# JakobHavtorn/benchmarking-lvms

Hardware: AMD Instinct MI355X
Metric: audio frames/sec training (VRNN, 16 kHz mu-law) (higher is better)
Workload: dtype f32

## Files before the change

### benchmarking-lvms_amd/blvm/ops.py

```python
import ctypes
from typing import List, NamedTuple, Optional, Sequence

import torch

from . import _hip
from ._hip import VrnnWeights, check, load, ptr, stream_ptr

ACT_NONE, ACT_RELU, ACT_LEAKY = 0, 1, 2
LEAKY_SLOPE = 0.01

LAYOUT_BATCH_MAJOR, LAYOUT_TIME_MAJOR = 0, 1

seq_timer_hook = None


def _tick(tag):
    if seq_timer_hook is not None:
        seq_timer_hook(tag)


def _c_ints(v):
    return (ctypes.c_int * len(v))(*[int(i) for i in v])


# ... 626 lines not shown


def _rollout(scratch_floats, T, max_scratch_floats, who, x, call, carry):
    n = _steps_per_launch(scratch_floats, T, max_scratch_floats, who) if T > 0 else 0
    scratch = torch.empty(scratch_floats(n), device=x.device, dtype=torch.float32)
    if n == T:
        call(0, T, None, x, scratch)
        return
    state = None
    for t0 in range(0, T, n):
        t1 = min(T, t0 + n)
        xc = torch.empty(x.shape[0], t1 - t0, x.shape[2], device=x.device, dtype=torch.float32)
        call(t0, t1, state, xc, scratch)
        x[:, t0:t1] = xc
        state = carry(xc, t1)


def _decode_weight_ptrs(w, first, first_lin, dec_lin, lik_lin):
    keep = [_f32c(t) for lin in (*first_lin, *dec_lin, lik_lin) for t in (lin.weight, lin.bias)]
    names = [f"{part}_{k}{i}" for part in (first, "dec") for i in range(3) for k in "wb"] + ["lik_w", "lik_b"]
    _hip.fill(w, names, [ptr(t) for t in keep])
    return keep


def _head_scalars(head):
    if isinstance(head, DmolHead):
        return 0, int(head.num_mix), float(head.log_eps), 0.0, 0.0
    if isinstance(head, GmmHead):
        return 1, int(head.num_mix), 0.0, float(head.sd_beta), float(head.sd_eps)
    if isinstance(head, GaussHead):
        return 2, 0, 0.0, float(head.sd_beta), float(head.sd_eps)
    raise TypeError(f"head: one of ops.DmolHead, ops.GmmHead, ops.GaussHead (got {type(head).__name__})")


@torch.no_grad()
def vrnn_decode(enc_lin, cell_params, dec_lin, lik_lin, x0, h0, eps, u, v, S, H, Z, R, num_mix, sd_eps, slope, log_eps, whole_chip=None,
                max_scratch_floats=None, head=None):
    from ._hip import VrnnDecodeWeights

    lib = load()
    T, B = eps.shape[0], x0.shape[0]
    dev = x0.device
    cp = [_f32c(p) for p in cell_params]
    cw = _pack_weights(cp)
    w = VrnnDecodeWeights()
    keep = _decode_weight_ptrs(w, "enc", enc_lin, dec_lin, lik_lin)
    w.cell = ctypes.pointer(cw)
    x0, eps = _f32c(x0), _f32c(eps)
    h0 = _f32c(h0) if h0 is not None else None
    u = _f32c(u) if u is not None else None
    v = _f32c(v) if v is not None else None
    if whole_chip is None:
        whole_chip = B <= lib.blvm_pchain_max_batch()
    hs5 = None if head is None else _head_scalars(head)
    x = torch.empty(B, T, S, device=dev, dtype=torch.float32)
    hn = torch.empty(B, R, device=dev, dtype=torch.float32)
    if whole_chip:

        def call(t0, t1, state, xc, scratch):
            xs, hs = (x0, h0) if state is None else state
            uc, vc = (None if u is None else u[t0:t1]), (None if v is None else v[t0:t1])
            if hs5 is None:
                check(lib.blvm_vrnn_generate(ctypes.byref(w), ptr(xs), ptr(hs), ptr(eps[t0:t1]), ptr(uc), ptr(vc), t1 - t0, B, S, H, Z, R, num_mix,
                                             sd_eps, slope, log_eps, ptr(xc), ptr(hn), ptr(scratch), stream_ptr()), "blvm_vrnn_generate")
            else:
                check(lib.blvm_vrnn_generate_head(ctypes.byref(w), ptr(xs), ptr(hs), ptr(eps[t0:t1]), ptr(uc), ptr(vc), t1 - t0, B, S, H, Z, R, *hs5,
                                                  sd_eps, slope, ptr(xc), ptr(hn), ptr(scratch), stream_ptr()), "blvm_vrnn_generate_head")

        floats = ((lambda n: lib.blvm_vrnn_generate_scratch_floats(n, B, S, H, Z, R)) if hs5 is None
                  else (lambda n: lib.blvm_vrnn_generate_scratch_floats_head(n, B, S, H, Z, R, hs5[0])))
        _rollout(floats, T, max_scratch_floats, "vrnn_decode", x, call, lambda xc, t1: (xc[:, -1].contiguous(), hn.clone()))
        return x, hn
    scratch = torch.empty(lib.blvm_vrnn_decode_scratch_floats(S, H, Z, R), device=dev, dtype=torch.float32)
    if hs5 is None:
        check(lib.blvm_vrnn_decode(ctypes.byref(w), ptr(x0), ptr(h0), ptr(eps), ptr(u), ptr(v), T, B, S, H, Z, R, num_mix, sd_eps, slope,
                                   log_eps, ptr(x), ptr(hn), ptr(scratch), stream_ptr()), "blvm_vrnn_decode")
    else:
        check(lib.blvm_vrnn_decode_head(ctypes.byref(w), ptr(x0), ptr(h0), ptr(eps), ptr(u), ptr(v), T, B, S, H, Z, R, *hs5, sd_eps, slope,
                                        ptr(x), ptr(hn), ptr(scratch), stream_ptr()), "blvm_vrnn_decode_head")
    return x, hn


class _VRNNSeqFunction(torch.autograd.Function):

    @staticmethod
    def forward(ctx, enc, h0, eps, x_sl_dev, cfg, dec, *params):
        Tp, B, X, H, Z, R, residual, sd_eps, stride, fn_floor = cfg
        enc, eps = _f32c(enc), _f32c(eps)
        params, dparams = tuple(_f32c(p) for p in params[:28]), tuple(_f32c(p) for p in params[28:])
        dev = enc.device
        lib = load()
        f32 = dict(device=dev, dtype=torch.float32)
        decin = torch.empty(Tp + 1, B, H + R, **f32)
        mu_q, sd_q, mu_p, sd_p, z = (torch.empty(Tp, B, Z, **f32) for _ in range(5))
        w = _pack_weights(params)
        if dec is None:
            reserve = torch.empty(lib.blvm_vrnn_reserve_floats(Tp, B, X, H, Z, R), **f32)
            _tick("fwd_begin")
            check(
                lib.blvm_vrnn_seq_fwd(w, ptr(enc), ptr(_f32c(h0)) if h0 is not None else None, ptr(eps), Tp, B, X, H, Z, R,
                                      int(residual), sd_eps, ptr(decin), ptr(mu_q), ptr(sd_q), ptr(mu_p), ptr(sd_p), ptr(z),
                                      ptr(reserve), stream_ptr()),
                "blvm_vrnn_seq_fwd",
            )
        else:
            keep = [_f32c(t.detach()) for lin in dec.layers for t in (lin.weight, lin.bias)]
            DH, SF = keep[0].shape[0], keep[4].shape[0]
            ys = [torch.empty(Tp * B, n, **f32) for n in (DH, DH, SF)]
            three = ctypes.c_void_p * 3
            dw, db, dy = three(*(ptr(t) for t in keep[0::2])), three(*(ptr(t) for t in keep[1::2])), three(*(ptr(t) for t in ys))
            reserve = torch.empty(lib.blvm_vrnn_fwd_reserve_floats(Tp, B, X, H, Z, R, DH, SF), **f32)
            folded = ctypes.c_int(0)
            _tick("fwd_begin")
            check(
                lib.blvm_vrnn_seq_fwd_dec(w, ptr(enc), ptr(_f32c(h0)) if h0 is not None else None, ptr(eps), Tp, B, X, H, Z, R,
                                          int(residual), sd_eps, ptr(decin), ptr(mu_q), ptr(sd_q), ptr(mu_p), ptr(sd_p), ptr(z),
                                          ptr(reserve), dw, db, dy, DH, SF, dec.slope, ctypes.byref(folded), stream_ptr()),
                "blvm_vrnn_seq_fwd_dec",
            )
            dec.given = tuple(ys[: folded.value]) if folded.value else None
        joint = dec is not None and len(dparams) == 6 and dec.given is not None and len(dec.given) == 3
        _tick("fwd_end")
        kld = torch.zeros(B, device=dev, dtype=torch.float64)
        kld_fn = torch.zeros(B, device=dev, dtype=torch.float64)
        check(
            lib.blvm_kl_fwd(ptr(mu_q), ptr(sd_q), ptr(mu_p), ptr(sd_p), LAYOUT_TIME_MAJOR, ptr(x_sl_dev), B, Tp, Z, stride,
                            fn_floor, ptr(kld), ptr(kld_fn), stream_ptr()),
            "blvm_kl_fwd",
        )
        ctx.cfg = cfg
        ctx.has_h0 = h0 is not None
        ctx.joint, ctx.n_dpar, ctx.dec_slope = joint, len(dparams), dec.slope if joint else 0.0
        ctx.save_for_backward(enc, eps, x_sl_dev, decin, mu_q, sd_q, mu_p, sd_p, z, reserve, *params, *((*dparams, ys[0], ys[1]) if joint else ()))
        ctx.mark_non_differentiable(mu_q, sd_q, mu_p, sd_p, z)
        ctx.set_materialize_grads(False)
        return decin, kld, kld_fn, mu_q, sd_q, mu_p, sd_p, z, (ys[2] if joint else None)

    @staticmethod
    def backward(ctx, d_decin, g_kld, g_kld_fn, *rest):
        Tp, B, X, H, Z, R, residual, sd_eps, stride, fn_floor = ctx.cfg
        enc, eps, x_sl_dev, decin, mu_q, sd_q, mu_p, sd_p, z, reserve, *params = ctx.saved_tensors
        dev = enc.device
        lib = load()
        f32 = dict(device=dev, dtype=torch.float32)
        c_raw = _grad_f32(g_kld) if g_kld is not None else None
        c_fn = _grad_f32(g_kld_fn) if g_kld_fn is not None else None
        d_dec = rest[5] if ctx.joint else None
        dgrads = (None,) * ctx.n_dpar
        if d_dec is not None:
            params, (W1, b1, W2, b2, W3, b3, y1, y2) = params[:28], params[28:]
            dz3, M, DH, SF, slope = _f32c(d_dec), Tp * B, W2.shape[0], W3.shape[0], ctx.dec_slope
            dy2, dy1 = torch.empty(M, DH, **f32), torch.empty(M, DH, **f32)
            grads = _zeros_like_many(params)
            d_enc = torch.empty_like(enc)
            d_h0 = torch.empty(B, R, **f32) if ctx.has_h0 else None
            w, g = _pack_weights(params), _pack_weights(grads, _hip.VrnnGrads)
            folded = ctypes.c_int(0)
            if d_decin is None:
                ws = torch.empty(lib.blvm_vrnn_bwd_dec_workspace_floats(Tp, B, X, H, Z, R, DH, SF), **f32)
                dw = (ctypes.c_void_p * 3)(ptr(W1), ptr(W2), ptr(W3))
                _tick("bwd_begin")
                check(
                    lib.blvm_vrnn_seq_bwd_dec(w, ptr(enc), ptr(eps), ptr(decin), ptr(mu_q), ptr(sd_q), ptr(mu_p), ptr(sd_p), ptr(z),
                                              ptr(reserve), ptr(x_sl_dev), ptr(c_raw), ptr(c_fn), stride, fn_floor, Tp, B, X, H, Z, R,
                                              int(residual), sd_eps, ptr(d_enc), ptr(d_h0), g, ptr(ws), ptr(dz3), ptr(y1), ptr(y2), dw,
                                              ptr(dy2), ptr(dy1), DH, SF, slope, ctypes.byref(folded), stream_ptr()),
                    "blvm_vrnn_seq_bwd_dec",
                )
            if not folded.value:
                gemm(0, 1, M, DH, SF, dz3, SF, W3, DH, dy2, DH, slope=slope, gate=y2, ldg=DH)
                gemm(0, 1, M, DH, DH, dy2, DH, W2, DH, dy1, DH, slope=slope, gate=y1, ldg=DH)
                dx = torch.empty(M, H + R, **f32)
                gemm(0, 1, M, H + R, DH, dy1, DH, W1, H + R, dx, H + R, slope=slope)
                dd = torch.zeros_like(decin)
                dd[:Tp] = dx.view(Tp, B, H + R)
                if d_decin is not None:
                    dd = dd + _f32c(d_decin)
                ws = torch.empty(lib.blvm_vrnn_bwd_workspace_floats(Tp, B, X, H, Z, R), **f32)
                _tick("bwd_begin")
                check(
                    lib.blvm_vrnn_seq_bwd(w, ptr(enc), ptr(eps), ptr(decin), ptr(mu_q), ptr(sd_q), ptr(mu_p), ptr(sd_p), ptr(z),
                                          ptr(reserve), ptr(dd), ptr(x_sl_dev), ptr(c_raw), ptr(c_fn), stride, fn_floor, Tp, B,
                                          X, H, Z, R, int(residual), sd_eps, ptr(d_enc), ptr(d_h0), g, ptr(ws), stream_ptr()),
                    "blvm_vrnn_seq_bwd",
                )
            _tick("bwd_end")
            dpar = (W1, b1, W2, b2, W3, b3)
            want = [ctx.needs_input_grad[6 + 28 + i] for i in range(6)]
            sizes = [(dpar[i].numel() + 3) // 4 * 4 if want[i] else 0 for i in range(6)]
            flat = torch.zeros(sum(sizes), **f32)
            views, off = [], 0
            for i in range(6):
                views.append(flat[off : off + dpar[i].numel()].view(dpar[i].shape) if want[i] else None)
                off += sizes[i]
            x2d = decin[:Tp].view(M, H + R)
            wgrad_group([(dz3, y2, views[4], views[5]), (dy2, y1, views[2], views[3]), (dy1, x2d, views[0], views[1])], M)
            return (d_enc, d_h0, None, None, None, None, *grads, *views)
        params = params[:28]
        d_decin = _f32c(d_decin) if d_decin is not None else torch.zeros_like(decin)
        grads = _zeros_like_many(params)
        d_enc = torch.empty_like(enc)
        d_h0 = torch.empty(B, R, **f32) if ctx.has_h0 else None
        ws = torch.empty(lib.blvm_vrnn_bwd_workspace_floats(Tp, B, X, H, Z, R), **f32)
        w, g = _pack_weights(params), _pack_weights(grads, _hip.VrnnGrads)
        _tick("bwd_begin")
        check(
            lib.blvm_vrnn_seq_bwd(w, ptr(enc), ptr(eps), ptr(decin), ptr(mu_q), ptr(sd_q), ptr(mu_p), ptr(sd_p), ptr(z),
                                  ptr(reserve), ptr(d_decin), ptr(x_sl_dev), ptr(c_raw), ptr(c_fn), stride, fn_floor, Tp, B,
                                  X, H, Z, R, int(residual), sd_eps, ptr(d_enc), ptr(d_h0), g, ptr(ws), stream_ptr()),
            "blvm_vrnn_seq_bwd",
        )
        _tick("bwd_end")
        return (d_enc, d_h0, None, None, None, None, *grads, *dgrads)


def vrnn_sequence(enc, h0, eps, x_sl_dev, params: Sequence[torch.Tensor], X, H, Z, R, residual_posterior, stride,
                  free_nats=0.0, sd_eps=1e-6, decoder=None):
    Tp, B, _ = enc.shape
    fn_floor = float(free_nats) / Z if free_nats else 0.0
    cfg = (Tp, B, X, H, Z, R, int(residual_posterior), float(sd_eps), int(stride), fn_floor)
    if decoder is None:
        return _VRNNSeqFunction.apply(enc, h0, eps, x_sl_dev, cfg, None, *params)[:8]
    decoder.given = decoder.dec = None
    dparams = ()
    if decoder.head_gates and load().blvm_vrnn_dec_bwd_fold(-1):
        dparams = tuple(t for lin in decoder.layers for t in (lin.weight, lin.bias))
    *out, decoder.dec = _VRNNSeqFunction.apply(enc, h0, eps, x_sl_dev, cfg, decoder, *params, *dparams)
    return tuple(out)


class DecoderFold:

    def __init__(self, layers, slope: float = LEAKY_SLOPE, head_gates: bool = False):
        self.layers, self.slope, self.given, self.head_gates, self.dec = list(layers), float(slope), None, bool(head_gates), None




class _LSTMSeqFunction(torch.autograd.Function):
    @staticmethod
    def forward(ctx, inp, h0, c0, lens_dev, Wih, Whh, bih, bhh):
        inp, Wih, Whh, bih, bhh = (_f32c(t) for t in (inp, Wih, Whh, bih, bhh))
        T, B, I = inp.shape
        H = Whh.shape[1]
        lib = load()
        f32 = dict(device=inp.device, dtype=torch.float32)
        out = torch.empty(T, B, H, **f32)
        hn, cn = torch.empty(B, H, **f32), torch.empty(B, H, **f32)
        reserve = torch.empty(lib.blvm_lstm_reserve_floats(T, B, H), **f32)
        check(
            lib.blvm_lstm_seq_fwd(ptr(Wih), ptr(Whh), ptr(bih), ptr(bhh), ptr(inp), ptr(_f32c(h0)) if h0 is not None else None,
                                  ptr(_f32c(c0)) if c0 is not None else None, ptr(lens_dev), T, B, I, H, ptr(out), ptr(hn), ptr(cn),
                                  ptr(reserve), stream_ptr()),
            "blvm_lstm_seq_fwd",
        )
        ctx.dims = (T, B, I, H)
        ctx.has_state = (h0 is not None, c0 is not None)
        ctx.save_for_backward(inp, Wih, Whh, reserve)
        ctx.mark_non_differentiable(hn, cn)
        return out, hn, cn

    @staticmethod
    def backward(ctx, d_out, _dhn, _dcn):
        T, B, I, H = ctx.dims
        inp, Wih, Whh, reserve = ctx.saved_tensors
        lib = load()
        f32 = dict(device=inp.device, dtype=torch.float32)
        d_out = _f32c(d_out)
        d_in = torch.empty_like(inp) if ctx.needs_input_grad[0] else None
        d_h0 = torch.empty(B, H, **f32) if ctx.has_state[0] and ctx.needs_input_grad[1] else None
        d_c0 = torch.empty(B, H, **f32) if ctx.has_state[1] and ctx.needs_input_grad[2] else None
        dWih, dWhh = torch.zeros_like(Wih), torch.zeros_like(Whh)
        dbih, dbhh = torch.zeros(4 * H, **f32), torch.zeros(4 * H, **f32)
        ws = torch.empty(lib.blvm_lstm_bwd_workspace_floats(T, B, H), **f32)
        check(
            lib.blvm_lstm_seq_bwd(ptr(Wih), ptr(Whh), ptr(inp), ptr(reserve), ptr(d_out), T, B, I, H, ptr(d_in), ptr(d_h0),
                                  ptr(d_c0), ptr(dWih), ptr(dWhh), ptr(dbih), ptr(dbhh), ptr(ws), stream_ptr()),
            "blvm_lstm_seq_bwd",
        )
        return d_in, d_h0, d_c0, None, dWih, dWhh, dbih, dbhh


def lstm_sequence(inp, h0, c0, lens_dev, Wih, Whh, bih, bhh):
    return _LSTMSeqFunction.apply(inp, h0, c0, lens_dev, Wih, Whh, bih, bhh)


class _LSTMBidirSeqFunction(torch.autograd.Function):

    @staticmethod
    def forward(ctx, inp, lens_dev, Wih_f, Whh_f, bih_f, bhh_f, Wih_r, Whh_r, bih_r, bhh_r):
        inp, *params = (_f32c(t) for t in (inp, Wih_f, Whh_f, bih_f, bhh_f, Wih_r, Whh_r, bih_r, bhh_r))
        T, B, I = inp.shape
        H = params[1].shape[1]
        lib = load()
        if not lib.blvm_lstm_bidir_applies(T, B, H):
            return None
        f32 = dict(device=inp.device, dtype=torch.float32)
        out = torch.empty(T, B, 2 * H, **f32)
        reserve = torch.empty(lib.blvm_lstm_bidir_reserve_floats(T, B, H), **f32)
        rc = lib.blvm_lstm_bidir_fwd(*(ptr(p) for p in params), ptr(inp), ptr(lens_dev), T, B, I, H, ptr(out), ptr(reserve), stream_ptr())
        if rc == BLVM_NOT_APPLICABLE:
            return None
        check(rc, "blvm_lstm_bidir_fwd")
        ctx.dims = (T, B, I, H)
        ctx.save_for_backward(inp, lens_dev, reserve, *params)
        return out

    @staticmethod
    def backward(ctx, d_out):
        T, B, I, H = ctx.dims
        inp, lens_dev, reserve, Wih_f, Whh_f, bih_f, bhh_f, Wih_r, Whh_r, bih_r, bhh_r = ctx.saved_tensors
        lib = load()
        d_out = _f32c(d_out)
        d_in = torch.empty_like(inp) if ctx.needs_input_grad[0] else None
        grads = [torch.zeros_like(p) for p in (Wih_f, Whh_f, bih_f, bhh_f, Wih_r, Whh_r, bih_r, bhh_r)]
        ws = torch.empty(lib.blvm_lstm_bidir_bwd_workspace_floats(T, B, H), device=inp.device, dtype=torch.float32)
        check(
            lib.blvm_lstm_bidir_bwd(ptr(Wih_f), ptr(Whh_f), ptr(Wih_r), ptr(Whh_r), ptr(inp), ptr(lens_dev), ptr(reserve), ptr(d_out),
                                    T, B, I, H, ptr(d_in), *(ptr(g) for g in grads), ptr(ws), stream_ptr()),
            "blvm_lstm_bidir_bwd",
        )
        return (d_in, None, *grads)


def lstm_bidir_sequence(inp, lens_dev, fwd_params, rev_params):
    return _LSTMBidirSeqFunction.apply(inp, lens_dev, *fwd_params, *rev_params)


def lstm_bidir_path_counts():
    out = (ctypes.c_ulonglong * 2)()
    check(load().blvm_lstm_bidir_path_counts(out), "blvm_lstm_bidir_path_counts")
    return int(out[0]), int(out[1])


def lstm_decode_weights(emb_lin, lstm, dec_lin, lik_lin):
    L = lstm.num_layers
    lk = [[_f32c(getattr(lstm, f"{n}_l{l}")) for l in range(L)] for n in ("weight_ih", "weight_hh", "bias_ih", "bias_hh")]
    arrays = [(ctypes.c_void_p * L)(*[t.data_ptr() for t in ts]) for ts in lk]
    w = _hip.LstmDecodeWeights()
    keep = _decode_weight_ptrs(w, "emb", emb_lin, dec_lin, lik_lin)
    w.wih, w.whh, w.bih, w.bhh = (ctypes.cast(a, ctypes.POINTER(ctypes.c_void_p)) for a in arrays)
    return w, (keep, lk, arrays)


def lstm_generate(emb_lin, lstm, dec_lin, lik_lin, x0, h0, c0, u, v, S, H, num_mix, log_eps, T=None, max_scratch_floats=None):
    lib = load()
    L, B, dev = lstm.num_layers, x0.shape[0], x0.device
    if (u is None) != (v is None) or (u is None and T is None):
        raise ValueError("lstm_generate: u and v are given together; the mode (neither) needs T")
    T = int(T) if u is None else u.shape[0]
    w, _keep = lstm_decode_weights(emb_lin, lstm, dec_lin, lik_lin)
    x0 = _f32c(x0)
    h0 = _f32c(h0) if h0 is not None else None
    c0 = _f32c(c0) if c0 is not None else None
# ... 1217 lines not shown
```

### benchmarking-lvms_amd/csrc/vrnn.hip

```cpp
#include <vector>
#include <stdlib.h>

#include <algorithm>
#include <atomic>

#include "common.h"
#include "pchain.h"
#include "vrnn_static.h"

namespace blvm {
namespace {

#include "stages.h"


template <int NW>
__global__ __launch_bounds__(NW * 64) void gru_stage_kernel(const float* decin_t, const float* Wih, const float* xg,
                                                            const float* gh, int B, int H, int R, float* decin_next,
                                                            float* rg, float* ug, float* ng) {
  __shared__ float red[3 * NW * 256];
  const int r0 = blockIdx.y * 16, c0 = blockIdx.x * 16, wave = threadIdx.x >> 6;
  const int ldd = H + R;
  const int t = threadIdx.x & 255;
  const int row = r0 + (t >> 4), col = c0 + (t & 15);
// ... 5 lines not shown
  const float hp = decin_t[(size_t)rowc * ldd + H + col];
  f32x4 acc[3];
#pragma unroll
  for (int g = 0; g < 3; ++g) acc[g] = (f32x4){0.f, 0.f, 0.f, 0.f};
  {
    const float* const As[3] = {decin_t, decin_t, decin_t};
    const float* const Ws[3] = {Wih, Wih, Wih};
    const int la[3] = {ldd, ldd, ldd}, lw[3] = {H, H, H}, cs[3] = {c0, R + c0, 2 * R + c0};
    wave_gemm16_multi<NW, 3, true>(As, la, r0, B, Ws, lw, cs, H, wave, acc);
  }
  float v[3];
  reduce_tiles<3, NW>(acc, red, v);
  if (!own) return;
  const float r = sigmoidf_(v[0] + x0 + hr);
  const float u = sigmoidf_(v[1] + x1 + hz);
  const float n = tanhf(v[2] + x2 + r * hn);
  decin_next[(size_t)row * ldd + H + col] = (1.f - u) * n + u * hp;
  const size_t o = (size_t)row * R + col;
  rg[o] = r; ug[o] = u; ng[o] = n;
}

struct DhArgs {
  const float *DP0, *DQ0;
  const float *WpT, *WqT;
  float* G;
  const float *rg, *ug, *ng, *gh;
  const float* decin_s;
  const float* ddecin_s;
  float *dgi, *dgh;
  int B, H, R, has_gemm, has_gates;
};

template <int NW>
__global__ __launch_bounds__(NW * 64) void dh_stage_kernel(const float* DP0, const float* DQ0, const float* WpT, const float* WqT,
                                                           float* G, unsigned b_h, int R, unsigned has, DhArgs a) {
  const int B = b_h & 0xffff, H = b_h >> 16;
  const int has_gemm = has & 1, has_gates = (has >> 1) & 1;
  __shared__ float red[2 * NW * 256];
  const int r0 = blockIdx.y * 16, c0 = blockIdx.x * 16, wave = threadIdx.x >> 6;
  const int ldd = H + R;
  const int t = threadIdx.x & 255;
  const int row = r0 + (t >> 4), col = c0 + (t & 15);
  const bool own = threadIdx.x < 256 && row < B;
  const int rowc = row < B ? row : r0;
  const size_t o = (size_t)rowc * R + col, o3 = (size_t)rowc * 3 * R + col;
  const float g0 = G[o];
  float r = 0.f, u = 0.f, n = 0.f, hn = 0.f, hp = 0.f, dd = 0.f;
  auto prefetch = [&]() {
    if (has_gates) {
      r = a.rg[o]; u = a.ug[o]; n = a.ng[o]; hn = a.gh[o3 + 2 * R];
      hp = a.decin_s[(size_t)rowc * ldd + H + col];
      dd = a.ddecin_s[(size_t)rowc * ldd + H + col];
    }
  };
  float v[2] = {0.f, 0.f};
  if (has_gemm) {
    f32x4 acc[2];
    acc[0] = (f32x4){0.f, 0.f, 0.f, 0.f};
    acc[1] = (f32x4){0.f, 0.f, 0.f, 0.f};
    {
      const float* const As[2] = {DP0, DQ0};
      const float* const Ws[2] = {WpT, WqT};
      const int ld[2] = {H, H}, cs[2] = {c0, c0};
      wave_gemm16_multi<NW, 2, false>(As, ld, r0, B, Ws, ld, cs, H, wave, acc, prefetch);
    }
    reduce_tiles<2, NW>(acc, red, v);
  } else {
    prefetch();
  }
  if (!own) return;
  const float g = g0 + v[0] + v[1];
  if (!has_gates) { G[o] = g; return; }
  const float dn_pre = g * (1.f - u) * (1.f - n * n);
  const float du_pre = g * (hp - n) * u * (1.f - u);
  const float dr_pre = dn_pre * hn * r * (1.f - r);
  a.dgi[o3] = dr_pre; a.dgi[o3 + R] = du_pre; a.dgi[o3 + 2 * R] = dn_pre;
  a.dgh[o3] = dr_pre; a.dgh[o3 + R] = du_pre; a.dgh[o3 + 2 * R] = dn_pre * r;
  G[o] = g * u + dd;
}

inline int vrnn_rt_max_b() {
  static int v = [] {
    const char* e = getenv("BLVM_PCHAIN_RT_MAX_B");
    return e ? atoi(e) : 256;
  }();
  return v;
}
inline int vrnn_rt(int B) {
  static const int min_b = [] { const char* e = getenv("BLVM_PCHAIN_RT_MIN_B"); return e ? atoi(e) : 65; }();
  if (B < min_b || B > vrnn_rt_max_b() || pchain_max_batch() <= 0 || operand_16bit()) return 0;
  if (B <= kPchainCarveMaxB && B > pchain_max_batch()) return 0;
  return 2;
}
inline bool vrnn_row_groups(int B) { return vrnn_rt(B) > 0; }
inline bool vrnn_shared_deal(bool groups, int tl) {
  static const int forced = [] { const char* e = getenv("BLVM_PCHAIN_SHARED"); return e ? atoi(e) : -1; }();
  static const int rt_tl = [] { const char* e = getenv("BLVM_PCHAIN_RT_SHARED_TL"); return e ? atoi(e) : 7; }();
  if (forced >= 0) return forced != 0;
  return groups && rt_tl > 0 && tl >= rt_tl;
}
inline bool vrnn_persistent(int B) { return pchain_applies(B) || vrnn_row_groups(B); }

struct Reserve {
  float *P[3], *Q[3], *FZ[3], *GHb, *RG, *UG, *NG, *XQ, *XG, *RAWQ, *RAWP;
  float *Wp[3], *Wq[3], *Wph, *Wqh, *Wf[4], *Wih, *Whh;
  float *H16, *P16[3], *Q16[3], *Z16, *FZ16[3], *PHI16;
  float *Y116, *Y216, *Y1P, *Wd[3];
  size_t x16_bytes;
};

size_t carve_reserve(float* base, int Tp, int B, int H, int Z, int R, Reserve* r, int SF = 0) {
  const size_t n = (size_t)Tp * B;
  Arena ar{base};
  Reserve tmp;
  for (int i = 0; i < 3; ++i) tmp.P[i] = ar.take(n * H);
  for (int i = 0; i < 3; ++i) tmp.Q[i] = ar.take(n * H);
  for (int i = 0; i < 3; ++i) tmp.FZ[i] = ar.take(n * H);
  tmp.GHb = ar.take(n * 3 * R);
  tmp.RG = ar.take(n * R); tmp.UG = ar.take(n * R); tmp.NG = ar.take(n * R);
  tmp.XQ = ar.take(n * H);
  tmp.XG = ar.take(n * 3 * R);
  tmp.RAWQ = ar.take(n * Z); tmp.RAWP = ar.take(n * Z);
  tmp.Wp[0] = ar.take((size_t)H * R); tmp.Wq[0] = ar.take((size_t)H * R);
  for (int i = 1; i < 3; ++i) { tmp.Wp[i] = ar.take((size_t)H * H); tmp.Wq[i] = ar.take((size_t)H * H); }
  tmp.Wph = ar.take((size_t)2 * Z * H); tmp.Wqh = ar.take((size_t)2 * Z * H);
  tmp.Wf[0] = ar.take((size_t)H * Z);
  for (int i = 1; i < 4; ++i) tmp.Wf[i] = ar.take((size_t)H * H);
  tmp.Wih = ar.take((size_t)3 * R * H); tmp.Whh = ar.take((size_t)3 * R * R);
  tmp.H16 = nullptr;
  if (B <= kPchainCarveMaxB || B <= vrnn_rt_max_b()) {
    const size_t rows = (size_t)((B + 15) / 16) * 16, m = (size_t)Tp * rows;
    tmp.H16 = ar.take((m + rows) * R);
    for (int i = 0; i < 3; ++i) tmp.P16[i] = ar.take(m * H);
    for (int i = 0; i < 3; ++i) tmp.Q16[i] = ar.take(m * H);
    tmp.Z16 = ar.take(m * Z);
    for (int i = 0; i < 3; ++i) tmp.FZ16[i] = ar.take(m * H);
    tmp.PHI16 = ar.take(m * H);
    tmp.Y116 = tmp.Y216 = tmp.Y1P = nullptr;
    if (SF > 0) { tmp.Y116 = ar.take(m * H); tmp.Y216 = ar.take(m * H); tmp.Y1P = ar.take(n * H); }
    tmp.x16_bytes = ar.bytes_from(tmp.H16);
    if (SF > 0) { tmp.Wd[0] = ar.take((size_t)H * (H + R)); tmp.Wd[1] = ar.take((size_t)H * H); tmp.Wd[2] = ar.take((size_t)SF * H); }
  }
  if (r) *r = tmp;
  return ar.floats();
}

struct BwdWs {
  float *pT[3], *phT, *qT[3], *qhT, *fT[4], *wihT, *whhT;
  float *DGI, *DGH, *DPHI[4], *DQH, *DPH, *DP[3], *DQ[3], *G;
  float *GA, *GB, *DP16[3], *DQ16[3], *DGI16, *DGH16, *DPHI16[4], *DPH16, *DQH16, *DPHI16b, *DPHI16c;
  size_t x16_bytes;
  float *DPHI3b, *DPHI3c;
  float *DY216, *DY116, *DD, *dT[3];
};

size_t carve_ws(float* base, int Tp, int B, int X, int H, int Z, int R, BwdWs* w, int SF = 0) {
  (void)X;
  const size_t n = (size_t)Tp * B;
  Arena ar{base};
  BwdWs t;
  t.pT[0] = ar.take((size_t)R * H); t.pT[1] = ar.take((size_t)H * H); t.pT[2] = ar.take((size_t)H * H);
  t.phT = ar.take((size_t)H * 2 * Z);
  t.qT[0] = ar.take((size_t)R * H); t.qT[1] = ar.take((size_t)H * H); t.qT[2] = ar.take((size_t)H * H);
  t.qhT = ar.take((size_t)H * 2 * Z);
  t.fT[0] = ar.take((size_t)Z * H);
  for (int i = 1; i < 4; ++i) t.fT[i] = ar.take((size_t)H * H);
  t.wihT = ar.take((size_t)H * 3 * R);
  t.whhT = ar.take((size_t)R * 3 * R);
  t.DGI = ar.take(n * 3 * R); t.DGH = ar.take(n * 3 * R);
  for (int i = 0; i < 4; ++i) t.DPHI[i] = ar.take(n * H);
  t.DQH = ar.take(n * 2 * Z); t.DPH = ar.take(n * 2 * Z);
  for (int i = 0; i < 3; ++i) t.DP[i] = ar.take(n * H);
  for (int i = 0; i < 3; ++i) t.DQ[i] = ar.take(n * H);
  t.G = ar.take((size_t)B * R);
  t.GA = nullptr;
  if (B <= kPchainCarveMaxB || B <= vrnn_rt_max_b()) {
    const size_t m = (size_t)Tp * ((B + 15) / 16) * 16;
    t.GA = ar.take(n * R); t.GB = ar.take(n * R);
    for (int i = 0; i < 3; ++i) { t.DP16[i] = ar.take(m * H); t.DQ16[i] = ar.take(m * H); }
    t.DGI16 = ar.take(m * 3 * R); t.DGH16 = ar.take(m * 3 * R);
    for (int i = 0; i < 4; ++i) t.DPHI16[i] = ar.take(m * H);
    t.DPH16 = ar.take(m * 2 * Z); t.DQH16 = ar.take(m * 2 * Z);
    t.DPHI16b = ar.take(m * H); t.DPHI16c = ar.take(m * H);
    t.DY216 = t.DY116 = t.DD = nullptr;
    if (SF > 0) { t.DY216 = ar.take(m * H); t.DY116 = ar.take(m * H); t.DD = ar.take(n * (H + R)); }
    t.x16_bytes = ar.bytes_from(t.GA);
    t.DPHI3b = ar.take(n * H); t.DPHI3c = ar.take(n * H);
    if (SF > 0) { t.dT[0] = ar.take((size_t)(H + R) * H); t.dT[1] = ar.take((size_t)H * H); t.dT[2] = ar.take((size_t)H * SF); }
  }
  if (w) *w = t;
  return ar.floats();
}

__global__ __launch_bounds__(256) void add3_kernel(float4* __restrict__ a, const float4* __restrict__ b, const float4* __restrict__ c, size_t n4) {
  for (size_t i = (size_t)blockIdx.x * 256 + threadIdx.x; i < n4; i += (size_t)gridDim.x * 256) {
    float4 x = a[i];
    const float4 y = b[i], z = c[i];
    x.x += y.x + z.x; x.y += y.y + z.y; x.z += y.z + z.z; x.w += y.w + z.w;
    a[i] = x;
  }
}

inline bool pchain_split3() {
  static int v = [] {
    const char* e = getenv("BLVM_PCHAIN_SPLIT3");
    return e ? atoi(e) : 1;
  }();
  return v != 0;
}

struct VrnnDecoder {
  const float *w[3], *b[3];
  float* y[3];
};
int g_dec_fold = [] { const char* e = getenv("BLVM_VRNN_DEC_FOLD"); const int v = e ? atoi(e) : 1; return v >= 0 && v <= 2 ? v : 1; }();
long g_dec_folded = 0;
int dec_ct(int layers, int SF) { return layers == 3 ? SF / 16 : layers == 2 ? 1 : 0; }
int vrnn_dec_folds(int B, int H, int Z, int R, int DH, int SF) {
  if (!g_dec_fold || !vrnn_persistent(B) || device_cus() < 32 || operand_16bit() || pchain_optype(B) != OP_F32) return 0;
  if (B > 64 || vrnn_row_groups(B) || Z != H || DH != H || SF <= 0 || SF % 16 != 0) return 0;
  const int tl = (B + 15) / 16, layers = g_dec_fold == 2 ? 2 : 3;
  const bool fits = pchain::vrnn_fwd_deal(H / 16, Z / 16, R / 16, tl, device_cus() & ~7, vrnn_shared_deal(false, tl), dec_ct(layers, SF)).dec[0].nwg > 0;
  return fits ? layers : 0;
}

struct VrnnDecBwd {
  const float *dz3, *y1, *y2, *w[3];
  float *dy2, *dy1;
  int DH, SF;
  float slope;
};
int g_dec_bwd_fold = [] { const char* e = getenv("BLVM_VRNN_DEC_BWD_FOLD"); return e ? (atoi(e) != 0 ? 1 : 0) : 1; }();
long g_dec_bwd_folded = 0;
bool vrnn_dec_bwd_folds(int Tp, int B, int H, int Z, int R, int DH, int SF) {
  if (!g_dec_bwd_fold || !vrnn_persistent(B) || device_cus() < 32 || operand_16bit() || pchain_optype(B) != OP_F32) return false;
  if (B > 64 || vrnn_row_groups(B) || Z != H || DH != H || H != 256 || R != 512 || SF <= 0 || SF % 16 != 0) return false;
  if (Tp + 1 <= pchain::kArmAhead || Tp <= pchain::kBdecAhead) return false;
  const int tl = (B + 15) / 16;
  if (vrnn_shared_deal(false, tl)) return false;
  const pchain::VrnnBwdDeal dl = pchain::vrnn_bwd_deal(H / 16, Z / 16, R / 16, tl, device_cus() & ~7, false, pchain_split3(), (H + R) / 16);
  return dl.split3 && dl.bdec[0].nwg > 0;
}

enum { VRNN_FWD_PROGRAM = 0, VRNN_FWD_PER_LINK = 1, VRNN_BWD_PROGRAM = 2, VRNN_BWD_PER_LINK = 3, VRNN_ROW_GROUPS = 4, VRNN_LIN16 = 5, VRNN_LIN32 = 6 };
std::atomic<unsigned long long> g_vrnn_counts[7];
inline void count_vrnn(int k) { g_vrnn_counts[k].fetch_add(1, std::memory_order_relaxed); }
inline void count_lin(int tile_width) { count_vrnn(tile_width == 32 ? VRNN_LIN32 : VRNN_LIN16); }

int check_dims(int Tp, int B, int X, int H, int Z, int R) {
  BLVM_REQUIRE(Tp > 0 && B > 0, "vrnn: bad Tp=%d B=%d", Tp, B);
  BLVM_REQUIRE(X > 0 && H > 0 && Z > 0 && R > 0 && X % 16 == 0 && H % 16 == 0 && Z % 16 == 0 && R % 16 == 0,
               "vrnn: X,H,Z,R must be positive multiples of 16 (got %d,%d,%d,%d)", X, H, Z, R);
  BLVM_REQUIRE(B < 65536 && H < 65536 && R < 65536, "vrnn: B, H and R must be below 65536 (packed kernel arguments)");
  return BLVM_OK;
}

}
}

using namespace blvm;

extern "C" int blvm_vrnn_path_counts(unsigned long long out[7]) {
  BLVM_REQUIRE(out, "vrnn_path_counts: null pointer");
  for (int k = 0; k < 7; ++k) out[k] = g_vrnn_counts[k].load(std::memory_order_relaxed);
  return BLVM_OK;
}

extern "C" size_t blvm_vrnn_reserve_floats(int Tp, int B, int X, int H, int Z, int R) {
  (void)X;
  return carve_reserve(nullptr, Tp, B, H, Z, R, nullptr);
}
extern "C" size_t blvm_vrnn_fwd_reserve_floats(int Tp, int B, int X, int H, int Z, int R, int DH, int SF) {
  (void)X;
  return carve_reserve(nullptr, Tp, B, H, Z, R, nullptr, vrnn_dec_folds(B, H, Z, R, DH, SF) ? SF : 0);
}
extern "C" int blvm_vrnn_dec_fold(int mode) {
  if (mode == -2) return (int)std::min<long>(g_dec_folded, 0x7fffffffL);
  const int was = g_dec_fold;
  if (mode >= 0) g_dec_fold = mode <= 2 ? mode : 1;
  return was;
}

extern "C" size_t blvm_vrnn_bwd_workspace_floats(int Tp, int B, int X, int H, int Z, int R) {
  return carve_ws(nullptr, Tp, B, X, H, Z, R, nullptr);
}
extern "C" size_t blvm_vrnn_bwd_dec_workspace_floats(int Tp, int B, int X, int H, int Z, int R, int DH, int SF) {
  return carve_ws(nullptr, Tp, B, X, H, Z, R, nullptr, vrnn_dec_bwd_folds(Tp, B, H, Z, R, DH, SF) ? SF : 0);
}
extern "C" int blvm_vrnn_dec_bwd_fold(int mode) {
  if (mode == -2) return (int)std::min<long>(g_dec_bwd_folded, 0x7fffffffL);
  const int was = g_dec_bwd_fold;
  if (mode >= 0) g_dec_bwd_fold = mode != 0;
  return was;
}

static int vrnn_seq_fwd_impl(const BlvmVrnnWeights* w, const float* enc, const float* h0, const float* eps,
                             int Tp, int B, int X, int H, int Z, int R, int residual_posterior, float sd_eps,
                             float* decin, float* mu_q, float* sd_q, float* mu_p, float* sd_p, float* z,
                             float* reserve, hipStream_t s, const VrnnDecoder* dec = nullptr, int DH = 0, int SF = 0,
                             float dec_slope = 0.f, int* folded = nullptr) {
  BLVM_TRY(check_dims(Tp, B, X, H, Z, R));
  BLVM_REQUIRE(w && enc && eps && decin && mu_q && sd_q && mu_p && sd_p && z && reserve, "vrnn_fwd: null pointer");
  BLVM_REQUIRE(aligned16(enc) && aligned16(decin) && aligned16(reserve) && aligned16(z),
               "vrnn_fwd: buffers must be 16-byte aligned");
  if (folded) *folded = 0;
  const int fold = dec != nullptr ? vrnn_dec_folds(B, H, Z, R, DH, SF) : 0;
  Reserve rs;
  carve_reserve(reserve, Tp, B, H, Z, R, &rs, fold ? SF : 0);
  const size_t n = (size_t)Tp * B;
  const int ldd = H + R;
  const float beta = softplus_beta_of(sd_eps);

  BLVM_TRY(gemm_f32(0, 0, (int)n, H, X, enc, X, w->post_w[0] + R, R + X, rs.XQ, H, w->post_b[0], 0, 0.f, nullptr, 0, 0, 1, s));
  BLVM_TRY(gemm_f32(0, 0, (int)n, 3 * R, X, enc, X, w->gru_wih, X + H, rs.XG, 3 * R, w->gru_bih, 0, 0.f, nullptr, 0, 0, 1, s));

  T16PackScope pack_scope(pchain_optype(B), s);
  BLVM_TRY(t16_pack_rows(w->prior_w[0], R, H, R, rs.Wp[0], s));
  BLVM_TRY(t16_pack_rows(w->post_w[0], R + X, H, R, rs.Wq[0], s));
  for (int l = 1; l < 3; ++l) {
    BLVM_TRY(t16_pack_rows(w->prior_w[l], H, H, H, rs.Wp[l], s));
    BLVM_TRY(t16_pack_rows(w->post_w[l], H, H, H, rs.Wq[l], s));
  }
  BLVM_TRY(t16_pack_rows(w->prior_hw, H, 2 * Z, H, rs.Wph, s));
  BLVM_TRY(t16_pack_rows(w->post_hw, H, 2 * Z, H, rs.Wqh, s));
  BLVM_TRY(t16_pack_rows(w->phi_w[0], Z, H, Z, rs.Wf[0], s));
  for (int l = 1; l < 4; ++l) BLVM_TRY(t16_pack_rows(w->phi_w[l], H, H, H, rs.Wf[l], s));
  BLVM_TRY(t16_pack_rows(w->gru_wih + X, X + H, 3 * R, H, rs.Wih, s));
  BLVM_TRY(t16_pack_rows(w->gru_whh, R, 3 * R, R, rs.Whh, s));
  if (fold) {
    BLVM_TRY(t16_pack_rows(dec->w[0], H + R, H, H + R, rs.Wd[0], s));
    BLVM_TRY(t16_pack_rows(dec->w[1], H, H, H, rs.Wd[1], s));
    if (fold == 3) BLVM_TRY(t16_pack_rows(dec->w[2], H, SF, H, rs.Wd[2], s));
  }
  BLVM_TRY(pack_scope.flush());

  if (!(vrnn_persistent(B) && device_cus() >= 32)) BLVM_HIP(copy_or_zero_2d(decin + H, sizeof(float) * ldd, h0, sizeof(float) * R, B, s));
  BLVM_HIP(hipMemset2DAsync(decin + n * ldd, sizeof(float) * ldd, 0, sizeof(float) * H, B, s));

  const int rt = (B + 15) / 16;
  if (vrnn_persistent(B) && device_cus() >= 32) {
    using namespace pchain;
    const int ctH = H / 16, ctZ = Z / 16, ctR = R / 16, cus = device_cus() & ~7;
    const long sH = (long)B * H, sZ = (long)B * Z, sR = (long)B * R, s3R = 3 * sR, sD = (long)B * ldd;
    const long xH = (long)rt * 16 * H, xZ = (long)rt * 16 * Z, xR = (long)rt * 16 * R;
    const bool groups = vrnn_row_groups(B);
    count_vrnn(VRNN_FWD_PROGRAM);
    if (groups) count_vrnn(VRNN_ROW_GROUPS);
    const int RTG = groups ? vrnn_rt(B) : 1;
    const int tl = (rt + RTG - 1) / RTG;
    const bool shared = vrnn_shared_deal(groups, tl);
    const VrnnFwdDeal dl = vrnn_fwd_deal(ctH, ctZ, ctR, tl, cus, shared, dec_ct(fold, SF));
    Builder bld;
    bld.begin(pchain_optype(B), Tp, B, groups ? 8 : 4, false, dl.g);
    bld.p.rt_group = RTG;
    Operands hp;
    hp.p[LIN_A] = {rs.H16, xR}; hp.p[LIN_W] = rs.Whh; hp.p[LIN_BIAS] = w->gru_bhh; hp.p[LIN_ORM] = {rs.GHb, s3R}; hp.ld[LD_OUT] = 3 * R;
    auto hproj = [&]() { add_desc(bld, K_LIN, dl.hproj.ct, dl.hproj.wg0, dl.hproj.nwg, R, DF_RM_SC1 | DF_GENTLE | ((pchain_tune() & 16) ? DF_CANARY : 0), 0, Tp, hp); };
    if (!shared) hproj();
    {
      const SeqLink lp[3] = {{rs.Wp[0], w->prior_b[0], rs.P[0], sH, H, rs.P16[0]}, {rs.Wp[1], w->prior_b[1], rs.P[1], sH, H, rs.P16[1]}, {rs.Wp[2], w->prior_b[2], rs.P[2], sH, H, rs.P16[2]}};
      const SeqLink lq[3] = {{rs.Wq[0], nullptr, rs.Q[0], sH, H, rs.Q16[0]}, {rs.Wq[1], w->post_b[1], rs.Q[1], sH, H, rs.Q16[1]}, {rs.Wq[2], w->post_b[2], rs.Q[2], sH, H, rs.Q16[2]}};
      add_linseq(bld, ctH, dl.prior.wg0, dl.prior.nwg, H, true, false, 0, Tp, {rs.H16, xR}, 3, lp, 0, xH, ctH, 0.f, 0, R);
      add_linseq(bld, ctH, dl.post.wg0, dl.post.nwg, H, true, false, 0, Tp, {rs.H16, xR}, 3, lq, 0, xH, ctH, 0.f, 0, R, {rs.XQ, sH}, H);
    }
    if (shared) hproj();
    {
      Operands o;
      o.p[HEAD_P16] = {rs.P16[2], xH}; o.p[HEAD_Q16] = {rs.Q16[2], xH}; o.p[HEAD_WP] = rs.Wph; o.p[HEAD_BP] = w->prior_hb; o.p[HEAD_WQ] = rs.Wqh;
      o.p[HEAD_BQ] = w->post_hb; o.p[HEAD_EPS] = {eps, sZ}; o.p[HEAD_MU_P] = {mu_p, sZ}; o.p[HEAD_SD_P] = {sd_p, sZ}; o.p[HEAD_MU_Q] = {mu_q, sZ};
      o.p[HEAD_SD_Q] = {sd_q, sZ}; o.p[HEAD_RAW_P] = {rs.RAWP, sZ}; o.p[HEAD_RAW_Q] = {rs.RAWQ, sZ}; o.p[HEAD_Z] = {z, sZ}; o.p[HEAD_Z16] = {rs.Z16, xZ};
      o.ld[LD_OUT] = Z; o.n16[N16_OUT] = ctZ; o.i[HEAD_I_Z] = Z; o.i[HEAD_I_RESIDUAL] = residual_posterior; o.f[HEAD_F_BETA] = beta; o.f[HEAD_F_INV_BETA] = 1.f / beta;
      o.f[HEAD_F_SD_EPS] = sd_eps;
      add_desc(bld, K_HEAD, ctZ, dl.head.wg0, dl.head.nwg, H, 0, 0, Tp, o);
    }
    const int first_seq = Z == H ? 0 : 1;
    if (first_seq) {
      Operands o;
      o.p[LIN_A] = {rs.Z16, xZ}; o.p[LIN_W] = rs.Wf[0]; o.p[LIN_BIAS] = w->phi_b[0]; o.p[LIN_ORM] = {rs.FZ[0], sH}; o.ld[LD_OUT] = H; o.p[LIN_O16] = {rs.FZ16[0], xH};
      o.n16[N16_OUT] = ctH;
      add_desc(bld, K_LIN, ctH, dl.phi.wg0, dl.phi.nwg, Z, DF_RELU, 0, Tp, o);
    }
    {
      SeqLink lf[4];
      for (int l = first_seq; l < 4; ++l)
        lf[l - first_seq] = SeqLink{rs.Wf[l], w->phi_b[l], l == 3 ? decin : rs.FZ[l], l == 3 ? sD : sH, l == 3 ? ldd : H, l == 3 ? rs.PHI16 : rs.FZ16[l]};
      add_linseq(bld, ctH, dl.phi.wg0, dl.phi.nwg, H, true, false, 0, Tp, first_seq == 0 ? Ptr(rs.Z16, xZ) : Ptr(rs.FZ16[0], xH), 4 - first_seq,
                 lf, 0, xH, ctH, 0.f, 0);
    }
    {
      Operands o;
      o.p[GRU_X16] = {rs.PHI16, xH}; o.p[GRU_WIH] = rs.Wih; o.p[GRU_XG] = {rs.XG, s3R}; o.p[GRU_GH] = {rs.GHb, s3R}; o.p[GRU_HPREV] = {decin + H, sD};
      o.p[GRU_HRM] = {decin + sD + H, sD}; o.p[GRU_H16] = {rs.H16 + xR, xR}; o.p[GRU_RG] = {rs.RG, sR}; o.p[GRU_UG] = {rs.UG, sR}; o.p[GRU_NG] = {rs.NG, sR};
      o.ld[GRU_LD_HPREV] = ldd; o.ld[LD_OUT] = ldd; o.n16[N16_OUT] = ctR; o.i[GRU_I_R] = R;
      add_desc(bld, K_GRU, ctR, dl.gru.wg0, dl.gru.nwg, H, 0, 0, Tp, o);
    }
    if (fold) {
      const long sF = (long)B * SF;
      const int canary = (pchain_tune() & 16) ? DF_CANARY : 0, ldw = H + R;
      Operands o;
      o.p[LIN_A] = {rs.H16, xR}; o.p[LIN_W] = rs.Wd[0] + (size_t)ctH * 256; o.i[LIN_I_W_WIDTH] = ldw; o.p[LIN_BIAS] = dec->b[0];
      o.p[LIN_ORM] = {rs.Y1P, sH}; o.ld[LD_OUT] = H;
      add_desc(bld, K_LIN, dl.dec[0].ct, dl.dec[0].wg0, dl.dec[0].nwg, R, DF_RM_SC1 | DF_GENTLE | canary, 0, Tp, o);
      o = Operands();
      o.p[LIN_A] = {rs.PHI16, xH}; o.p[LIN_W] = rs.Wd[0]; o.i[LIN_I_W_WIDTH] = ldw; o.p[LIN_ADD] = {rs.Y1P, sH}; o.ld[LIN_LD_ADD] = H;
      o.p[LIN_ORM] = {dec->y[0], sH}; o.ld[LD_OUT] = H; o.p[LIN_O16] = {rs.Y116, xH}; o.n16[N16_OUT] = ctH; o.f[LIN_F_SLOPE] = dec_slope;
      add_desc(bld, K_LIN, dl.dec[1].ct, dl.dec[1].wg0, dl.dec[1].nwg, H, DF_ADD_POLLED | DF_RELU | DF_GENTLE | canary, 0, Tp, o);
      o = Operands();
      o.p[LIN_A] = {rs.Y116, xH}; o.p[LIN_W] = rs.Wd[1]; o.p[LIN_BIAS] = dec->b[1]; o.p[LIN_ORM] = {dec->y[1], sH}; o.ld[LD_OUT] = H;
      o.p[LIN_O16] = {rs.Y216, xH}; o.n16[N16_OUT] = ctH; o.f[LIN_F_SLOPE] = dec_slope;
      add_desc(bld, K_LIN, dl.dec[2].ct, dl.dec[2].wg0, dl.dec[2].nwg, H, DF_RELU | DF_GENTLE | canary, 0, Tp, o);
      if (fold == 3) {
        o = Operands();
        o.p[LIN_A] = {rs.Y216, xH}; o.p[LIN_W] = rs.Wd[2]; o.p[LIN_BIAS] = dec->b[2]; o.p[LIN_ORM] = {dec->y[2], sF}; o.ld[LD_OUT] = SF;
        o.f[LIN_F_SLOPE] = dec_slope;
        add_desc(bld, K_LIN, dl.dec[3].ct, dl.dec[3].wg0, dl.dec[3].nwg, H, DF_RELU | DF_GENTLE | canary, 0, Tp, o);
      }
    }
    ArmPlan plan;
    plan.fill(rs.H16, rs.x16_bytes);
    plan.fill(rs.GHb, sizeof(float) * n * 3 * R);
    plan.fill(decin, sizeof(float) * n * ldd);
    if (!groups) {
      plan.add(arm_t16(rs.H16, R, rt, Tp + 1));
      for (int i = 0; i < 3; ++i) { plan.add(arm_t16(rs.P16[i], H, rt, Tp)); plan.add(arm_t16(rs.Q16[i], H, rt, Tp)); plan.add(arm_t16(rs.FZ16[i], H, rt, Tp)); }
      plan.add(arm_t16(rs.Z16, Z, rt, Tp));
      plan.add(arm_t16(rs.PHI16, H, rt, Tp));
      plan.add(arm_t16(rs.Y116, H, rt, Tp)); plan.add(arm_t16(rs.Y216, H, rt, Tp));
      plan.add(arm_rm(rs.Y1P, H, B, Tp));
      plan.add(arm_rm(rs.GHb, 3 * R, B, Tp));
      plan.add(arm_rm(decin, ldd, B, Tp));
    }
    auto pre = [&]() -> int {
      BLVM_HIP(copy_or_zero_2d(decin + H, sizeof(float) * ldd, h0, sizeof(float) * R, B, s));
      return pchain_rows_to_t16(h0, R, B, R, rs.H16, s);
    };
    BLVM_TRY(vrnn_launch(bld, true, "vrnn_fwd", s, plan, pre));
    if (fold) { ++g_dec_folded; if (folded) *folded = fold; }
    return BLVM_OK;
  }
  count_vrnn(VRNN_FWD_PER_LINK);
  for (int t = 0; t < Tp; ++t) {
    const size_t oH = (size_t)t * B * H, oZ = (size_t)t * B * Z, oR = (size_t)t * B * R, o3R = (size_t)t * B * 3 * R;
    const float* dec_t = decin + (size_t)t * B * ldd;
    float* dec_n = decin + (size_t)(t + 1) * B * ldd;
    const float* hprev = dec_t + H;
    LinLaunch a;
    a.B = B;
    a.nseg = 3;
    a.seg[0] = seg(hprev, ldd, rs.Wp[0], R, w->prior_b[0], nullptr, 0, nullptr, 0, rs.P[0] + oH, H, H, R, 1);
    a.seg[1] = seg(hprev, ldd, rs.Wq[0], R, nullptr, rs.XQ + oH, H, nullptr, 0, rs.Q[0] + oH, H, H, R, 1);
    a.seg[2] = seg(hprev, ldd, rs.Whh, R, w->gru_bhh, nullptr, 0, nullptr, 0, rs.GHb + o3R, 3 * R, 3 * R, R, 0);
    count_lin(launch_lin(a, s));
    a.nseg = 2;
    for (int l = 1; l < 3; ++l) {
      a.seg[0] = seg(rs.P[l - 1] + oH, H, rs.Wp[l], H, w->prior_b[l], nullptr, 0, nullptr, 0, rs.P[l] + oH, H, H, H, 1);
      a.seg[1] = seg(rs.Q[l - 1] + oH, H, rs.Wq[l], H, w->post_b[l], nullptr, 0, nullptr, 0, rs.Q[l] + oH, H, H, H, 1);
      count_lin(launch_lin(a, s));
    }
    HeadArgs h;
    h.P = rs.P[2] + oH; h.Q = rs.Q[2] + oH;
    h.Wp = rs.Wph; h.bp = w->prior_hb; h.Wq = rs.Wqh; h.bq = w->post_hb;
    h.eps = eps + oZ;
    h.mu_p = mu_p + oZ; h.sd_p = sd_p + oZ; h.mu_q = mu_q + oZ; h.sd_q = sd_q + oZ; h.z = z + oZ;
    h.raw_p = rs.RAWP + oZ; h.raw_q = rs.RAWQ + oZ;
    h.B = B; h.H = H; h.Z = Z; h.residual = residual_posterior;
    h.beta = beta; h.inv_beta = 1.f / beta; h.sd_eps = sd_eps; h.muq_raw = nullptr;
    launch_head(h, pick_nw(H, 4), dim3(Z / 16, rt), s);
    a.nseg = 1;
    a.seg[0] = seg(z + oZ, Z, rs.Wf[0], Z, w->phi_b[0], nullptr, 0, nullptr, 0, rs.FZ[0] + oH, H, H, Z, 1);
    count_lin(launch_lin(a, s));
    a.seg[0] = seg(rs.FZ[0] + oH, H, rs.Wf[1], H, w->phi_b[1], nullptr, 0, nullptr, 0, rs.FZ[1] + oH, H, H, H, 1);
    count_lin(launch_lin(a, s));
    a.seg[0] = seg(rs.FZ[1] + oH, H, rs.Wf[2], H, w->phi_b[2], nullptr, 0, nullptr, 0, rs.FZ[2] + oH, H, H, H, 1);
    count_lin(launch_lin(a, s));
    a.seg[0] = seg(rs.FZ[2] + oH, H, rs.Wf[3], H, w->phi_b[3], nullptr, 0, nullptr, 0, decin + (size_t)t * B * ldd, ldd, H, H, 1);
    count_lin(launch_lin(a, s));
    {
      const int nw = pick_nw(H, 3);
      const dim3 grid(R / 16, rt);
      const float *xg_t = rs.XG + o3R, *gh_t = rs.GHb + o3R;
      float *rg_t = rs.RG + oR, *ug_t = rs.UG + oR, *ng_t = rs.NG + oR;
      LAUNCH_NW(gru_stage_kernel<NW_>, nw, grid, s, dec_t, (const float*)rs.Wih, xg_t, gh_t, B, H, R, dec_n, rg_t, ug_t, ng_t);
    }
  }
  BLVM_CHECK_LAUNCH("vrnn_seq_fwd");
  return BLVM_OK;
}

extern "C" int blvm_vrnn_seq_fwd(const BlvmVrnnWeights* w, const float* enc, const float* h0, const float* eps,
                                 int Tp, int B, int X, int H, int Z, int R, int residual_posterior, float sd_eps,
                                 float* decin, float* mu_q, float* sd_q, float* mu_p, float* sd_p, float* z,
                                 float* reserve, void* stream_) {
  return vrnn_seq_fwd_impl(w, enc, h0, eps, Tp, B, X, H, Z, R, residual_posterior, sd_eps, decin, mu_q, sd_q, mu_p, sd_p, z, reserve,
                           static_cast<hipStream_t>(stream_));
}

extern "C" int blvm_vrnn_seq_fwd_dec(const BlvmVrnnWeights* w, const float* enc, const float* h0, const float* eps,
                                     int Tp, int B, int X, int H, int Z, int R, int residual_posterior, float sd_eps,
                                     float* decin, float* mu_q, float* sd_q, float* mu_p, float* sd_p, float* z,
                                     float* reserve, const float* const* dec_w, const float* const* dec_b, float* const* dec_y,
                                     int DH, int SF, float slope, int* folded, void* stream_) {
  BLVM_REQUIRE(dec_w && dec_b && dec_y && folded, "vrnn_seq_fwd_dec: null pointer");
  VrnnDecoder d;
  for (int l = 0; l < 3; ++l) {
    d.w[l] = dec_w[l]; d.b[l] = dec_b[l]; d.y[l] = dec_y[l];
    BLVM_REQUIRE(d.w[l] && d.b[l] && d.y[l] && aligned16(d.y[l]), "vrnn_seq_fwd_dec: decoder layer %d: null or unaligned pointer", l);
  }
  BLVM_REQUIRE(DH > 0 && SF > 0, "vrnn_seq_fwd_dec: bad decoder widths %d, %d", DH, SF);
  return vrnn_seq_fwd_impl(w, enc, h0, eps, Tp, B, X, H, Z, R, residual_posterior, sd_eps, decin, mu_q, sd_q, mu_p, sd_p, z, reserve,
                           static_cast<hipStream_t>(stream_), &d, DH, SF, slope, folded);
}

static int vrnn_seq_bwd_impl(const BlvmVrnnWeights* w, const float* enc, const float* eps, const float* decin,
                             const float* mu_q, const float* sd_q, const float* mu_p, const float* sd_p,
                             const float* z, const float* reserve, const float* d_decin, const int32_t* x_sl,
                             const float* c_raw, const float* c_fn, int stride, float fn_floor, int Tp, int B, int X, int H, int Z,
                             int R, int residual_posterior, float sd_eps, float* d_enc, float* d_h0,
                             const BlvmVrnnGrads* gr, float* workspace, hipStream_t s, const VrnnDecBwd* dec = nullptr) {
  BLVM_TRY(check_dims(Tp, B, X, H, Z, R));
  BLVM_REQUIRE(w && enc && eps && decin && mu_q && sd_q && mu_p && sd_p && z && reserve && (d_decin || dec) && workspace && gr,
               "vrnn_bwd: null pointer");
  BLVM_REQUIRE((c_fn == nullptr && c_raw == nullptr) || x_sl != nullptr, "vrnn_bwd: KL coefficients need x_sl");
  BLVM_REQUIRE(aligned16(workspace) && aligned16(reserve) && aligned16(d_decin), "vrnn_bwd: buffers must be 16-byte aligned");
  Reserve rs;
  carve_reserve(const_cast<float*>(reserve), Tp, B, H, Z, R, &rs);
  BwdWs ws;
  carve_ws(workspace, Tp, B, X, H, Z, R, &ws, dec ? dec->SF : 0);
  const size_t n = (size_t)Tp * B;
  const int ldd = H + R;
  const float beta = softplus_beta_of(sd_eps);

  T16PackScope pack_scope(pchain_optype(B), s);
  BLVM_TRY(t16_pack_transposed(w->prior_w[0], R, H, R, ws.pT[0], s));
  BLVM_TRY(t16_pack_transposed(w->prior_w[1], H, H, H, ws.pT[1], s));
  BLVM_TRY(t16_pack_transposed(w->prior_w[2], H, H, H, ws.pT[2], s));
  BLVM_TRY(t16_pack_transposed(w->prior_hw, H, 2 * Z, H, ws.phT, s));
  BLVM_TRY(t16_pack_transposed(w->post_w[0], R + X, H, R, ws.qT[0], s));
  BLVM_TRY(t16_pack_transposed(w->post_w[1], H, H, H, ws.qT[1], s));
  BLVM_TRY(t16_pack_transposed(w->post_w[2], H, H, H, ws.qT[2], s));
  BLVM_TRY(t16_pack_transposed(w->post_hw, H, 2 * Z, H, ws.qhT, s));
  BLVM_TRY(t16_pack_transposed(w->phi_w[0], Z, H, Z, ws.fT[0], s));
  for (int i = 1; i < 4; ++i) BLVM_TRY(t16_pack_transposed(w->phi_w[i], H, H, H, ws.fT[i], s));
  BLVM_TRY(t16_pack_transposed(w->gru_wih + X, X + H, 3 * R, H, ws.wihT, s));
  BLVM_TRY(t16_pack_transposed(w->gru_whh, R, 3 * R, R, ws.whhT, s));
  if (dec) {
    BLVM_TRY(t16_pack_transposed(dec->w[0], H + R, H, H + R, ws.dT[0], s));
    BLVM_TRY(t16_pack_transposed(dec->w[1], H, H, H, ws.dT[1], s));
    BLVM_TRY(t16_pack_transposed(dec->w[2], H, dec->SF, H, ws.dT[2], s));
  }
  BLVM_TRY(pack_scope.flush());

  BLVM_HIP(hipMemsetAsync(ws.G, 0, sizeof(float) * (size_t)B * R, s));
  const int rt = (B + 15) / 16;

  auto launch_dh = [&](int t_gemm, int s_gates) {
    DhArgs d;
    d.has_gemm = t_gemm >= 0; d.has_gates = s_gates >= 0;
    d.DP0 = d.has_gemm ? ws.DP[0] + (size_t)t_gemm * B * H : nullptr;
    d.DQ0 = d.has_gemm ? ws.DQ[0] + (size_t)t_gemm * B * H : nullptr;
    d.WpT = ws.pT[0]; d.WqT = ws.qT[0]; d.G = ws.G;
    const size_t sg = d.has_gates ? (size_t)s_gates : 0;
    d.rg = rs.RG + sg * B * R; d.ug = rs.UG + sg * B * R; d.ng = rs.NG + sg * B * R;
    d.gh = rs.GHb + sg * B * 3 * R;
    d.decin_s = decin + sg * B * ldd; d.ddecin_s = d_decin + sg * B * ldd;
    d.dgi = ws.DGI + sg * B * 3 * R; d.dgh = ws.DGH + sg * B * 3 * R;
    d.B = B; d.H = H; d.R = R;
    {
      const int nw = pick_nw(H, 2);
      const dim3 grid(R / 16, rt);
      const unsigned b_h = (unsigned)B | ((unsigned)H << 16), has = (d.has_gemm ? 1u : 0u) | (d.has_gates ? 2u : 0u);
      LAUNCH_NW(dh_stage_kernel<NW_>, nw, grid, s, d.DP0, d.DQ0, d.WpT, d.WqT, d.G, b_h, R, has, d);
    }
  };

  const float* hprev_all = decin + H;
  auto batched = [&]() -> int {
    if (d_enc) {
      BLVM_TRY(gemm_f32(0, 1, (int)n, X, H, ws.DQ[0], H, w->post_w[0] + R, R + X, d_enc, X, nullptr, 0, 0.f, nullptr, 0, 0, 1, s));
      BLVM_TRY(gemm_f32(0, 1, (int)n, X, 3 * R, ws.DGI, 3 * R, w->gru_wih, X + H, d_enc, X, nullptr, 0, 0.f, nullptr, 0, 1, 1, s));
    }
    {
      WgradGroup grp;
      auto job = [&](const float* D, int ldd_, int n_out, const float* Act, int lda, int k_in, float* dW, int ldw, float* db = nullptr) {
        grp.add(D, ldd_, n_out, Act, lda, k_in, dW, ldw, db);
      };
      job(ws.DGI, 3 * R, 3 * R, enc, X, X, gr->gru_wih, X + H, gr->gru_bih);
      job(ws.DGI, 3 * R, 3 * R, decin, ldd, H, gr->gru_wih ? gr->gru_wih + X : nullptr, X + H);
      job(ws.DGH, 3 * R, 3 * R, hprev_all, ldd, R, gr->gru_whh, R, gr->gru_bhh);
      job(ws.DPHI[0], H, H, z, Z, Z, gr->phi_w[0], Z, gr->phi_b[0]);
      for (int l = 1; l < 4; ++l) job(ws.DPHI[l], H, H, rs.FZ[l - 1], H, H, gr->phi_w[l], H, gr->phi_b[l]);
      job(ws.DPH, 2 * Z, 2 * Z, rs.P[2], H, H, gr->prior_hw, H, gr->prior_hb);
      job(ws.DQH, 2 * Z, 2 * Z, rs.Q[2], H, H, gr->post_hw, H, gr->post_hb);
      for (int l = 2; l >= 1; --l) {
        job(ws.DP[l], H, H, rs.P[l - 1], H, H, gr->prior_w[l], H, gr->prior_b[l]);
        job(ws.DQ[l], H, H, rs.Q[l - 1], H, H, gr->post_w[l], H, gr->post_b[l]);
      }
      job(ws.DP[0], H, H, hprev_all, ldd, R, gr->prior_w[0], R, gr->prior_b[0]);
      job(ws.DQ[0], H, H, hprev_all, ldd, R, gr->post_w[0], R + X);
      job(ws.DQ[0], H, H, enc, X, X, gr->post_w[0] ? gr->post_w[0] + R : nullptr, R + X, gr->post_b[0]);
      BLVM_TRY(grp.run(n, s));
    }
    return BLVM_OK;
  };
  if (vrnn_persistent(B) && device_cus() >= 32) {
    using namespace pchain;
    const int ctH = H / 16, ctZ = Z / 16, ctR = R / 16, cus = device_cus() & ~7, T = Tp;
    const long sH = (long)B * H, sZ = (long)B * Z, sR = (long)B * R, s3R = 3 * sR, s2Z = 2 * sZ, sD = (long)B * ldd;
    const long xH = (long)rt * 16 * H, x2Z = (long)rt * 16 * 2 * Z, x3R = (long)rt * 16 * 3 * R;
    const bool groups = vrnn_row_groups(B);
    count_vrnn(VRNN_BWD_PROGRAM);
    if (groups) count_vrnn(VRNN_ROW_GROUPS);
    const int RTG = groups ? vrnn_rt(B) : 1;
    const int tl = (rt + RTG - 1) / RTG;
    const bool shared = vrnn_shared_deal(groups, tl);
    const VrnnBwdDeal dl = vrnn_bwd_deal(ctH, ctZ, ctR, tl, cus, shared, pchain_split3(), dec ? (H + R) / 16 : 0);
    BLVM_REQUIRE(!dec || (dl.split3 && dl.bdec[0].nwg > 0 && !groups), "vrnn_bwd: the deal has no decoder leader range");
    Builder bld;
    bld.begin(pchain_optype(B), T + 1, B, groups ? 8 : 2, true, dl.g);
    bld.p.rt_group = RTG;
    auto last = [&](const float* base, long step) { return rev(base, step, T - 1); };
    {
      Operands o;
      o.p[GRUB_D0_16] = rev(ws.DP16[0], xH, T); o.p[GRUB_D1_16] = rev(ws.DQ16[0], xH, T); o.p[GRUB_W0] = ws.pT[0]; o.p[GRUB_W1] = ws.qT[0];
      o.p[GRUB_G_IN] = rev(ws.GB, sR, T); o.p[GRUB_RG] = last(rs.RG, sR); o.p[GRUB_UG] = last(rs.UG, sR); o.p[GRUB_NG] = last(rs.NG, sR);
      o.p[GRUB_GH] = last(rs.GHb, s3R); o.p[GRUB_HPREV] = last(decin + H, sD); o.p[GRUB_DD] = dec ? Ptr() : last(d_decin + H, sD); o.p[GRUB_DGI] = last(ws.DGI, s3R);
      o.p[GRUB_DGI16] = last(ws.DGI16, x3R); o.p[GRUB_DGH] = last(ws.DGH, s3R); o.p[GRUB_DGH16] = last(ws.DGH16, x3R); o.p[GRUB_GA] = last(ws.GA, sR);
      o.p[GRUB_G_OUT] = d_h0 ? d_h0 : ws.G; o.ld[GRUB_LD_H] = ldd; o.ld[LD_OUT] = 3 * R; o.n16[N16_OUT] = 3 * ctR; o.i[GRUB_I_R] = R; o.i[GRUB_I_GEMM_FROM] = 1;
      o.i[GRUB_I_GATES_TO] = T; o.i[GRUB_I_GIN_FROM] = 1;
      add_desc(bld, K_GRUB, ctR, dl.grub.wg0, dl.grub.nwg, H, 0, 0, T + 1, o);
    }
    const bool split3 = dl.split3;
    Operands o;
    o.p[LIN_GATE] = last(decin, sD); o.ld[LIN_LD_ADD] = ldd; o.ld[LIN_LD_GATE] = ldd; o.ld[LD_OUT] = H; o.n16[N16_OUT] = ctH;
    if (split3) {
      const size_t wthird = (size_t)ctR * 256 / (bld.p.ot != OP_F32 ? 2 : 1);
      float* const orm[3] = {ws.DPHI[3], ws.DPHI3b, ws.DPHI3c};
      float* const o16[3] = {ws.DPHI16[3], ws.DPHI16b, ws.DPHI16c};
      o.ld[LIN_LD_A] = 3 * R; o.i[LIN_I_W_WIDTH] = 3 * R;
      for (int part = 0; part < 3; ++part) {
        o.p[LIN_A] = last(ws.DGI16 + (size_t)part * ctR * 256, x3R); o.p[LIN_W] = ws.wihT + part * wthird;
        o.p[LIN_ADD] = dec ? (part == 2 ? last(ws.DD, sD) : Ptr()) : (part == 0 ? last(d_decin, sD) : Ptr());
        o.p[LIN_ORM] = last(orm[part], sH); o.p[LIN_O16] = last(o16[part], xH);
        add_desc(bld, K_LIN, ctH, dl.part[part].wg0, dl.part[part].nwg, R, dec && part == 2 ? DF_ADD_POLLED | DF_ADD_EARLY : 0, 0, T, o);
      }
    } else {
      o.p[LIN_A] = last(ws.DGI16, x3R); o.p[LIN_W] = ws.wihT; o.p[LIN_ADD] = last(d_decin, sD); o.p[LIN_ORM] = last(ws.DPHI[3], sH);
      o.p[LIN_O16] = last(ws.DPHI16[3], xH);
      add_desc(bld, K_LIN, ctH, dl.dphi.wg0, dl.dphi.nwg, 3 * R, 0, 0, T, o);
    }
    Operands gb;
    gb.p[LIN_A] = last(ws.DGH16, x3R); gb.p[LIN_W] = ws.whhT; gb.p[LIN_ADD] = last(ws.GA, sR); gb.ld[LIN_LD_ADD] = R; gb.p[LIN_ORM] = last(ws.GB, sR); gb.ld[LD_OUT] = R;
    if (dec) { gb.p[LIN_ADD2] = last(ws.DD + H, sD); gb.i[LIN_I_LD_ADD2] = ldd; }
    add_desc(bld, K_LIN, ctR, dl.gb.wg0, dl.gb.nwg, 3 * R,
             DF_ADD_POLLED | DF_RM_SC1 | DF_GENTLE | ((pchain_tune() & 16) ? DF_CANARY : 0) | (dec ? DF_ADD2_POLLED : 0), 0, T, gb);
    auto blink = [&](const float* W, const float* gate, float* orm, float* o16) { return rev_link(W, gate, orm, o16, T - 1, sH, H, xH); };
    const SeqLink lf[3] = {blink(ws.fT[3], rs.FZ[2], ws.DPHI[2], ws.DPHI16[2]), blink(ws.fT[2], rs.FZ[1], ws.DPHI[1], ws.DPHI16[1]),
                           blink(ws.fT[1], rs.FZ[0], ws.DPHI[0], ws.DPHI16[0])};
    if (split3) {
      Operands o3;
      o3.p[LIN_A] = last(ws.DPHI16[3], xH); o3.p[LIN_W] = ws.fT[3]; o3.p[LIN_GATE] = last(rs.FZ[2], sH); o3.ld[LIN_LD_GATE] = H; o3.p[LIN_ORM] = last(ws.DPHI[2], sH);
      o3.ld[LD_OUT] = H; o3.p[LIN_O16] = last(ws.DPHI16[2], xH); o3.n16[N16_OUT] = ctH; o3.p[LIN_A2] = last(ws.DPHI16b, xH); o3.p[LIN_A3] = last(ws.DPHI16c, xH);
      add_desc(bld, K_LIN, ctH, dl.wide_h.wg0, dl.wide_h.nwg, H, DF_A_SUM3, 0, T, o3);
    }
    add_linseq(bld, ctH, dl.wide_h.wg0, dl.wide_h.nwg, H, false, true, 0, T, last(ws.DPHI16[split3 ? 2 : 3], xH), split3 ? 2 : 3, lf + (split3 ? 1 : 0), -sH,
               -xH, ctH, 0.f, H);
    {
      Operands z;
      z.p[DZ_D16] = last(ws.DPHI16[0], xH); z.p[DZ_WT] = ws.fT[0]; z.p[DZ_MU_Q] = last(mu_q, sZ); z.p[DZ_SD_Q] = last(sd_q, sZ); z.p[DZ_MU_P] = last(mu_p, sZ);
      z.p[DZ_SD_P] = last(sd_p, sZ); z.p[DZ_EPS] = last(eps, sZ); z.p[DZ_RAW_Q] = last(rs.RAWQ, sZ); z.p[DZ_RAW_P] = last(rs.RAWP, sZ); z.p[DZ_X_SL] = x_sl;
      z.p[DZ_C_RAW] = c_raw; z.p[DZ_C_FN] = c_fn; z.p[DZ_DQH] = last(ws.DQH, s2Z); z.p[DZ_DQH16] = last(ws.DQH16, x2Z); z.p[DZ_DPH] = last(ws.DPH, s2Z);
      z.p[DZ_DPH16] = last(ws.DPH16, x2Z); z.ld[LD_OUT] = 2 * Z; z.n16[N16_OUT] = 2 * ctZ; z.i[DZ_I_Z] = Z; z.i[DZ_I_RESIDUAL] = residual_posterior;
      z.i[DZ_I_STRIDE] = stride; z.i[DZ_I_T0] = T - 1; z.f[DZ_F_FN_FLOOR] = fn_floor; z.f[DZ_F_BETA] = beta; z.f[DZ_F_SD_EPS] = sd_eps;
      add_desc(bld, K_DZ, ctZ, dl.dz.wg0, dl.dz.nwg, H, 0, 0, T, z);
    }
    {
      const SeqLink lp[3] = {blink(ws.phT, rs.P[2], ws.DP[2], ws.DP16[2]), blink(ws.pT[2], rs.P[1], ws.DP[1], ws.DP16[1]), blink(ws.pT[1], rs.P[0], ws.DP[0], ws.DP16[0])};
      const SeqLink lq[3] = {blink(ws.qhT, rs.Q[2], ws.DQ[2], ws.DQ16[2]), blink(ws.qT[2], rs.Q[1], ws.DQ[1], ws.DQ16[1]), blink(ws.qT[1], rs.Q[0], ws.DQ[0], ws.DQ16[0])};
      add_linseq(bld, ctH, dl.prior.wg0, dl.prior.nwg, H, false, true, 0, T, last(ws.DPH16, x2Z), 3, lp, -sH, -xH, ctH, 0.f, H, 2 * Z);
      add_linseq(bld, ctH, dl.post.wg0, dl.post.nwg, H, false, true, 0, T, last(ws.DQH16, x2Z), 3, lq, -sH, -xH, ctH, 0.f, H, 2 * Z);
    }
    if (dec) {
      const int L = kBdecAhead, SF = dec->SF;
      const long sF = (long)B * SF;
      auto lead = [&](const float* base, long step) { return rev(base, step, T - 1 - L); };
      Operands b0, b1, b2;
      b0.p[LIN_A] = lead(dec->dz3, sF); b0.ld[LIN_LD_A] = SF; b0.p[LIN_W] = ws.dT[2]; b0.p[LIN_GATE] = lead(dec->y2, sH); b0.ld[LIN_LD_GATE] = H;
      b0.p[LIN_ORM] = lead(dec->dy2, sH); b0.ld[LD_OUT] = H; b0.p[LIN_O16] = lead(ws.DY216, xH); b0.n16[N16_OUT] = ctH; b0.f[LIN_F_SLOPE] = dec->slope;
      add_desc(bld, K_LIN, ctH, dl.bdec[0].wg0, dl.bdec[0].nwg, SF, DF_A_PLAIN | DF_GENTLE, 0, T - L, b0);
      b1.p[LIN_A] = lead(ws.DY216, xH); b1.p[LIN_W] = ws.dT[1]; b1.p[LIN_GATE] = lead(dec->y1, sH); b1.ld[LIN_LD_GATE] = H;
      b1.p[LIN_ORM] = lead(dec->dy1, sH); b1.ld[LD_OUT] = H; b1.p[LIN_O16] = lead(ws.DY116, xH); b1.n16[N16_OUT] = ctH; b1.f[LIN_F_SLOPE] = dec->slope;
      add_desc(bld, K_LIN, ctH, dl.bdec[1].wg0, dl.bdec[1].nwg, H, DF_GENTLE | DF_CANARY, 0, T - L, b1);
      b2.p[LIN_A] = lead(ws.DY116, xH); b2.p[LIN_W] = ws.dT[0]; b2.p[LIN_ORM] = lead(ws.DD, sD); b2.ld[LD_OUT] = ldd;
      add_desc(bld, K_LIN, (H + R) / 16, dl.bdec[2].wg0, dl.bdec[2].nwg, H, DF_RM_SC1 | DF_GENTLE | DF_CANARY, 0, T - L, b2);
    }
    ArmPlan plan;
    plan.fill(ws.GA, ws.x16_bytes);
    if (!groups) {
      plan.add(arm_rm(ws.GA, R, B, T, true)); plan.add(arm_rm(ws.GB, R, B, T, true));
      for (int i = 0; i < 3; ++i) { plan.add(arm_t16(ws.DP16[i], H, rt, T, true)); plan.add(arm_t16(ws.DQ16[i], H, rt, T, true)); }
      plan.add(arm_t16(ws.DGI16, 3 * R, rt, T, true)); plan.add(arm_t16(ws.DGH16, 3 * R, rt, T, true));
      for (int i = 0; i < 4; ++i) plan.add(arm_t16(ws.DPHI16[i], H, rt, T, true));
      plan.add(arm_t16(ws.DPH16, 2 * Z, rt, T, true)); plan.add(arm_t16(ws.DQH16, 2 * Z, rt, T, true));
      plan.add(arm_t16(ws.DPHI16b, H, rt, T, true)); plan.add(arm_t16(ws.DPHI16c, H, rt, T, true));
      if (dec) { plan.add(arm_t16(ws.DY216, H, rt, T, true)); plan.add(arm_t16(ws.DY116, H, rt, T, true)); plan.add(arm_rm(ws.DD, ldd, B, T, true)); }
    }
    auto lead_rows = [&]() -> int {
      if (!dec) return BLVM_OK;
      const int L = kBdecAhead, M = L * B, SF = dec->SF;
      const size_t r0 = (size_t)(T - L) * B;
      BLVM_TRY(gemm_f32(0, 1, M, H, SF, dec->dz3 + r0 * SF, SF, dec->w[2], H, dec->dy2 + r0 * H, H, nullptr, 0, dec->slope, dec->y2 + r0 * H, H, 0, 1, s));
      BLVM_TRY(gemm_f32(0, 1, M, H, H, dec->dy2 + r0 * H, H, dec->w[1], H, dec->dy1 + r0 * H, H, nullptr, 0, dec->slope, dec->y1 + r0 * H, H, 0, 1, s));
      return gemm_f32(0, 1, M, H + R, H, dec->dy1 + r0 * H, H, dec->w[0], H + R, ws.DD + r0 * ldd, ldd, nullptr, 0, 0.f, nullptr, 0, 0, 1, s);
    };
    BLVM_TRY(vrnn_launch(bld, false, "vrnn_bwd", s, plan, lead_rows));
    if (dec) ++g_dec_bwd_folded;
    if (split3) {
      const size_t n4 = n * H / 4;
      hipLaunchKernelGGL(add3_kernel, dim3((unsigned)std::min<size_t>((n4 + 255) / 256, 2048)), dim3(256), 0, s, reinterpret_cast<float4*>(ws.DPHI[3]),
                         reinterpret_cast<const float4*>(ws.DPHI3b), reinterpret_cast<const float4*>(ws.DPHI3c), n4);
    }
    return batched();
  }

  BLVM_REQUIRE(!dec, "vrnn_bwd: the decoder leader needs the persistent path");
  count_vrnn(VRNN_BWD_PER_LINK);
  launch_dh(-1, Tp - 1);
  for (int t = Tp - 1; t >= 0; --t) {
    const size_t oH = (size_t)t * B * H, oZ = (size_t)t * B * Z, o3R = (size_t)t * B * 3 * R, o2Z = (size_t)t * B * 2 * Z;
    const float* dec_t = decin + (size_t)t * B * ldd;
    const float* ddec_t = d_decin + (size_t)t * B * ldd;
    LinLaunch a;
    a.B = B;
    a.nseg = 2;
    a.seg[0] = seg(ws.DGI + o3R, 3 * R, ws.wihT, 3 * R, nullptr, ddec_t, ldd, dec_t, ldd, ws.DPHI[3] + oH, H, H, 3 * R, 0);
    a.seg[1] = seg(ws.DGH + o3R, 3 * R, ws.whhT, 3 * R, nullptr, ws.G, R, nullptr, 0, ws.G, R, R, 3 * R, 0);
    count_lin(launch_lin(a, s));
    a.nseg = 1;
    for (int l = 3; l >= 1; --l) {
      a.seg[0] = seg(ws.DPHI[l] + oH, H, ws.fT[l], H, nullptr, nullptr, 0, rs.FZ[l - 1] + oH, H, ws.DPHI[l - 1] + oH, H, H, H, 0);
      count_lin(launch_lin(a, s));
    }
    DzArgs d;
    d.D = ws.DPHI[0] + oH; d.WT = ws.fT[0]; d.D2 = nullptr; d.WT2 = nullptr; d.dz_add = nullptr; d.ld_add = 0; d.has_gemm = 1;
    d.mu_q = mu_q + oZ; d.sd_q = sd_q + oZ; d.mu_p = mu_p + oZ; d.sd_p = sd_p + oZ; d.eps = eps + oZ;
    d.raw_q = rs.RAWQ + oZ; d.raw_p = rs.RAWP + oZ;
    d.x_sl = x_sl; d.c_raw = c_raw; d.c_fn = c_fn;
    d.dqh = ws.DQH + o2Z; d.dph = ws.DPH + o2Z;
    d.B = B; d.H = H; d.Z = Z; d.residual = residual_posterior; d.t = t; d.stride = stride;
    d.fn_floor = fn_floor; d.beta = beta; d.sd_eps = sd_eps; d.muq_raw = nullptr;
    launch_dz(d, pick_nw(H, 1), dim3(Z / 16, rt), s);
    a.nseg = 2;
    a.seg[0] = seg(ws.DPH + o2Z, 2 * Z, ws.phT, 2 * Z, nullptr, nullptr, 0, rs.P[2] + oH, H, ws.DP[2] + oH, H, H, 2 * Z, 0);
    a.seg[1] = seg(ws.DQH + o2Z, 2 * Z, ws.qhT, 2 * Z, nullptr, nullptr, 0, rs.Q[2] + oH, H, ws.DQ[2] + oH, H, H, 2 * Z, 0);
    count_lin(launch_lin(a, s));
    for (int l = 2; l >= 1; --l) {
      a.seg[0] = seg(ws.DP[l] + oH, H, ws.pT[l], H, nullptr, nullptr, 0, rs.P[l - 1] + oH, H, ws.DP[l - 1] + oH, H, H, H, 0);
      a.seg[1] = seg(ws.DQ[l] + oH, H, ws.qT[l], H, nullptr, nullptr, 0, rs.Q[l - 1] + oH, H, ws.DQ[l - 1] + oH, H, H, H, 0);
      count_lin(launch_lin(a, s));
    }
    launch_dh(t, t - 1);
  }
  BLVM_CHECK_LAUNCH("vrnn_seq_bwd");
  if (d_h0) BLVM_HIP(hipMemcpyAsync(d_h0, ws.G, sizeof(float) * (size_t)B * R, hipMemcpyDeviceToDevice, s));

  return batched();
}

extern "C" int blvm_vrnn_seq_bwd(const BlvmVrnnWeights* w, const float* enc, const float* eps, const float* decin,
                                 const float* mu_q, const float* sd_q, const float* mu_p, const float* sd_p,
                                 const float* z, const float* reserve, const float* d_decin, const int32_t* x_sl,
                                 const float* c_raw, const float* c_fn, int stride, float fn_floor, int Tp, int B, int X, int H, int Z,
                                 int R, int residual_posterior, float sd_eps, float* d_enc, float* d_h0,
                                 const BlvmVrnnGrads* gr, float* workspace, void* stream_) {
  return vrnn_seq_bwd_impl(w, enc, eps, decin, mu_q, sd_q, mu_p, sd_p, z, reserve, d_decin, x_sl, c_raw, c_fn, stride, fn_floor, Tp, B, X,
                           H, Z, R, residual_posterior, sd_eps, d_enc, d_h0, gr, workspace, static_cast<hipStream_t>(stream_));
}

extern "C" int blvm_vrnn_seq_bwd_dec(const BlvmVrnnWeights* w, const float* enc, const float* eps, const float* decin,
                                     const float* mu_q, const float* sd_q, const float* mu_p, const float* sd_p, const float* z,
                                     const float* reserve, const int32_t* x_sl, const float* c_raw, const float* c_fn, int stride,
                                     float fn_floor, int Tp, int B, int X, int H, int Z, int R, int residual_posterior, float sd_eps,
                                     float* d_enc, float* d_h0, const BlvmVrnnGrads* gr, float* workspace, const float* dz3,
                                     const float* dec_y1, const float* dec_y2, const float* const* dec_w, float* dy2, float* dy1, int DH,
                                     int SF, float slope, int* folded, void* stream_) {
  BLVM_REQUIRE(folded != nullptr, "vrnn_bwd_dec: null pointer");
  *folded = 0;
  BLVM_TRY(check_dims(Tp, B, X, H, Z, R));
  if (!vrnn_dec_bwd_folds(Tp, B, H, Z, R, DH, SF)) return BLVM_OK;
  BLVM_REQUIRE(dz3 && dec_y1 && dec_y2 && dec_w && dec_w[0] && dec_w[1] && dec_w[2] && dy2 && dy1, "vrnn_bwd_dec: null pointer");
  BLVM_REQUIRE(aligned16(dz3) && aligned16(dy2) && aligned16(dy1), "vrnn_bwd_dec: buffers must be 16-byte aligned");
  const VrnnDecBwd dec{dz3, dec_y1, dec_y2, {dec_w[0], dec_w[1], dec_w[2]}, dy2, dy1, DH, SF, slope};
  BLVM_TRY(vrnn_seq_bwd_impl(w, enc, eps, decin, mu_q, sd_q, mu_p, sd_p, z, reserve, nullptr, x_sl, c_raw, c_fn, stride, fn_floor, Tp, B, X,
                             H, Z, R, residual_posterior, sd_eps, d_enc, d_h0, gr, workspace, static_cast<hipStream_t>(stream_), &dec));
  *folded = 1;
  return BLVM_OK;
}
```

### benchmarking-lvms_amd/csrc/vrnn_static.h

```cpp
#pragma once
#include <algorithm>
#include <initializer_list>

#include "pchain.h"

namespace blvm {
namespace pchain {

struct LinkRange {
  int ct, wg0, nwg;
};
constexpr int kMaxTiles = 8;
struct VrnnFwdDeal {
  int def_n, half, g, spare;
  LinkRange hproj, prior, post, head, phi, gru, dec[4];
};
inline VrnnFwdDeal vrnn_fwd_deal(int ctH, int ctZ, int ctR, int tl, int cus, bool shared, int ctD = 0) {
  VrnnFwdDeal d;
  d.def_n = shared ? 0 : range_for(3 * ctR * tl, std::min(cus / 4, 64));
  d.half = range_for(ctH * tl, (cus - d.def_n) / 2);
  d.g = 2 * d.half;
  const int wide = shared ? d.half : d.g;
  d.hproj = shared ? LinkRange{3 * ctR, d.half, d.half} : LinkRange{3 * ctR, d.g, d.def_n};
  d.prior = LinkRange{ctH, 0, d.half};
  d.post = LinkRange{ctH, d.half, d.half};
  d.head = LinkRange{ctZ, 0, range_for(ctZ * tl, wide)};
  d.phi = LinkRange{ctH, 0, range_for(ctH * tl, wide)};
  d.gru = LinkRange{ctR, 0, range_for(ctR * tl, d.g)};
  d.spare = shared ? 0 : cus - d.g - d.def_n;
  for (LinkRange& r : d.dec) r = LinkRange{0, 0, 0};
  if (ctD > 0 && d.spare >= 8) {
    const int w0 = d.g + d.def_n, n12 = range_for(ctH * tl, d.spare), n3 = range_for(ctD * tl, d.spare);
    bool fits = true;
    for (bool xcd : {false, true})
      fits = fits && tiles_per_workgroup(tl, ctH, n12, xcd) <= 1 && tiles_per_workgroup(tl, ctD, n3, xcd) <= kMaxTiles;
    if (fits) {
      d.dec[0] = d.dec[1] = d.dec[2] = LinkRange{ctH, w0, n12};
      d.dec[3] = LinkRange{ctD, w0, n3};
    }
  }
  return d;
}
constexpr int kBdecAhead = 2;
struct VrnnBwdDeal {
  int def_n, half, g, spare;
  bool split3;
  LinkRange grub, part[3], dphi, gb, wide_h, dz, prior, post, bdec[3];
};
inline VrnnBwdDeal vrnn_bwd_deal(int ctH, int ctZ, int ctR, int tl, int cus, bool shared, bool allow_split3, int ctD = 0) {
  VrnnBwdDeal d;
  d.def_n = shared ? 0 : range_for(ctR * tl, std::min(cus / 4, 64));
  d.half = range_for(ctH * tl, (cus - d.def_n) / 2);
  d.g = 2 * d.half;
  const int wide = shared ? d.half : d.g;
  d.spare = cus - d.g - d.def_n;
  d.split3 = !shared && d.spare >= 8 && d.half >= 8 && allow_split3;
  d.grub = LinkRange{ctR, 0, range_for(ctR * tl, d.g)};
  d.part[0] = LinkRange{ctH, 0, range_for(ctH * tl, d.half)};
  d.part[1] = LinkRange{ctH, d.half, range_for(ctH * tl, d.half)};
  d.part[2] = LinkRange{ctH, d.g + d.def_n, d.split3 ? range_for(ctH * tl, d.spare) : 0};
  d.dphi = LinkRange{ctH, 0, range_for(ctH * tl, wide)};
  d.gb = shared ? LinkRange{ctR, d.half, d.half} : LinkRange{ctR, d.g, d.def_n};
  d.wide_h = LinkRange{ctH, 0, range_for(ctH * tl, wide)};
  d.dz = LinkRange{ctZ, 0, range_for(ctZ * tl, wide)};
  d.prior = LinkRange{ctH, 0, d.half};
  d.post = LinkRange{ctH, d.half, d.half};
  for (LinkRange& r : d.bdec) r = LinkRange{0, 0, 0};
  if (ctD > 0 && d.split3) {
    const int w0 = d.part[2].wg0, n = d.part[2].nwg;
    bool fits = n == ctH * tl;
    for (bool xcd : {false, true})
      fits = fits && tiles_per_workgroup(tl, ctH, n, xcd) <= 1 && tiles_per_workgroup(tl, ctD, n, xcd) <= kMaxTiles;
    if (fits) {
      d.bdec[0] = d.bdec[1] = LinkRange{ctH, w0, n};
      d.bdec[2] = LinkRange{ctD, w0, n};
    }
  }
  return d;
}

constexpr std::initializer_list<int> kFwdResident = {1, 2, 3, 4, 5};
constexpr std::initializer_list<int> kBwdResident = {0, 1, 2, 3, 5, 6, 7, 8, 9};
constexpr int kFwdDesc = 6, kFwdDecDesc = 10;
constexpr std::initializer_list<int> kFwdDecResident = {6, 7, 8};
constexpr int kBwdDesc = 10, kBwdDecDesc = 13;
constexpr std::initializer_list<int> kBwdDecResident = {11};
inline bool one_tile_each(const Program& p, std::initializer_list<int> links, bool xcd) {
  for (int i : links)
    if (tiles_per_workgroup((p.B + 15) / 16, p.d[i].ct, p.d[i].nwg, xcd) > 1) return false;
  return true;
}
inline bool one_tile_each(const Program& p, std::initializer_list<int> links) { return one_tile_each(p, links, p.xcd != 0); }

enum Place {
  kPlaceProgram = 0,
  kPlacePlain = 1,
  kPlaceLocal = 2,
};
constexpr int kPlaceSpan = 128;
__host__ __device__ __forceinline__ int place_wg(int p) { return p < kPlaceSpan ? 64 * ((p & 7) >> 2) + 4 * (p >> 3) + (p & 3) : p; }
inline bool place_local_applies(const Program& p, int prior, int post, int grid) {
  if ((p.B + 15) / 16 != 4 || grid < kPlaceSpan) return false;
  if (p.d[prior].wg0 != 0 || p.d[prior].nwg != 64 || p.d[post].wg0 != 64 || p.d[post].nwg != 64) return false;
  for (int i = 0; i < p.ndesc; ++i) {
    const int lo = p.d[i].wg0, hi = lo + p.d[i].nwg;
    const bool kept = (lo == 0 && (hi == 64 || hi == kPlaceSpan)) || (lo == 64 && hi == kPlaceSpan) || lo >= kPlaceSpan;
    if (!kept) return false;
  }
  return true;
}
inline int place_for(int want, int fallback, const Program& p, int prior, int post, int grid) {
  if (want == kPlaceLocal) return place_local_applies(p, prior, post, grid) ? kPlaceLocal : (fallback == kPlacePlain ? kPlacePlain : kPlaceProgram);
  return want == kPlacePlain ? kPlacePlain : kPlaceProgram;
}
inline bool place_xcd(int place, const Program& p) { return place == kPlaceProgram && p.xcd != 0; }
inline int grid_of(const Program& p) {
  int g = 0;
  for (int i = 0; i < p.ndesc; ++i) g = std::max(g, p.d[i].wg0 + p.d[i].nwg);
  return g;
}

constexpr int kArmAhead = 4;
constexpr int kArmMax = 24;
constexpr int kArmCandidates = 64;
struct ArmEntry {
  float* base;
  int step, tile, n4, n4_last, nslabs;
};
struct ArmTable {
  ArmEntry e[kArmMax];
  int n;
};
inline ArmEntry arm_t16(float* buf, int width, int rt, int nslabs, bool reversed = false) {
  const int step = rt * 16 * width;
  return ArmEntry{reversed ? buf + (long)(nslabs - 1) * step : buf, reversed ? -step : step, 16 * width, 4 * width, 4 * width, nslabs};
}
inline ArmEntry arm_rm(float* buf, int ld, int B, int nslabs, bool reversed = false) {
  const int step = B * ld, rt = (B + 15) / 16;
  return ArmEntry{reversed ? buf + (long)(nslabs - 1) * step : buf, reversed ? -step : step, 16 * ld, 4 * ld, (B - 16 * (rt - 1)) * ld / 4, nslabs};
}
struct ArmPlan {
  ArmTable tab{};
  struct Region { void* p; size_t bytes; } full[3] = {};
  int nfull = 0;
  void add(const ArmEntry& e) { if (e.base != nullptr && tab.n < kArmMax) tab.e[tab.n++] = e; else if (e.base != nullptr) tab.n = kArmMax + 1; }
  void fill(void* p, size_t bytes) { full[nfull++] = Region{p, bytes}; }
};
__host__ __device__ __forceinline__ void arm_share(const ArmEntry& e, int r, int rt, int k, int log2n, int* first, int* count) {
  const int total = r == rt - 1 ? e.n4_last : e.n4, per = (total + (1 << log2n) - 1) >> log2n;
  *first = k * per < total ? k * per : total;
  *count = per < total - *first ? per : total - *first;
}
inline bool arm_rank(const Program& p, int link, int cand0, int ncand, bool xcd, int w, int* r, int* k, int* n) {
  const int rt = (p.B + 15) / 16;
  const Desc& d = p.d[link];
  TileIter mine(w, d.wg0, d.nwg, rt, d.ct, xcd);
  if (w < cand0 || w >= cand0 + ncand || !mine.valid()) return false;
  *r = mine.r0() / 16; *k = 0; *n = 0;
  for (int c = cand0; c < cand0 + ncand; ++c) {
    TileIter it(c, d.wg0, d.nwg, rt, d.ct, xcd);
    if (!it.valid() || it.r0() != mine.r0()) continue;
    ++*n;
    if (c < w) ++*k;
  }
  return true;
}
inline int arm_operand_slot(int kind) {
  switch (kind) {
    case K_LIN: return LIN_A;
    case K_LINSEQ: return LINSEQ_A0;
    case K_HEAD: return HEAD_P16;
    case K_GRU: return GRU_X16;
    case K_GRUB: return GRUB_D0_16;
    case K_DZ: return DZ_D16;
    default: return -1;
  }
}
inline bool arm_applies(const Program& p, const ArmTable& t, int link, std::initializer_list<int> idle, int cand0, int ncand, bool xcd) {
  const int rt = (p.B + 15) / 16;
  if (t.n <= 0 || t.n > kArmMax || ncand <= 0 || ncand > kArmCandidates || p.S <= kArmAhead || p.rt_group != 1) return false;
  for (int i = 0; i < t.n; ++i) {
    const ArmEntry& e = t.e[i];
    const long span = e.step < 0 ? -(long)e.step : e.step;
    if (e.base == nullptr || (reinterpret_cast<unsigned long long>(e.base) & 15) != 0 || e.step % 4 != 0 || e.tile % 4 != 0) return false;
    if (e.n4 <= 0 || e.n4_last <= 0 || e.n4_last > e.n4 || 4L * e.n4 > e.tile || (long)(rt - 1) * e.tile + 4L * e.n4_last > span) return false;
    if (e.nslabs < p.S - 1 || e.nslabs > p.S + 1) return false;
  }
  for (int i = 0; i < p.ndesc; ++i) {
    const Desc& d = p.d[i];
    const int slot = arm_operand_slot(d.kind);
    if (slot < 0 || d.p[slot] == nullptr || p.stride[d.sidx[slot]] == 0) return false;
    if (d.kind == K_LIN && (d.flags & DF_A_PLAIN) != 0) {
      const Desc& role = p.d[link];
      for (int w = d.wg0; w < d.wg0 + d.nwg; ++w)
        if (TileIter(w, d.wg0, d.nwg, rt, d.ct, xcd).valid() && !TileIter(w, role.wg0, role.nwg, rt, role.ct, xcd).valid()) return false;
      continue;
    }
    bool inside = false;
    for (int k = 0; k < t.n && !inside; ++k) {
      const ArmEntry& e = t.e[k];
      const long span = e.step < 0 ? -(long)e.step : e.step;
      const float* lo = e.step < 0 ? e.base - (long)(e.nslabs - 1) * span : e.base;
      inside = d.p[slot] >= lo && d.p[slot] <= lo + (long)e.nslabs * span;
    }
    if (!inside) return false;
  }
  const Desc& d = p.d[link];
  int armers[4] = {0, 0, 0, 0};
  if (rt > 4) return false;
  for (int w = cand0; w < cand0 + ncand; ++w) {
    int tiles = 0, r = 0;
    for (TileIter it(w, d.wg0, d.nwg, rt, d.ct, xcd); it.valid(); it.next()) { ++tiles; r = it.r0() / 16; }
    if (tiles > 1) return false;
    if (tiles == 1) ++armers[r];
    for (int i : idle)
      if (TileIter(w, p.d[i].wg0, p.d[i].nwg, rt, p.d[i].ct, xcd).valid()) return false;
  }
  for (int r = 0; r < rt; ++r)
    if (armers[r] == 0 || (armers[r] & (armers[r] - 1)) != 0) return false;
  return true;
}

}
}
```

### benchmarking-lvms_amd/csrc/vrnn_static.hip

```cpp
#include <algorithm>
#include <mutex>

#include "common.h"
#include "pchain.h"
#include "vrnn_static.h"

namespace blvm {
namespace {
using namespace pchain;

struct SPtr {
  float* base;
  int stride;
  __device__ __forceinline__ float* at(int s) const { return base + (long)s * stride; }
};

__device__ __forceinline__ int placed_wg(int place) { return place == kPlaceLocal ? place_wg((int)blockIdx.x) : (int)blockIdx.x; }
__device__ __forceinline__ int tile_lanes(int w, int wg0, int nwg, int rt, int ct, bool xcd) {
  TileIter it(w, wg0, nwg, rt, ct, xcd);
  const int lane = threadIdx.x & 63;
  it.j += lane * it.step;
  return (lane < kMaxTiles && it.valid()) ? (it.r0() | (it.c() << 16)) : -1;
}
__device__ __forceinline__ int tile_count(int lanes) { return __popcll(__ballot(lanes >= 0)); }

constexpr int kAnatBase = 128, kAnatRole = 512, kAnatSlots = 56;
#ifdef PCHAIN_TPROF
__device__ __forceinline__ void anat_begin(unsigned* tab) {
  for (int i = threadIdx.x; i < kAnatSlots * 8; i += blockDim.x) tab[i] = 0u;
  __syncthreads();
}
__device__ __forceinline__ void anat_arm(Poll& pl) { pl.rpolls = 0; pl.t_st = 0; }
__device__ __forceinline__ void anat_note(unsigned* tab, int slot, const Poll& pl) {
  const unsigned long long now = wall_clock64();
  if ((threadIdx.x & 63) == 0 && pl.rpolls != 0) {
    unsigned* q = tab + (slot * 2 + (threadIdx.x < 256 ? 0 : 1)) * 4;
    atomicAdd(q, 1u); atomicAdd(q + 1, pl.rpolls); atomicAdd(q + 2, (unsigned)(pl.t_ok - pl.t_issue));
    atomicAdd(q + 3, (unsigned)((pl.t_st != 0 ? pl.t_st : now) - pl.t_ok));
  }
}
__device__ __forceinline__ void anat_end(const unsigned* tab, unsigned long long* prof, int role, bool chosen) {
  __syncthreads();
  if (prof != nullptr && chosen)
    for (int i = threadIdx.x; i < kAnatSlots * 8; i += blockDim.x) prof[kAnatBase + role * kAnatRole + i] = tab[i];
}
#define ANAT(x) x
#else
#define ANAT(x)
#endif

struct LinChainArgs {
  SPtr a16, orm, o16;
  const float *W, *bias;
  int ldo, n16, B, s0, S, wg0, nwg, ct, xcd, place;
  Ctl ctl;
  int pace_early, pace_epi;
  ANAT(unsigned long long* prof;)
};
template <class PC>
__device__ __forceinline__ PC chain_pace(const LinChainArgs& a) {
  if constexpr (PC::paced) return PC{a.pace_early, a.pace_epi};
  else return PC();
}

template <int NW, int K, bool RES, class PC = PaceOff>
__global__ __launch_bounds__(NW * 64, 1) void static_lin_chain_kernel(LinChainArgs a) {
  __shared__ __attribute__((aligned(16))) float red[2][NW * 256];
  ANAT(__shared__ unsigned anat[kAnatSlots * 8]; anat_begin(anat);)
  const int w = placed_wg(a.place), B = a.B;
  const int tiles = tile_lanes(w, a.wg0, a.nwg, (B + 15) / 16, a.ct, a.place == kPlaceProgram && a.xcd != 0);
  const int nt = tile_count(tiles);
  if (nt == 0) return;
  Poll pl{a.ctl, 0u, false, 1};
  int par = 0;
  if constexpr (RES) {
    const int trc = __builtin_amdgcn_readlane(tiles, 0), r0 = trc & 0xffff, c0 = (trc >> 16) * 16;
    WRegs<OP_F32, 1, K / (16 * NW)> ws;
    const float* const Ws[1] = {a.W};
    const int cs[1] = {c0};
    load_w<NW, OP_F32, 1, K / (16 * NW)>(ws.w, Ws, cs, K);
    const PC pace = chain_pace<PC>(a);
    for (int s = a.s0; s < a.S; ++s) {
      pl.code = (unsigned)s << 4;
      auto late = [&]() { return LinLate{a.bias, nullptr, nullptr, 0, 0, false, true, 0.f, Out{a.orm.at(s), a.ldo, false, a.o16.at(s), a.n16}}; };
      ANAT(anat_arm(pl);)
      tile_lin_late<NW, OP_F32>(a.a16.at(s), 0, true, a.W, K, late, r0, c0, B, red[par], pl, nullptr, nullptr, 0, ws, pace);
      ANAT(anat_note(anat, 0, pl);)
      par ^= 1;
    }
    ANAT(anat_end(anat, a.prof, 0, w == a.wg0);)
    return;
  }
  for (int s = a.s0; s < a.S; ++s) {
    pl.code = (unsigned)s << 4;
    const float* A = a.a16.at(s);
    auto late = [&]() { return LinLate{a.bias, nullptr, nullptr, 0, 0, false, true, 0.f, Out{a.orm.at(s), a.ldo, false, a.o16.at(s), a.n16}}; };
    for (int tk = 0; tk < nt; ++tk) {
      const int trc = __builtin_amdgcn_readlane(tiles, tk);
      tile_lin_late<NW, false>(A, 0, true, a.W, K, late, trc & 0xffff, (trc >> 16) * 16, B, red[par], pl);
      par ^= 1;
    }
  }
}

constexpr int kH = 256, kR = 512;

struct LinArgs {
  SPtr a, a2, a3, add, gate, orm, o16, o16b;
  const float *W, *bias;
  int ld0, ld1, ld2, ld3, n16, n16b, w_width;
  float slope;
};
struct SeqArgs {
  SPtr a0, add0, aux[4], orm[4], o16[4];
  const float* W[4];
  int ld[4], ldadd0, ldgate, n16;
  float slope;
};
struct HeadArgs {
  SPtr P, Q, eps, mu_p, sd_p, mu_q, sd_q, raw_p, raw_q, muq_raw, z, z16, z16b;
  const float *Wp, *bp, *Wq, *bq;
  int ld3, n16, n16b, Z, residual;
  float beta, inv_beta, sd_eps;
};
struct GruArgs {
  SPtr X, xg, gh, hprev, hrm, h16, h16b, rg, ug, ng;
  const float *Wih, *bih;
  int ld0, ld3, n16, n16b, R;
};
struct DzArgs {
  SPtr D, add, mu_q, sd_q, mu_p, sd_p, eps, raw_q, raw_p, muq_raw, dqh, dqh16, dph, dph16;
  const float *WT, *c_raw, *c_fn;
  const int32_t* x_sl;
  int ld1, ld3, n16, Z, residual, stride, t0, first_gemm;
  float fn_floor, beta, sd_eps;
};
struct GrubArgs {
  SPtr D0, D1, g_in, rg, ug, ng, gh, hprev, dd, dgi, dgi16, dgh, dgh16, ga, g_add;
  const float *W0, *W1, *g_out;
  int ld0, ld1, ld3, n16, R, first_gemm, end_gates, first_gin;
};
struct Deal {
  int wg0, nwg, ct, s_begin, s_end, idx;
};

struct Walk {
  float* red0;
  float* red1;
  int par, B;
  Poll pl;
  ANAT(unsigned* anat;)
  __device__ __forceinline__ float* red() { par ^= 1; return par ? red0 : red1; }
  __device__ __forceinline__ void at(const Deal& d, int s, bool gentle, unsigned li = 0) {
    pl.nap = gentle ? 16 : 1;
    pl.code = ((unsigned)s << 4) | (unsigned)d.idx | (li << 28);
  }
};

template <int K, int G = 1>
using Res = WRegs<OP_F32, G, K / 256>;
template <int N, int K0, int K>
struct RunRes {
  Res<K0> first;
  Res<K> rest[N - 1];
};
__device__ __forceinline__ int tile_c0(int tiles) { return (__builtin_amdgcn_readlane(tiles, 0) >> 16) * 16; }

template <int NW, int K>
__device__ __forceinline__ void load_lin(Res<K>& r, const float* W, int ldw, int tiles, int nt) {
  if (nt == 0) return;
  const float* const Ws[1] = {W};
  const int cs[1] = {tile_c0(tiles)};
  load_w<NW, OP_F32, 1, K / 256>(r.w, Ws, cs, ldw > 0 ? ldw : K);
}
template <int NW, int N, int K0, int K>
__device__ __forceinline__ void load_run(RunRes<N, K0, K>& r, const SeqArgs& q, int tiles, int nt) {
  load_lin<NW, K0>(r.first, q.W[0], K0, tiles, nt);
#pragma unroll
  for (int li = 1; li < N; ++li) load_lin<NW, K>(r.rest[li - 1], q.W[li], K, tiles, nt);
// ... 127 lines not shown

template <int NW, class PC = PaceOff>
__device__ __forceinline__ void visit_grub(const GrubArgs& q, const Deal& d, int s, int tiles, int nt, Walk& wk, const Res<kH, 2>& ws) {
  if (nt == 0 || s < d.s_begin || s >= d.s_end) return;
  wk.at(d, s, false);
  GrubIn g;
  g.D0 = q.D0.at(s); g.D1 = q.D1.at(s); g.W0 = q.W0; g.W1 = q.W1; g.g_in = q.g_in.at(s); g.g_add = q.g_add.at(s); g.ld_gadd = q.ld1;
  g.rg = q.rg.at(s); g.ug = q.ug.at(s); g.ng = q.ng.at(s); g.gh = q.gh.at(s); g.hprev = q.hprev.at(s); g.dd = q.dd.at(s); g.ldh = q.ld0;
  g.dgi = Out{q.dgi.at(s), q.ld3, false, q.dgi16.at(s), q.n16};
  g.dgh = Out{q.dgh.at(s), q.ld3, false, q.dgh16.at(s), q.n16};
  g.ga = q.ga.at(s); g.g_out = const_cast<float*>(q.g_out);
  g.has_gemm = s >= q.first_gemm; g.has_gates = s < q.end_gates; g.has_gin = s >= q.first_gin;
  const int trc = __builtin_amdgcn_readlane(tiles, 0);
  ANAT(anat_arm(wk.pl);)
  tile_grub<NW, OP_F32>(g, kH, q.R, trc & 0xffff, (trc >> 16) * 16, wk.B, wk.red(), wk.pl, ws, PC());
  ANAT(anat_note(wk.anat, 4 * d.idx, wk.pl);)
}

struct Armer {
  int r, k, log2n;
};
__device__ __forceinline__ Armer arm_rank_dev(int w, const Deal& link, int cand0, int ncand, int rt, bool xcd, int tiles, int nt, int entries) {
  if (entries == 0 || nt != 1 || w < cand0 || w >= cand0 + ncand) return Armer{0, 0, -1};
  const int lane = threadIdx.x & 63, my_r0 = __builtin_amdgcn_readlane(tiles, 0) & 0xffff;
  const TileIter it(cand0 + lane, link.wg0, link.nwg, rt, link.ct, xcd);
  const unsigned long long same = __ballot(lane < ncand && it.valid() && it.r0() == my_r0);
  const int n = (int)__popcll(same);
  return Armer{my_r0 >> 4, (int)__popcll(same & ((1ull << (w - cand0)) - 1ull)), __builtin_ctz((unsigned)n)};
}
template <int NW>
__device__ __forceinline__ void arm_ahead(const ArmTable& t, int j, int rt, const Armer& a) {
  if (a.log2n < 0) return;
  const int lane = threadIdx.x & 63, wave = __builtin_amdgcn_readfirstlane((int)(threadIdx.x >> 6));
  const u32x4 ff = {SENTINEL, SENTINEL, SENTINEL, SENTINEL};
  for (int e = wave; e < t.n; e += NW) {
    const ArmEntry& en = t.e[e];
    if (j >= en.nslabs) continue;
    int first, count;
    arm_share(en, a.r, rt, a.k, a.log2n, &first, &count);
    const rsrc_t dst = make_rsrc(en.base + (long)j * en.step + (long)a.r * en.tile + 4L * first);
    for (int i = lane; i < count; i += 64) __builtin_amdgcn_raw_buffer_store_b128(ff, dst, 16 * i, 0, PCHAIN_STORE_AUX);
  }
  asm volatile("s_waitcnt vmcnt(0)" ::: "memory");
}

template <class A>
__device__ __forceinline__ const A& kargs() {
  typedef const __attribute__((address_space(4))) char kchar;
  kchar* p = (kchar*)__builtin_amdgcn_kernarg_segment_ptr();
  asm volatile("" : "+s"(p));
  return *(const A*)p;
}

struct FwdArgs {
  LinArgs hproj;
  SeqArgs run[2];
  HeadArgs head;
  SeqArgs phi;
  GruArgs gru;
  LinArgs dec[4];
  Deal deal[kFwdDecDesc];
  int ndec;
  int B, s0, S, xcd, place;
  Ctl ctl;
  ArmTable arm;
  ANAT(unsigned long long* prof;)
};
constexpr int kFwdProducts = 4, kBwdProducts = 2;

template <int NW, int HALF>
__device__ __forceinline__ void fwd_half(const FwdArgs& a, int w, int rt, bool xcd, Walk& wk) {
  const int t1 = tile_lanes(w, a.deal[1 + HALF].wg0, a.deal[1 + HALF].nwg, rt, a.deal[1 + HALF].ct, xcd), n1 = tile_count(t1);
  const int t3 = tile_lanes(w, a.deal[3].wg0, a.deal[3].nwg, rt, a.deal[3].ct, xcd), n3 = tile_count(t3);
  const int t4 = tile_lanes(w, a.deal[4].wg0, a.deal[4].nwg, rt, a.deal[4].ct, xcd), n4 = tile_count(t4);
  const int t5 = tile_lanes(w, a.deal[5].wg0, a.deal[5].nwg, rt, a.deal[5].ct, xcd), n5 = tile_count(t5);
  RunRes<3, kR, kH> run;
  Res<kH, 4> head;
  RunRes<4, kH, kH> phi;
  Res<kH, 3> gru;
  load_run<NW>(run, kargs<FwdArgs>().run[HALF], t1, n1);
  load_head<NW>(head, kargs<FwdArgs>().head, t3, n3);
  load_run<NW>(phi, kargs<FwdArgs>().phi, t4, n4);
  load_gru<NW>(gru, kargs<FwdArgs>().gru, t5, n5);
  for (int s = a.s0; s < a.S; ++s) {
    visit_run<NW, 3, kR, kH, false, Paced>(kargs<FwdArgs>().run[HALF], kargs<FwdArgs>().deal[1 + HALF], s, t1, n1, wk, run);
    visit_head<NW, Paced>(kargs<FwdArgs>().head, kargs<FwdArgs>().deal[3], s, t3, n3, wk, head);
    visit_run<NW, 4, kH, kH, false, Paced>(kargs<FwdArgs>().phi, kargs<FwdArgs>().deal[4], s, t4, n4, wk, phi);
    if constexpr (HALF == 0) visit_gru<NW, Paced>(kargs<FwdArgs>().gru, kargs<FwdArgs>().deal[5], s, t5, n5, wk, gru);
    else visit_gru<NW>(kargs<FwdArgs>().gru, kargs<FwdArgs>().deal[5], s, t5, n5, wk, gru);
  }
  ANAT(anat_end(wk.anat, kargs<FwdArgs>().prof, HALF, w == kargs<FwdArgs>().deal[1 + HALF].wg0);)
}

template <int NW>
__device__ __forceinline__ void fwd_post_arming(const FwdArgs& a, int w, int rt, bool xcd, Walk& wk) {
  const int t1 = tile_lanes(w, a.deal[2].wg0, a.deal[2].nwg, rt, a.deal[2].ct, xcd), n1 = tile_count(t1);
  const int t5 = tile_lanes(w, a.deal[5].wg0, a.deal[5].nwg, rt, a.deal[5].ct, xcd), n5 = tile_count(t5);
  const Armer armer = arm_rank_dev(w, a.deal[5], a.deal[2].wg0, a.deal[0].wg0 - a.deal[2].wg0, rt, xcd, t5, n5, a.arm.n);
  RunRes<3, kR, kH> run;
  Res<kH, 3> gru;
  load_run<NW>(run, kargs<FwdArgs>().run[1], t1, n1);
  load_gru<NW>(gru, kargs<FwdArgs>().gru, t5, n5);
  for (int s = a.s0; s < a.S; ++s) {
    visit_run<NW, 3, kR, kH, false, Paced>(kargs<FwdArgs>().run[1], kargs<FwdArgs>().deal[2], s, t1, n1, wk, run);
    arm_ahead<NW>(kargs<FwdArgs>().arm, s + kArmAhead, rt, armer);
    visit_gru<NW>(kargs<FwdArgs>().gru, kargs<FwdArgs>().deal[5], s, t5, n5, wk, gru);
  }
  ANAT(anat_end(wk.anat, kargs<FwdArgs>().prof, 1, w == kargs<FwdArgs>().deal[2].wg0);)
}

constexpr int kDecFlags = DF_RELU | DF_GENTLE | DF_CANARY;
template <int NW>
__device__ __forceinline__ void fwd_dec(const FwdArgs& a, int w, int rt, bool xcd, Walk& wk) {
  const int t6 = tile_lanes(w, a.deal[6].wg0, a.deal[6].nwg, rt, a.deal[6].ct, xcd), n6 = tile_count(t6);
  const int t7 = tile_lanes(w, a.deal[7].wg0, a.deal[7].nwg, rt, a.deal[7].ct, xcd), n7 = tile_count(t7);
  const int t8 = tile_lanes(w, a.deal[8].wg0, a.deal[8].nwg, rt, a.deal[8].ct, xcd), n8 = tile_count(t8);
  const int t9 = tile_lanes(w, a.deal[9].wg0, a.deal[9].nwg, rt, a.deal[9].ct, xcd), n9 = tile_count(t9);
  if ((n6 | n7 | n8 | n9) == 0) return;
  Res<kR> w1h;
  Res<kH> w1p, w2;
  load_lin<NW, kR>(w1h, kargs<FwdArgs>().dec[0].W, kargs<FwdArgs>().dec[0].w_width, t6, n6);
  load_lin<NW, kH>(w1p, kargs<FwdArgs>().dec[1].W, kargs<FwdArgs>().dec[1].w_width, t7, n7);
  load_lin<NW, kH>(w2, kargs<FwdArgs>().dec[2].W, kH, t8, n8);
  for (int s = a.s0; s < a.S; ++s) {
    visit_lin<NW, kR, DF_RM_SC1 | DF_GENTLE | DF_CANARY>(kargs<FwdArgs>().dec[0], kargs<FwdArgs>().deal[6], s, t6, n6, wk, w1h);
    visit_lin<NW, kH, DF_ADD_POLLED | kDecFlags>(kargs<FwdArgs>().dec[1], kargs<FwdArgs>().deal[7], s, t7, n7, wk, w1p);
    visit_lin<NW, kH, kDecFlags>(kargs<FwdArgs>().dec[2], kargs<FwdArgs>().deal[8], s, t8, n8, wk, w2);
    visit_lin<NW, kH, kDecFlags, PaceOff, true>(kargs<FwdArgs>().dec[3], kargs<FwdArgs>().deal[9], s, t9, n9, wk, WMem());
  }
}

template <int NW>
__global__ __launch_bounds__(NW * 64, 1) void vrnn_static_fwd_kernel(FwdArgs a) {
  extern __shared__ __attribute__((aligned(16))) float lds_red[];
  const int w = placed_wg(a.place), rt = (a.B + 15) / 16;
  const bool xcd = a.place == kPlaceProgram && a.xcd != 0;
  Walk wk{lds_red, lds_red + kFwdProducts * NW * 256, 0, a.B, Poll{a.ctl, 0u, false, 1}};
  ANAT(__shared__ unsigned anat[kAnatSlots * 8]; anat_begin(anat); wk.anat = anat;)
  if (a.ndec != 0 && w >= a.deal[6].wg0) {
    fwd_dec<NW>(a, w, rt, xcd, wk);
    return;
  }
  if (w >= a.deal[0].wg0) {
    const int t0 = tile_lanes(w, a.deal[0].wg0, a.deal[0].nwg, rt, a.deal[0].ct, xcd), n0 = tile_count(t0);
    if (n0 == 0) return;
    for (int s = a.s0; s < a.S; ++s) visit_lin<NW, kR, DF_RM_SC1 | DF_GENTLE | DF_CANARY>(kargs<FwdArgs>().hproj, kargs<FwdArgs>().deal[0], s, t0, n0, wk, WMem());
    return;
  }
  if (w < a.deal[2].wg0) fwd_half<NW, 0>(a, w, rt, xcd, wk);
  else if (a.arm.n != 0) fwd_post_arming<NW>(a, w, rt, xcd, wk);
  else fwd_half<NW, 1>(a, w, rt, xcd, wk);
}

struct BwdArgs {
  GrubArgs grub;
  LinArgs part[3], gb, sum;
  SeqArgs phi;
  DzArgs dz;
  SeqArgs run[2];
  LinArgs bdec[3];
  Deal deal[kBwdDecDesc];
  int nbdec;
  int bdec_k, gb_ldadd2;
  SPtr gb_add2;
  int B, s0, S, xcd, place;
  Ctl ctl;
  ArmTable arm;
  ANAT(unsigned long long* prof;)
};

static_assert(sizeof(BwdArgs) <= 4096 && sizeof(FwdArgs) <= 4096, "kernel argument size");

template <int NW, int HALF>
__device__ __forceinline__ void bwd_half(const BwdArgs& a, int w, int rt, bool xcd, Walk& wk) {
  const int t0 = tile_lanes(w, a.deal[0].wg0, a.deal[0].nwg, rt, a.deal[0].ct, xcd), n0 = tile_count(t0);
  const int t1 = tile_lanes(w, a.deal[1 + HALF].wg0, a.deal[1 + HALF].nwg, rt, a.deal[1 + HALF].ct, xcd), n1 = tile_count(t1);
  const int t5 = tile_lanes(w, a.deal[5].wg0, a.deal[5].nwg, rt, a.deal[5].ct, xcd), n5 = tile_count(t5);
  const int t6 = tile_lanes(w, a.deal[6].wg0, a.deal[6].nwg, rt, a.deal[6].ct, xcd), n6 = tile_count(t6);
  const int t7 = tile_lanes(w, a.deal[7].wg0, a.deal[7].nwg, rt, a.deal[7].ct, xcd), n7 = tile_count(t7);
  const int t8 = tile_lanes(w, a.deal[8 + HALF].wg0, a.deal[8 + HALF].nwg, rt, a.deal[8 + HALF].ct, xcd), n8 = tile_count(t8);
  Res<kH, 2> grub;
  Res<kR> part;
  Res<kH> sum, dz;
  RunRes<2, kH, kH> phi;
  RunRes<3, 2 * kH, kH> run;
  load_grub<NW>(grub, kargs<BwdArgs>().grub, t0, n0);
  load_lin<NW, kR>(part, kargs<BwdArgs>().part[HALF].W, kargs<BwdArgs>().part[HALF].w_width, t1, n1);
  load_lin<NW, kH>(sum, kargs<BwdArgs>().sum.W, kH, t5, n5);
  load_run<NW>(phi, kargs<BwdArgs>().phi, t6, n6);
  load_lin<NW, kH>(dz, kargs<BwdArgs>().dz.WT, kH, t7, n7);
  load_run<NW>(run, kargs<BwdArgs>().run[HALF], t8, n8);
  for (int s = a.s0; s < a.S; ++s) {
    visit_grub<NW, Paced>(kargs<BwdArgs>().grub, kargs<BwdArgs>().deal[0], s, t0, n0, wk, grub);
    visit_lin<NW, kR, 0, Paced>(kargs<BwdArgs>().part[HALF], kargs<BwdArgs>().deal[1 + HALF], s, t1, n1, wk, part);
    visit_lin<NW, kH, DF_A_SUM3, Paced>(kargs<BwdArgs>().sum, kargs<BwdArgs>().deal[5], s, t5, n5, wk, sum);
    visit_run<NW, 2, kH, kH, true, Paced>(kargs<BwdArgs>().phi, kargs<BwdArgs>().deal[6], s, t6, n6, wk, phi);
    visit_dz<NW, Paced>(kargs<BwdArgs>().dz, kargs<BwdArgs>().deal[7], s, t7, n7, wk, dz);
    if constexpr (HALF == 0) visit_run<NW, 3, 2 * kH, kH, true, Paced>(kargs<BwdArgs>().run[HALF], kargs<BwdArgs>().deal[8 + HALF], s, t8, n8, wk, run);
    else visit_run<NW, 3, 2 * kH, kH, true>(kargs<BwdArgs>().run[HALF], kargs<BwdArgs>().deal[8 + HALF], s, t8, n8, wk, run);
  }
  ANAT(anat_end(wk.anat, kargs<BwdArgs>().prof, 2 + HALF, w == kargs<BwdArgs>().deal[1 + HALF].wg0);)
}

constexpr int kGbFlags = DF_ADD_POLLED | DF_RM_SC1 | DF_GENTLE | DF_CANARY;
constexpr int kPartLeadFlags = DF_ADD_POLLED | DF_ADD_EARLY;
constexpr int kBdec0Flags = DF_A_PLAIN | DF_GENTLE, kBdec1Flags = DF_GENTLE | DF_CANARY, kBdec2Flags = DF_RM_SC1 | DF_GENTLE | DF_CANARY;
template <int NW>
__device__ __forceinline__ void bwd_spare_leader(const BwdArgs& a, int w, int rt, bool xcd, Walk& wk) {
  const int t = tile_lanes(w, a.deal[3].wg0, a.deal[3].nwg, rt, a.deal[3].ct, xcd), n = tile_count(t);
  const int t10 = tile_lanes(w, a.deal[10].wg0, a.deal[10].nwg, rt, a.deal[10].ct, xcd), n10 = tile_count(t10);
  const int t11 = tile_lanes(w, a.deal[11].wg0, a.deal[11].nwg, rt, a.deal[11].ct, xcd), n11 = tile_count(t11);
  const int t12 = tile_lanes(w, a.deal[12].wg0, a.deal[12].nwg, rt, a.deal[12].ct, xcd), n12 = tile_count(t12);
  if ((n | n10 | n11 | n12) == 0) return;
  Res<kR> part;
  Res<kH> w2;
  load_lin<NW, kR>(part, kargs<BwdArgs>().part[2].W, kargs<BwdArgs>().part[2].w_width, t, n);
  load_lin<NW, kH>(w2, kargs<BwdArgs>().bdec[1].W, kH, t11, n11);
  const Armer armer = arm_rank_dev(w, a.deal[3], a.deal[3].wg0, a.deal[3].nwg, rt, xcd, t, n, a.arm.n);
#ifdef PCHAIN_TPROF
  unsigned long long lead = 0, arming = 0;
  const unsigned long long tb = wall_clock64();
#endif
  for (int s = a.s0; s < a.S; ++s) {
    visit_lin<NW, kR, kPartLeadFlags>(kargs<BwdArgs>().part[2], kargs<BwdArgs>().deal[3], s, t, n, wk, part);
    ANAT(const unsigned long long t0 = wall_clock64();)
    visit_lin<NW, 0, kBdec0Flags>(kargs<BwdArgs>().bdec[0], kargs<BwdArgs>().deal[10], s, t10, n10, wk, WMem(), kargs<BwdArgs>().bdec_k);
    visit_lin<NW, kH, kBdec1Flags>(kargs<BwdArgs>().bdec[1], kargs<BwdArgs>().deal[11], s, t11, n11, wk, w2);
    visit_lin<NW, kH, kBdec2Flags, PaceOff, true>(kargs<BwdArgs>().bdec[2], kargs<BwdArgs>().deal[12], s, t12, n12, wk, WMem());
    ANAT(const unsigned long long t1 = wall_clock64();)
    arm_ahead<NW>(kargs<BwdArgs>().arm, s + kArmAhead, rt, armer);
    ANAT(const unsigned long long t2 = wall_clock64(); lead += t1 - t0; arming += t2 - t1;)
  }
#ifdef PCHAIN_TPROF
  const unsigned long long whole = wall_clock64() - tb;
  if (threadIdx.x == 0) {
    unsigned* q = wk.anat + 13 * 2 * 4;
    q[0] = (unsigned)(a.S - a.s0); q[2] = (unsigned)lead; q[3] = (unsigned)arming;
    q[8] = 1u; q[10] = (unsigned)whole;
  }
  anat_end(wk.anat, kargs<BwdArgs>().prof, 4, w == kargs<BwdArgs>().deal[3].wg0);
#endif
}

template <int NW>
__global__ __launch_bounds__(NW * 64, 1) void vrnn_static_bwd_kernel(BwdArgs a) {
  extern __shared__ __attribute__((aligned(16))) float lds_red[];
  const int w = placed_wg(a.place), rt = (a.B + 15) / 16;
  const bool xcd = a.place == kPlaceProgram && a.xcd != 0;
  Walk wk{lds_red, lds_red + kBwdProducts * NW * 256, 0, a.B, Poll{a.ctl, 0u, false, 1}};
  ANAT(__shared__ unsigned anat[kAnatSlots * 8]; anat_begin(anat); wk.anat = anat;)
  if (a.nbdec != 0 && w >= a.deal[3].wg0) {
    bwd_spare_leader<NW>(a, w, rt, xcd, wk);
    return;
  }
  if (w >= a.deal[3].wg0) {
    const int t = tile_lanes(w, a.deal[3].wg0, a.deal[3].nwg, rt, a.deal[3].ct, xcd), n = tile_count(t);
    if (n == 0) return;
    Res<kR> part;
    load_lin<NW, kR>(part, kargs<BwdArgs>().part[2].W, kargs<BwdArgs>().part[2].w_width, t, n);
    const Armer armer = arm_rank_dev(w, a.deal[3], a.deal[3].wg0, a.deal[3].nwg, rt, xcd, t, n, a.arm.n);
    for (int s = a.s0; s < a.S; ++s) {
      visit_lin<NW, kR, 0>(kargs<BwdArgs>().part[2], kargs<BwdArgs>().deal[3], s, t, n, wk, part);
      arm_ahead<NW>(kargs<BwdArgs>().arm, s + kArmAhead, rt, armer);
    }
    ANAT(anat_end(wk.anat, kargs<BwdArgs>().prof, 4, w == kargs<BwdArgs>().deal[3].wg0);)
    return;
  }
  if (w >= a.deal[4].wg0) {
    const int t = tile_lanes(w, a.deal[4].wg0, a.deal[4].nwg, rt, a.deal[4].ct, xcd), n = tile_count(t);
    if (n == 0) return;
    if (a.nbdec != 0) {
      for (int s = a.s0; s < a.S; ++s)
        visit_lin<NW, 3 * kR, kGbFlags | DF_ADD2_POLLED>(kargs<BwdArgs>().gb, kargs<BwdArgs>().deal[4], s, t, n, wk, WMem(), 0, kargs<BwdArgs>().gb_add2,
                                                         kargs<BwdArgs>().gb_ldadd2);
      return;
    }
    for (int s = a.s0; s < a.S; ++s)
      visit_lin<NW, 3 * kR, kGbFlags>(kargs<BwdArgs>().gb, kargs<BwdArgs>().deal[4], s, t, n, wk, WMem());
    return;
  }
  if (w < a.deal[2].wg0) bwd_half<NW, 0>(a, w, rt, xcd, wk);
  else bwd_half<NW, 1>(a, w, rt, xcd, wk);
}

int static_place_fallback() { return (pchain_tune() & 32) ? kPlacePlain : kPlaceProgram; }
int static_place_wanted() { return (pchain_tune() & 64) ? kPlaceLocal : static_place_fallback(); }

bool int_strides(const Program& p) {
  for (long v : p.stride)
    if (v < -2147483647L || v > 2147483647L) return false;
  return true;
}
SPtr sptr(const Program& p, const Desc& d, int k) { return SPtr{const_cast<float*>(d.p[k]), (int)p.stride[d.sidx[k]]}; }

template <class Kern>
int static_go(Kern kernel, int slot, int grid, size_t lds, const char* what) {
  static std::mutex mu;
  static int attr_dev[3] = {-1, -1, -1}, occ[3] = {0, 0, 0};
  int dev = 0, cus = 0;
  BLVM_HIP(hipGetDevice(&dev));
  BLVM_HIP(hipDeviceGetAttribute(&cus, hipDeviceAttributeMultiprocessorCount, dev));
  {
    std::lock_guard<std::mutex> lock(mu);
    if (attr_dev[slot] != dev) {
      BLVM_HIP(hipFuncSetAttribute(reinterpret_cast<const void*>(kernel), hipFuncAttributeMaxDynamicSharedMemorySize, (int)lds));
      BLVM_HIP(hipOccupancyMaxActiveBlocksPerMultiprocessor(&occ[slot], kernel, 1024, lds));
      attr_dev[slot] = dev;
    }
    BLVM_REQUIRE((long)occ[slot] * cus >= grid, "%s: %d workgroups are not co-resident (%d per CU x %d CUs)", what, grid, occ[slot], cus);
  }
  return BLVM_OK;
}

int static_lin_chain_launch(const Program& p, hipStream_t stream, bool resident, bool pace = false, int early = 0, int epi = 0) {
  if (p.ndesc != 1 || p.ot != OP_F32 || p.rt_group != 1 || !int_strides(p)) return 1;
  const Desc& d = p.d[0];
  if (d.kind != K_LIN || d.flags != DF_RELU || d.f[LIN_F_SLOPE] != 0.f || (d.K != 256 && d.K != 512) || d.s_begin != 0 || d.s_end != p.S) return 1;
  if (d.ld[LIN_LD_A] != 0 || d.i[LIN_I_W_WIDTH] != 0 || d.p[LIN_ADD] || d.p[LIN_GATE] || d.p[LIN_O16B] || d.p[LIN_A2] || d.p[LIN_A3] || d.n16[N16_OUTB] != 0)
    return 1;
  const int rt = (p.B + 15) / 16;
  int place = resident ? static_place_wanted() : kPlaceProgram;
  if (place == kPlaceLocal && !(rt == 4 && d.wg0 == 0 && (d.nwg == 64 || d.nwg == kPlaceSpan) && device_cus() >= kPlaceSpan)) place = static_place_fallback();
  const bool xcd = place == kPlaceProgram && p.xcd != 0;
  if (d.nwg <= 0 || (p.xcd && d.nwg % 8 != 0) || tiles_per_workgroup(rt, d.ct, d.nwg, xcd) > (resident ? 1 : kMaxTiles)) return 1;
  LinChainArgs a{sptr(p, d, LIN_A), sptr(p, d, LIN_ORM), sptr(p, d, LIN_O16), d.p[LIN_W], d.p[LIN_BIAS], d.ld[LD_OUT], d.n16[N16_OUT], p.B, p.s_first, p.S,
                 d.wg0, d.nwg, d.ct, p.xcd, place, p.ctl, early, epi};
  ANAT(a.prof = pchain_profile_buffer();)
  const int grid = place == kPlaceLocal ? kPlaceSpan : d.wg0 + d.nwg;
  auto go = [&](auto kernel) -> int {
    BLVM_TRY(static_go(kernel, 2, grid, 0, "static_lin_chain"));
    hipLaunchKernelGGL(kernel, dim3(grid), dim3(1024), 0, stream, a);
    BLVM_CHECK_LAUNCH("static_lin_chain");
    return BLVM_OK;
  };
  if (resident && pace) return d.K == 256 ? go(&static_lin_chain_kernel<16, 256, true, PaceRt>) : go(&static_lin_chain_kernel<16, 512, true, PaceRt>);
  if (resident) return d.K == 256 ? go(&static_lin_chain_kernel<16, 256, true>) : go(&static_lin_chain_kernel<16, 512, true>);
  return d.K == 256 ? go(&static_lin_chain_kernel<16, 256, false>) : go(&static_lin_chain_kernel<16, 512, false>);
}

int g_static = 1;
long g_static_launches = 0;
long g_armed_launches = 0;
bool pchain_static_on() { return g_static != 0; }

SPtr sp(const Program& p, const Desc& d, int k) { return SPtr{const_cast<float*>(d.p[k]), d.p[k] ? (int)p.stride[d.sidx[k]] : 0}; }
Deal deal_of(const Desc& d, int idx) { return Deal{d.wg0, d.nwg, d.ct, d.s_begin, d.s_end, idx}; }
bool within(const Desc& d, int lo, int hi) { return d.wg0 >= lo && d.wg0 + d.nwg <= hi; }
bool few_tiles(const Program& p, const Desc& d, bool xcd) {
  if (d.nwg <= 0 || (p.xcd && d.nwg % 8 != 0)) return false;
  return tiles_per_workgroup((p.B + 15) / 16, d.ct, d.nwg, xcd) <= kMaxTiles;
}
bool shaped(const Desc& d, int kind, int flags, int K) { return d.kind == kind && d.flags == flags && d.K == K; }
bool run(const Desc& d, int n, int K0) { return d.i[LINSEQ_I_N] == n && d.i[LINSEQ_I_K0] == K0; }

LinArgs lin_args(const Program& p, const Desc& d) {
  return LinArgs{sp(p, d, LIN_A), sp(p, d, LIN_A2), sp(p, d, LIN_A3), sp(p, d, LIN_ADD), sp(p, d, LIN_GATE), sp(p, d, LIN_ORM), sp(p, d, LIN_O16),
                 sp(p, d, LIN_O16B), d.p[LIN_W], d.p[LIN_BIAS], d.ld[LIN_LD_A], d.ld[LIN_LD_ADD], d.ld[LIN_LD_GATE], d.ld[LD_OUT], d.n16[N16_OUT], d.n16[N16_OUTB],
                 d.i[LIN_I_W_WIDTH], d.f[LIN_F_SLOPE]};
}
SeqArgs seq_args(const Program& p, const Desc& d) {
  SeqArgs q{};
  q.a0 = sp(p, d, LINSEQ_A0); q.add0 = sp(p, d, LINSEQ_ADD0);
  for (int i = 0; i < d.i[LINSEQ_I_N]; ++i) {
    q.W[i] = d.p[LINSEQ_W + i]; q.aux[i] = sp(p, d, LINSEQ_AUX + i); q.orm[i] = sp(p, d, LINSEQ_ORM + i); q.o16[i] = sp(p, d, LINSEQ_O16 + i);
    q.ld[i] = d.ld[LINSEQ_LD_ORM + i];
  }
  q.ldadd0 = d.i[LINSEQ_I_LD_ADD0]; q.ldgate = d.i[LINSEQ_I_LD_GATE]; q.n16 = d.n16[N16_OUT]; q.slope = d.f[LINSEQ_F_SLOPE];
  return q;
}

__global__ __launch_bounds__(256) void arm_prefix_kernel(ArmTable t, int rt) {
  const ArmEntry& en = t.e[blockIdx.y];
  const uint4 ff = make_uint4(SENTINEL, SENTINEL, SENTINEL, SENTINEL);
  const int slabs = en.nslabs < kArmAhead ? en.nslabs : kArmAhead;
  for (int j = 0; j < slabs; ++j)
    for (int r = 0; r < rt; ++r) {
      uint4* const dst = reinterpret_cast<uint4*>(en.base + (long)j * en.step + (long)r * en.tile);
      const int n4 = r == rt - 1 ? en.n4_last : en.n4;
      for (int i = blockIdx.x * 256 + threadIdx.x; i < n4; i += gridDim.x * 256) dst[i] = ff;
    }
}
int full_fill(const ArmPlan& plan, hipStream_t stream) {
  for (int i = 0; i < plan.nfull; ++i) BLVM_HIP(pchain_fill_sentinel(plan.full[i].p, plan.full[i].bytes, stream));
  return BLVM_OK;
}
int arm_or_fill(const Program& p, const ArmPlan& plan, int link, std::initializer_list<int> idle, int cand0, int ncand, bool xcd, hipStream_t stream,
                ArmTable* arm) {
  arm->n = 0;
  if ((pchain_tune() & 128) != 0 || !arm_applies(p, plan.tab, link, idle, cand0, ncand, xcd)) return full_fill(plan, stream);
  *arm = plan.tab;
  hipLaunchKernelGGL(arm_prefix_kernel, dim3(8, plan.tab.n), dim3(256), 0, stream, plan.tab, (p.B + 15) / 16);
  BLVM_CHECK_LAUNCH("arm_prefix");
  return BLVM_OK;
}

int vrnn_static_check(const Program& p, int ndesc, int products, int prior, int post, int* place) {
  if (!pchain_static_on() || p.ndesc != ndesc || p.ot != OP_F32 || p.rt_group != 1 || p.s_first != 0 || p.B > 64) return 1;
  if (p.lds_products != products || !int_strides(p)) return 1;
  *place = place_for(static_place_wanted(), static_place_fallback(), p, prior, post, grid_of(p));
  for (int i = 0; i < p.ndesc; ++i)
    if (!few_tiles(p, p.d[i], place_xcd(*place, p))) return 1;
  return 0;
}

int vrnn_static_fwd(const Program& p, hipStream_t stream, const ArmPlan& plan, const std::function<int()>& pre) {
  int place = kPlaceProgram;
  const bool dec = p.ndesc == kFwdDecDesc || p.ndesc == kFwdDecDesc - 1;
  if (vrnn_static_check(p, dec ? p.ndesc : kFwdDesc, kFwdProducts, 1, 2, &place)) return 1;
  const Desc* d = p.d;
  const int S = p.S;
  for (int i = 0; i < p.ndesc; ++i)
    if (d[i].s_begin != 0 || d[i].s_end != S) return 1;
  if (!shaped(d[0], K_LIN, DF_RM_SC1 | DF_GENTLE | DF_CANARY, kR) || !shaped(d[1], K_LINSEQ, DF_RELU, kH) || !shaped(d[2], K_LINSEQ, DF_RELU, kH) ||
      !shaped(d[3], K_HEAD, 0, kH) || !shaped(d[4], K_LINSEQ, DF_RELU, kH) || !shaped(d[5], K_GRU, 0, kH))
    return 1;
  if (!run(d[1], 3, kR) || !run(d[2], 3, kR) || !run(d[4], 4, 0)) return 1;
  if (!one_tile_each(p, kFwdResident, place_xcd(place, p))) return 1;
  const int half = d[2].wg0, gentle = d[0].wg0;
  if (d[1].wg0 != 0 || !within(d[1], 0, half) || !within(d[2], half, gentle) || d[0].nwg <= 0) return 1;
  if (dec && !within(d[0], gentle, d[6].wg0)) return 1;
  for (int i = 3; i < 6; ++i)
    if (!within(d[i], 0, gentle)) return 1;
  if (dec) {
    const int from = gentle + d[0].nwg;
    if (!shaped(d[6], K_LIN, DF_RM_SC1 | DF_GENTLE | DF_CANARY, kR) || !shaped(d[7], K_LIN, DF_ADD_POLLED | kDecFlags, kH) ||
        !shaped(d[8], K_LIN, kDecFlags, kH) || (p.ndesc == kFwdDecDesc && !shaped(d[9], K_LIN, kDecFlags, kH)))
      return 1;
    for (int i = 6; i < p.ndesc; ++i) {
      if (d[i].wg0 != from || d[i].ld[LIN_LD_A] != 0 || d[i].p[LIN_A2] || d[i].p[LIN_A3] || d[i].p[LIN_O16B] || d[i].p[LIN_GATE]) return 1;
      if (d[i].i[LIN_I_W_WIDTH] != (i < 8 ? kH + kR : 0)) return 1;
    }
    if (!one_tile_each(p, kFwdDecResident, place_xcd(place, p))) return 1;
  }
  FwdArgs a{};
  a.hproj = lin_args(p, d[0]);
  a.run[0] = seq_args(p, d[1]); a.run[1] = seq_args(p, d[2]); a.phi = seq_args(p, d[4]);
  const Desc &h = d[3], &g = d[5];
  a.head = HeadArgs{sp(p, h, HEAD_P16), sp(p, h, HEAD_Q16), sp(p, h, HEAD_EPS), sp(p, h, HEAD_MU_P), sp(p, h, HEAD_SD_P), sp(p, h, HEAD_MU_Q),
                    sp(p, h, HEAD_SD_Q), sp(p, h, HEAD_RAW_P), sp(p, h, HEAD_RAW_Q), sp(p, h, HEAD_MUQ_RAW), sp(p, h, HEAD_Z), sp(p, h, HEAD_Z16),
                    sp(p, h, HEAD_Z16B), h.p[HEAD_WP], h.p[HEAD_BP], h.p[HEAD_WQ], h.p[HEAD_BQ], h.ld[LD_OUT], h.n16[N16_OUT], h.n16[N16_OUTB],
                    h.i[HEAD_I_Z], h.i[HEAD_I_RESIDUAL], h.f[HEAD_F_BETA], h.f[HEAD_F_INV_BETA], h.f[HEAD_F_SD_EPS]};
  a.gru = GruArgs{sp(p, g, GRU_X16), sp(p, g, GRU_XG), sp(p, g, GRU_GH), sp(p, g, GRU_HPREV), sp(p, g, GRU_HRM), sp(p, g, GRU_H16), sp(p, g, GRU_H16B),
                  sp(p, g, GRU_RG), sp(p, g, GRU_UG), sp(p, g, GRU_NG), g.p[GRU_WIH], g.p[GRU_BIH], g.ld[GRU_LD_HPREV], g.ld[LD_OUT], g.n16[N16_OUT],
                  g.n16[N16_OUTB], g.i[GRU_I_R]};
  a.ndec = dec ? p.ndesc - kFwdDesc : 0;
  for (int k = 0; k < a.ndec; ++k) a.dec[k] = lin_args(p, d[6 + k]);
  int grid = 0;
  for (int i = 0; i < p.ndesc; ++i) { a.deal[i] = deal_of(d[i], i); grid = std::max(grid, d[i].wg0 + d[i].nwg); }
  a.B = p.B; a.s0 = p.s_first; a.S = S; a.xcd = p.xcd; a.place = place; a.ctl = p.ctl;
  ANAT(a.prof = pchain_profile_buffer();)
  BLVM_TRY(arm_or_fill(p, plan, 5, {3, 4}, half, gentle - half, place_xcd(place, p), stream, &a.arm));
  BLVM_TRY(pre());
  const size_t lds = sizeof(float) * 2 * kFwdProducts * 16 * 256;
  BLVM_TRY(static_go(&vrnn_static_fwd_kernel<16>, 0, grid, lds, "vrnn_static_fwd"));
  hipLaunchKernelGGL(vrnn_static_fwd_kernel<16>, dim3(grid), dim3(1024), lds, stream, a);
  BLVM_CHECK_LAUNCH("vrnn_static_fwd");
  ++g_static_launches;
  if (a.arm.n != 0) ++g_armed_launches;
  return BLVM_OK;
}

int vrnn_static_bwd(const Program& p, hipStream_t stream, const ArmPlan& plan, const std::function<int()>& pre) {
  int place = kPlaceProgram;
  const bool lead = p.ndesc == kBwdDecDesc;
  if (vrnn_static_check(p, lead ? kBwdDecDesc : kBwdDesc, kBwdProducts, 8, 9, &place)) return 1;
  const Desc* d = p.d;
  const int S = p.S;
  for (int i = 0; i < kBwdDesc; ++i)
    if (d[i].s_begin != 0 || d[i].s_end != (i == 0 ? S : S - 1)) return 1;
  if (!shaped(d[0], K_GRUB, 0, kH) || !shaped(d[1], K_LIN, 0, kR) || !shaped(d[2], K_LIN, 0, kR) || !shaped(d[3], K_LIN, lead ? kPartLeadFlags : 0, kR) ||
      !shaped(d[4], K_LIN, lead ? kGbFlags | DF_ADD2_POLLED : kGbFlags, 3 * kR) || !shaped(d[5], K_LIN, DF_A_SUM3, kH) ||
      !shaped(d[6], K_LINSEQ, DF_SEQ_GATE, kH) || !shaped(d[7], K_DZ, 0, kH) || !shaped(d[8], K_LINSEQ, DF_SEQ_GATE, kH) ||
      !shaped(d[9], K_LINSEQ, DF_SEQ_GATE, kH))
    return 1;
  if (!run(d[6], 2, 0) || !run(d[8], 3, 2 * kH) || !run(d[9], 3, 2 * kH)) return 1;
  if (!one_tile_each(p, kBwdResident, place_xcd(place, p)) || d[7].p[DZ_D2_16] != nullptr) return 1;
  const int half = d[2].wg0, gentle = d[4].wg0, spare = d[3].wg0;
  if (!within(d[1], 0, half) || !within(d[8], 0, half) || !within(d[2], half, gentle) || !within(d[9], half, gentle) || !within(d[4], gentle, spare) ||
      d[3].nwg <= 0)
    return 1;
  for (int i : {0, 5, 6, 7})
    if (!within(d[i], 0, gentle)) return 1;
  if (lead) {
    for (int i = kBwdDesc; i < kBwdDecDesc; ++i) {
      if (d[i].s_begin != 0 || d[i].s_end != S - 1 - kBdecAhead || d[i].wg0 != spare || d[i].nwg != d[3].nwg) return 1;
      if (d[i].p[LIN_A2] || d[i].p[LIN_A3] || d[i].p[LIN_O16B] || d[i].p[LIN_ADD] || d[i].p[LIN_ADD2] || d[i].p[LIN_BIAS] || d[i].i[LIN_I_W_WIDTH] != 0) return 1;
    }
    if (d[10].kind != K_LIN || d[10].flags != kBdec0Flags || d[10].K <= 0 || d[10].K % 16 != 0 || d[10].ld[LIN_LD_A] != d[10].K) return 1;
    if (!shaped(d[11], K_LIN, kBdec1Flags, kH) || !shaped(d[12], K_LIN, kBdec2Flags, kH) || d[11].ld[LIN_LD_A] != 0 || d[12].ld[LIN_LD_A] != 0) return 1;
    if (!one_tile_each(p, kBwdDecResident, place_xcd(place, p))) return 1;
    if (d[3].p[LIN_ADD] == nullptr || d[4].p[LIN_ADD2] == nullptr || d[1].p[LIN_ADD] != nullptr || d[0].p[GRUB_DD] != nullptr) return 1;
  }
  BwdArgs a{};
  const Desc& g = d[0];
  a.grub = GrubArgs{sp(p, g, GRUB_D0_16), sp(p, g, GRUB_D1_16), sp(p, g, GRUB_G_IN), sp(p, g, GRUB_RG), sp(p, g, GRUB_UG), sp(p, g, GRUB_NG), sp(p, g, GRUB_GH),
                    sp(p, g, GRUB_HPREV), sp(p, g, GRUB_DD), sp(p, g, GRUB_DGI), sp(p, g, GRUB_DGI16), sp(p, g, GRUB_DGH), sp(p, g, GRUB_DGH16), sp(p, g, GRUB_GA),
                    sp(p, g, GRUB_G_ADD), g.p[GRUB_W0], g.p[GRUB_W1], g.p[GRUB_G_OUT], g.ld[GRUB_LD_H], g.ld[GRUB_LD_GADD], g.ld[LD_OUT], g.n16[N16_OUT],
                    g.i[GRUB_I_R], g.i[GRUB_I_GEMM_FROM], g.i[GRUB_I_GATES_TO], g.i[GRUB_I_GIN_FROM]};
  for (int k = 0; k < 3; ++k) a.part[k] = lin_args(p, d[1 + k]);
  a.gb = lin_args(p, d[4]); a.sum = lin_args(p, d[5]);
  a.phi = seq_args(p, d[6]); a.run[0] = seq_args(p, d[8]); a.run[1] = seq_args(p, d[9]);
  const Desc& z = d[7];
  a.dz = DzArgs{sp(p, z, DZ_D16), sp(p, z, DZ_ADD), sp(p, z, DZ_MU_Q), sp(p, z, DZ_SD_Q), sp(p, z, DZ_MU_P), sp(p, z, DZ_SD_P),
                sp(p, z, DZ_EPS), sp(p, z, DZ_RAW_Q), sp(p, z, DZ_RAW_P), sp(p, z, DZ_MUQ_RAW), sp(p, z, DZ_DQH), sp(p, z, DZ_DQH16), sp(p, z, DZ_DPH),
                sp(p, z, DZ_DPH16), z.p[DZ_WT], z.p[DZ_C_RAW], z.p[DZ_C_FN], reinterpret_cast<const int32_t*>(z.p[DZ_X_SL]), z.ld[DZ_LD_ADD],
                z.ld[LD_OUT], z.n16[N16_OUT], z.i[DZ_I_Z], z.i[DZ_I_RESIDUAL], z.i[DZ_I_STRIDE], z.i[DZ_I_T0], (int)z.f[DZ_F_GEMM_FROM], z.f[DZ_F_FN_FLOOR],
                z.f[DZ_F_BETA], z.f[DZ_F_SD_EPS]};
  a.nbdec = lead ? 3 : 0;
  if (lead) { a.bdec_k = d[kBwdDesc].K; a.gb_add2 = sp(p, d[4], LIN_ADD2); a.gb_ldadd2 = d[4].i[LIN_I_LD_ADD2]; }
  for (int k = 0; k < a.nbdec; ++k) a.bdec[k] = lin_args(p, d[kBwdDesc + k]);
  int grid = 0;
  for (int i = 0; i < p.ndesc; ++i) { a.deal[i] = deal_of(d[i], i); grid = std::max(grid, d[i].wg0 + d[i].nwg); }
  a.B = p.B; a.s0 = p.s_first; a.S = S; a.xcd = p.xcd; a.place = place; a.ctl = p.ctl;
  ANAT(a.prof = pchain_profile_buffer();)
  BLVM_TRY(arm_or_fill(p, plan, 3, {}, spare, d[3].nwg, place_xcd(place, p), stream, &a.arm));
  BLVM_TRY(pre());
  const size_t lds = sizeof(float) * 2 * kBwdProducts * 16 * 256;
  BLVM_TRY(static_go(&vrnn_static_bwd_kernel<16>, 1, grid, lds, "vrnn_static_bwd"));
  hipLaunchKernelGGL(vrnn_static_bwd_kernel<16>, dim3(grid), dim3(1024), lds, stream, a);
  BLVM_CHECK_LAUNCH("vrnn_static_bwd");
  ++g_static_launches;
  if (a.arm.n != 0) ++g_armed_launches;
  return BLVM_OK;
}

}

int vrnn_launch(pchain::Builder& bld, bool forward, const char* who, hipStream_t stream, const pchain::ArmPlan& plan, const std::function<int()>& pre) {
  BLVM_TRY(pchain_prepare(bld, who));
  const int rc = forward ? vrnn_static_fwd(bld.p, stream, plan, pre) : vrnn_static_bwd(bld.p, stream, plan, pre);
  if (rc != 1) return rc;
  BLVM_TRY(full_fill(plan, stream));
  BLVM_TRY(pre());
  return pchain_run(bld.p, stream);
}

}

extern "C" int blvm_pchain_static(int mode) {
  if (mode == -2) return (int)std::min<long>(blvm::g_static_launches, 0x7fffffffL);
  if (mode == -3) return (int)std::min<long>(blvm::g_armed_launches, 0x7fffffffL);
  const int was = blvm::g_static;
  if (mode >= 0) blvm::g_static = mode != 0;
  return was;
}

static int static_chain_probe(const float* W16, const float* bias, float* x16, float* xs, int B, int N, int L, int nwg, void* stream_, bool resident,
                              bool pace = false, int early = 0, int epi = 0) {
  using namespace blvm;
  using namespace blvm::pchain;
  hipStream_t s = static_cast<hipStream_t>(stream_);
  BLVM_REQUIRE(W16 && bias && x16 && xs && B > 0 && N > 0 && N % 16 == 0 && L > 0, "pchain_static_chain_probe: bad arguments");
  const int rt = (B + 15) / 16;
  const long x = (long)rt * 16 * N, sN = (long)B * N;
  Builder bld;
  bld.begin(OP_F32, L, B, 1, false, 0);
  const int nw = nwg > 0 ? nwg : range_for((N / 16) * rt, device_cus() & ~7);
  Operands o;
  o.p[LIN_A] = {x16, x}; o.p[LIN_W] = W16; o.p[LIN_BIAS] = bias; o.p[LIN_ORM] = {xs, sN}; o.p[LIN_O16] = {x16 + x, x}; o.ld[LD_OUT] = N; o.n16[N16_OUT] = N / 16;
  add_desc(bld, K_LIN, N / 16, 0, nw, N, DF_RELU, 0, L, o);
  BLVM_HIP(pchain_fill_sentinel(x16 + x, sizeof(float) * (size_t)x * L, s));
  BLVM_TRY(pchain_prepare(bld, "pchain_static_chain_probe"));
  const int rc = static_lin_chain_launch(bld.p, s, resident, pace, early, epi);
  BLVM_REQUIRE(rc != 1, "pchain_static_chain_probe: no static kernel for N = %d (256, 512) or this deal", N);
  return rc;
}
extern "C" int blvm_pchain_static_chain_probe(const float* W16, const float* bias, float* x16, float* xs, int B, int N, int L, int nwg, void* stream) {
  return static_chain_probe(W16, bias, x16, xs, B, N, L, nwg, stream, true);
}
extern "C" int blvm_pchain_static_chain_probe_fetch(const float* W16, const float* bias, float* x16, float* xs, int B, int N, int L, int nwg, void* stream) {
  return static_chain_probe(W16, bias, x16, xs, B, N, L, nwg, stream, false);
}
extern "C" int blvm_pchain_static_chain_probe_paced(const float* W16, const float* bias, float* x16, float* xs, int B, int N, int L, int nwg,
                                                    int early_delay, int epi_delay, void* stream) {
  using namespace blvm;
  BLVM_REQUIRE(early_delay >= 0 && early_delay <= 64 && epi_delay >= 0 && epi_delay <= 64,
               "pchain_static_chain_probe_paced: delays are 0 .. 64 s_sleep units");
  return static_chain_probe(W16, bias, x16, xs, B, N, L, nwg, stream, true, (early_delay | epi_delay) != 0, early_delay, epi_delay);
}
```

### include/blvm_hip.h

```cpp
#ifndef BLVM_HIP_H
#define BLVM_HIP_H

#include <stddef.h>
#include <stdint.h>

#ifdef __cplusplus
extern "C" {
#endif

#define BLVM_OK 0
#define BLVM_EINVAL (-1)
#define BLVM_ELAUNCH (-2)
#define BLVM_ENOSUP (-3)
#define BLVM_NOT_APPLICABLE 1

int blvm_version(void);
const char* blvm_last_error(void);
int blvm_device_ok(void);
int blvm_async_errors(unsigned* last_code);
int blvm_async_errors_take(unsigned* last_code);
int blvm_pchain_configure(int max_batch, int waves);
int blvm_pchain_max_batch(void);
#define BLVM_DTYPE_F32 0
#define BLVM_DTYPE_BF16 1
// ... 32 lines not shown
#define BLVM_GEMM_ARMS 17
int blvm_gemm_arm(int op_a, int op_b, int M, int N, int K, size_t a_addr, int lda, size_t b_addr, int ldb, int split_k, int has_bias,
                  int act, int has_gate, int has_colsum, int operand, int min_rows);
int blvm_wgrad_group_route(int n, const int* N_out, const int* K_in, int rows, const size_t* d_addr, const int* ldd, const size_t* x_addr,
                           const int* ldx, const int* has_dw, int operand, int* joins);
int blvm_gemm_arm_counts(unsigned long long out[17]);

int blvm_act_bwd_f32(const float* dy, const float* y, float slope, float* dz, size_t n, void* stream);

int blvm_wgrad_f32(int N_out, int K_in, int rows, const float* D, int ldd, const float* X, int ldx, float* dW, int lddw, float* db,
                   int split_k, void* stream);

int blvm_wgrad_group_f32(int n, const int* N_out, const int* K_in, int rows, const float* const* D, const int* ldd, const float* const* X,
                         const int* ldx, float* const* dW, const int* lddw, float* const* db, void* stream);

int blvm_colsum_f32(int M, int N, const float* X, int ldx, float* out, int accumulate, void* stream);

int blvm_dmol_fwd(const float* dec, int layout, const float* W, const float* bias, const float* y,
                  const int32_t* x_sl, int B, int T, int Tp, int S, int num_mix, int num_bins, float log_eps,
                  double* log_prob, float* ll_twise, void* stream);

int blvm_dmol_bwd(const float* dec, int layout, const float* W, const float* bias, const float* y,
                  const int32_t* x_sl, const float* g_b, int B, int T, int Tp, int S, int num_mix, int num_bins,
                  float log_eps, float* d_dec, float* d_par, void* stream);

size_t blvm_dmol_bwd_fused_workspace_floats(int B, int Tp, int S);
int blvm_dmol_bwd_fused(const float* dec, int layout, const float* W, const float* bias, const float* y,
                        const int32_t* x_sl, const float* g_b, int B, int T, int Tp, int S, int num_mix, int num_bins,
                        float log_eps, float act_slope, float* dz, float* dW, float* db, float* workspace, void* stream);

int blvm_gmm_fwd(const float* dec, int layout, const float* W, const float* bias, const float* y, const int32_t* x_sl,
                 int B, int T, int Tp, int S, int num_mix, float sd_beta, float sd_eps, double* log_prob, float* ll_twise,
                 void* stream);
int blvm_gmm_bwd(const float* dec, int layout, const float* W, const float* bias, const float* y, const int32_t* x_sl,
                 const float* g_b, int B, int T, int Tp, int S, int num_mix, float sd_beta, float sd_eps, float* d_dec,
                 float* d_par, void* stream);
int blvm_gauss_head_fwd(const float* dec, int layout, const float* W, const float* bias, const float* y,
                        const int32_t* x_sl, int B, int T, int Tp, int S, float sd_beta, float sd_eps, double* log_prob,
                        float* ll_twise, void* stream);
int blvm_gauss_head_bwd(const float* dec, int layout, const float* W, const float* bias, const float* y,
                        const int32_t* x_sl, const float* g_b, int B, int T, int Tp, int S, float sd_beta, float sd_eps,
                        float* d_dec, float* d_par, void* stream);

int blvm_mix_sample(const float* par, const float* u, const float* v, long long n, int num_mix, int kind, float log_eps,
                    float sd_beta, float sd_eps, float* out, void* stream);

int blvm_cat_fwd(const float* dec, const float* W, const float* bias, const int32_t* y, const int32_t* x_sl, int B, int T, int Tp, int S,
                 int C, int V, float* lse, float* ll, double* log_prob, void* stream);

size_t blvm_cat_bwd_workspace_floats(long long frames, int C, int V);
int blvm_cat_bwd(const float* dec, const float* W, const float* bias, const int32_t* y, const int32_t* x_sl, const float* lse,
                 const float* g_b, int B, int T, int Tp, int S, int C, int V, float* d_dec, float* dW, float* db, float* workspace,
                 void* stream);

int blvm_cat_sample(const float* logits, const float* u, long long n, int V, int32_t* out, void* stream);

int blvm_kl_fwd(const float* mu_q, const float* sd_q, const float* mu_p, const float* sd_p, int layout,
                const int32_t* x_sl, int B, int Tp, int Z, int stride, float fn_floor, double* kld,
                double* kld_fn, void* stream);

int blvm_kl_bwd(const float* mu_q, const float* sd_q, const float* mu_p, const float* sd_p, int layout,
                const int32_t* x_sl, const float* c_raw, const float* c_fn, int B, int Tp, int Z, int stride,
                float fn_floor, float* d_mu_q, float* d_sd_q, float* d_mu_p, float* d_sd_p, void* stream);

int blvm_elbo_fwd(const double* log_prob, const double* kld, const double* kld_fn, double beta, double n_frames, int B,
                  int kl_raw, double* elbo, double* loss, double* sums, void* stream);
int blvm_elbo_bwd(const double* g_loss, const double* g_elbo, double beta, double n_frames, int B, double* g64, float* g32,
                  void* stream);

int blvm_gauss_latent_fwd(const float* mu_p, const float* sd_p_raw, const float* mu_q_raw, const float* sd_q_raw,
                          const float* eps, size_t n, float beta_p, float beta_q, float sd_eps, int mode, float* sd_p,
                          float* mu_q, float* sd_q, float* z, void* stream);
int blvm_gauss_latent_bwd(const float* mu_p, const float* sd_p_raw, const float* mu_q_raw, const float* sd_q_raw,
                          const float* eps, const float* g_sd_p, const float* g_mu_q, const float* g_sd_q, const float* g_z,
                          size_t n, float beta_p, float beta_q, float sd_eps, int mode, float* d_mu_p, float* d_sd_p_raw,
                          float* d_mu_q_raw, float* d_sd_q_raw, void* stream);

typedef struct BlvmVrnnWeights {
  const float *prior_w[3], *prior_b[3];
  const float *prior_hw, *prior_hb;
  const float *post_w[3], *post_b[3];
  const float *post_hw, *post_hb;
  const float *phi_w[4], *phi_b[4];
  const float *gru_wih, *gru_whh;
  const float *gru_bih, *gru_bhh;
} BlvmVrnnWeights;

typedef struct BlvmVrnnGrads {
  float *prior_w[3], *prior_b[3], *prior_hw, *prior_hb;
  float *post_w[3], *post_b[3], *post_hw, *post_hb;
  float *phi_w[4], *phi_b[4];
  float *gru_wih, *gru_whh, *gru_bih, *gru_bhh;
} BlvmVrnnGrads;

typedef struct BlvmVrnnDecodeWeights {
  const float *enc_w[3], *enc_b[3];
  const BlvmVrnnWeights* cell;
  const float *dec_w[3], *dec_b[3];
  const float *lik_w, *lik_b;
} BlvmVrnnDecodeWeights;
size_t blvm_vrnn_decode_scratch_floats(int S, int H, int Z, int R);
int blvm_vrnn_decode(const BlvmVrnnDecodeWeights* w, const float* x0, const float* h0, const float* eps, const float* u,
                     const float* v, int T, int B, int S, int H, int Z, int R, int num_mix, float sd_eps, float slope,
                     float log_eps, float* x_out, float* h_out, float* scratch, void* stream);

size_t blvm_vrnn_generate_scratch_floats(int T, int B, int S, int H, int Z, int R);
int blvm_vrnn_generate(const BlvmVrnnDecodeWeights* w, const float* x0, const float* h0, const float* eps, const float* u,
                       const float* v, int T, int B, int S, int H, int Z, int R, int num_mix, float sd_eps, float slope,
                       float log_eps, float* x_out, float* h_out, float* scratch, void* stream);

size_t blvm_vrnn_generate_scratch_floats_head(int T, int B, int S, int H, int Z, int R, int head_kind);
int blvm_vrnn_decode_applies(int S, int H, int Z, int R);
int blvm_vrnn_generate_head(const BlvmVrnnDecodeWeights* w, const float* x0, const float* h0, const float* eps, const float* u,
                            const float* v, int T, int B, int S, int H, int Z, int R, int head_kind, int num_mix, float log_eps,
                            float head_sd_beta, float head_sd_eps, float sd_eps, float slope, float* x_out, float* h_out,
                            float* scratch, void* stream);
int blvm_vrnn_decode_head(const BlvmVrnnDecodeWeights* w, const float* x0, const float* h0, const float* eps, const float* u,
                          const float* v, int T, int B, int S, int H, int Z, int R, int head_kind, int num_mix, float log_eps,
                          float head_sd_beta, float head_sd_eps, float sd_eps, float slope, float* x_out, float* h_out,
                          float* scratch, void* stream);

size_t blvm_vrnn_reserve_floats(int Tp, int B, int X, int H, int Z, int R);
size_t blvm_vrnn_bwd_workspace_floats(int Tp, int B, int X, int H, int Z, int R);

int blvm_vrnn_seq_fwd(const BlvmVrnnWeights* w, const float* enc, const float* h0, const float* eps, int Tp, int B,
                      int X, int H, int Z, int R, int residual_posterior, float sd_eps, float* decin,
                      float* mu_q, float* sd_q, float* mu_p, float* sd_p, float* z, float* reserve, void* stream);

size_t blvm_vrnn_fwd_reserve_floats(int Tp, int B, int X, int H, int Z, int R, int DH, int SF);
int blvm_vrnn_seq_fwd_dec(const BlvmVrnnWeights* w, const float* enc, const float* h0, const float* eps, int Tp, int B,
                          int X, int H, int Z, int R, int residual_posterior, float sd_eps, float* decin,
                          float* mu_q, float* sd_q, float* mu_p, float* sd_p, float* z, float* reserve,
                          const float* const* dec_w, const float* const* dec_b, float* const* dec_y, int DH, int SF, float slope,
                          int* folded, void* stream);
int blvm_vrnn_dec_fold(int mode);

int blvm_vrnn_seq_bwd(const BlvmVrnnWeights* w, const float* enc, const float* eps, const float* decin,
                      const float* mu_q, const float* sd_q, const float* mu_p, const float* sd_p, const float* z,
                      const float* reserve, const float* d_decin, const int32_t* x_sl, const float* c_raw,
                      const float* c_fn, int stride, float fn_floor, int Tp, int B, int X, int H, int Z, int R,
                      int residual_posterior, float sd_eps, float* d_enc, float* d_h0, const BlvmVrnnGrads* grads,
                      float* workspace, void* stream);

size_t blvm_vrnn_bwd_dec_workspace_floats(int Tp, int B, int X, int H, int Z, int R, int DH, int SF);
int blvm_vrnn_seq_bwd_dec(const BlvmVrnnWeights* w, const float* enc, const float* eps, const float* decin,
                          const float* mu_q, const float* sd_q, const float* mu_p, const float* sd_p, const float* z,
                          const float* reserve, const int32_t* x_sl, const float* c_raw, const float* c_fn, int stride,
                          float fn_floor, int Tp, int B, int X, int H, int Z, int R, int residual_posterior, float sd_eps,
                          float* d_enc, float* d_h0, const BlvmVrnnGrads* grads, float* workspace, const float* dz3,
                          const float* dec_y1, const float* dec_y2, const float* const* dec_w, float* dy2, float* dy1, int DH,
                          int SF, float slope, int* folded, void* stream);
int blvm_vrnn_dec_bwd_fold(int mode);

size_t blvm_lstm_reserve_floats(int T, int B, int H);
size_t blvm_lstm_bwd_workspace_floats(int T, int B, int H);
int blvm_lstm_seq_fwd(const float* Wih, const float* Whh, const float* bih, const float* bhh, const float* in,
                      const float* h0, const float* c0, const int32_t* lens, int T, int B, int I, int H, float* out,
                      float* hn, float* cn, float* reserve, void* stream);
int blvm_lstm_seq_bwd(const float* Wih, const float* Whh, const float* in, const float* reserve, const float* d_out,
                      int T, int B, int I, int H, float* d_in, float* d_h0, float* d_c0, float* dWih, float* dWhh,
                      float* dbih, float* dbhh, float* workspace, void* stream);

size_t blvm_lstm_bidir_reserve_floats(int T, int B, int H);
size_t blvm_lstm_bidir_bwd_workspace_floats(int T, int B, int H);
int blvm_lstm_bidir_fwd(const float* Wih_f, const float* Whh_f, const float* bih_f, const float* bhh_f,
                        const float* Wih_r, const float* Whh_r, const float* bih_r, const float* bhh_r, const float* in,
                        const int32_t* lens, int T, int B, int I, int H, float* out, float* reserve, void* stream);
int blvm_lstm_bidir_bwd(const float* Wih_f, const float* Whh_f, const float* Wih_r, const float* Whh_r, const float* in,
                        const int32_t* lens, const float* reserve, const float* d_out, int T, int B, int I, int H,
                        float* d_in, float* dWih_f, float* dWhh_f, float* dbih_f, float* dbhh_f, float* dWih_r,
                        float* dWhh_r, float* dbih_r, float* dbhh_r, float* workspace, void* stream);
int blvm_lstm_bidir_applies(int T, int B, int H);
int blvm_lstm_bidir_path_counts(unsigned long long out[2]);

size_t blvm_gru_reserve_floats(int T, int B, int R);
size_t blvm_gru_bwd_workspace_floats(int T, int B, int R);
int blvm_gru_seq_fwd(const float* Wih, const float* Whh, const float* bih, const float* bhh, const float* in,
                     int ld_in, const float* h0, const int32_t* lens, int reverse, int T, int B, int I, int R,
                     float* out, long long out_ts, int out_ld, float* hn, float* reserve, void* stream);
int blvm_gru_seq_bwd(const float* Wih, const float* Whh, const float* in, int ld_in, const int32_t* lens, int reverse,
                     const float* reserve, const float* d_out, long long out_ts, int out_ld, int T, int B, int I,
                     int R, float* d_in, int ld_din, int accumulate_din, float* d_h0, float* dWih, float* dWhh,
                     float* dbih, float* dbhh, float* workspace, void* stream);

typedef struct BlvmSrnnWeights {
  const float *prior_w[3], *prior_b[3];
  const float *prior_hw, *prior_hb;
  const float *post_w[3], *post_b[3];
  const float *post_hw, *post_hb;
} BlvmSrnnWeights;

typedef struct BlvmSrnnGrads {
  float *prior_w[3], *prior_b[3], *prior_hw, *prior_hb;
  float *post_w[3], *post_b[3], *post_hw, *post_hb;
} BlvmSrnnGrads;

size_t blvm_srnn_reserve_floats(int Tp, int B, int H, int Z, int R);
size_t blvm_srnn_bwd_workspace_floats(int Tp, int B, int H, int Z, int R);
int blvm_srnn_latent_fwd(const BlvmSrnnWeights* w, const float* d, const float* a, const float* z0, const float* eps,
                         int Tp, int B, int H, int Z, int R, int residual_posterior, float sd_eps, float slope,
                         float* zs, float* mu_q, float* sd_q, float* mu_p, float* sd_p, float* reserve, void* stream);
int blvm_srnn_latent_bwd(const BlvmSrnnWeights* w, const float* d, const float* a, const float* eps, const float* zs,
                         const float* mu_q, const float* sd_q, const float* mu_p, const float* sd_p,
                         const float* reserve, const float* d_z, const int32_t* x_sl, const float* c_raw,
                         const float* c_fn, int stride, float fn_floor, int Tp, int B, int H, int Z, int R,
                         int residual_posterior, float sd_eps, float slope, float* d_d, float* d_a, float* d_z0,
                         const BlvmSrnnGrads* grads, float* workspace, void* stream);

typedef struct BlvmSrnnDecodeWeights {
  const float *enc_w[3], *enc_b[3];
  const float *gru_wih, *gru_whh, *gru_bih, *gru_bhh;
  const BlvmSrnnWeights* chain;
  const float *dec_w[3], *dec_b[3];
  const float *lik_w, *lik_b;
} BlvmSrnnDecodeWeights;
size_t blvm_srnn_generate_scratch_floats(int T, int B, int S, int H, int Z, int R);
int blvm_srnn_generate(const BlvmSrnnDecodeWeights* w, const float* x0, const float* d0, const float* z0, const float* eps,
                       const float* u, const float* v, int T, int B, int S, int H, int Z, int R, int num_mix, float sd_eps,
                       float slope, float log_eps, float* x_out, float* d_out, float* z_out, float* scratch, void* stream);
size_t blvm_srnn_generate_scratch_floats_head(int T, int B, int S, int H, int Z, int R, int head_kind);
int blvm_srnn_generate_head(const BlvmSrnnDecodeWeights* w, const float* x0, const float* d0, const float* z0, const float* eps,
                            const float* u, const float* v, int T, int B, int S, int H, int Z, int R, int head_kind, int num_mix,
                            float log_eps, float head_sd_beta, float head_sd_eps, float sd_eps, float slope, float* x_out,
                            float* d_out, float* z_out, float* scratch, void* stream);

typedef struct BlvmLstmDecodeWeights {
  const float *emb_w[3], *emb_b[3];
  const float *const *wih, *const *whh, *const *bih, *const *bhh;
  const float *dec_w[3], *dec_b[3];
  const float *lik_w, *lik_b;
} BlvmLstmDecodeWeights;
size_t blvm_lstm_generate_scratch_floats(int T, int B, int S, int H, int num_layers);
int blvm_lstm_generate_any_stack(const BlvmLstmDecodeWeights* w, const float* x0, const float* h0, const float* c0, const float* u,
                                 const float* v, int T, int B, int S, int H, int num_layers, int num_mix, float log_eps, float* x_out,
                                 float* h_out, float* c_out, float* scratch, void* stream);
int blvm_lstm_generate(const BlvmLstmDecodeWeights* w, const float* x0, const float* h0, const float* c0, const float* u,
                       const float* v, int T, int B, int S, int H, int num_layers, int num_mix, float log_eps, float* x_out,
                       float* h_out, float* c_out, float* scratch, void* stream);

int blvm_scale_act_f32(const float* x, float scale, float slope, float* y, size_t n, void* stream);
size_t blvm_conv1d_k2_workspace_floats(int Cin, int Cout);
int blvm_conv1d_k2_fwd(const float* x, const float* W, const float* bias, int L_in, int B, int Cin, int Cout,
                       int dilation, float* out, float* workspace, void* stream);
int blvm_conv1d_k2_bwd(const float* x, const float* W, const float* d_out, int L_in, int B, int Cin, int Cout,
                       int dilation, float* d_x, float* dW, float* db, float* workspace, void* stream);

size_t blvm_wavenet_block_reserve_floats(int L_in, int B, int C, int dilation);
size_t blvm_wavenet_block_workspace_floats(int L_in, int B, int C, int S, int dilation);
int blvm_wavenet_block_fwd(const float* x, const float* conv_w, const float* conv_b, const float* rs_w,
                           const float* rs_b, int L_in, int B, int C, int S, int dilation, int T_skip, float inv_std,
                           float* o, float* skip, float* reserve, float* workspace, void* stream);
int blvm_wavenet_block_bwd(const float* x, const float* conv_w, const float* rs_w, const float* reserve,
                           const float* d_o, const float* d_skip, int L_in, int B, int C, int S, int dilation,
                           int T_skip, float inv_std, float* d_x, float* dconv_w, float* dconv_b, float* drs_w,
                           float* drs_b, float* workspace, void* stream);

int blvm_wavenet_stack_floats(int L, int B, int C, const int* dilations, int n_blocks, size_t* acts_floats, size_t* reserve_floats);
int blvm_wavenet_stack_fwd(const float* x, const float* const* params, const int* dilations, const int* groups, int n_blocks, int L,
                           int B, int C, int S, int T_skip, float inv_std, float* acts, float* const* skips, float* reserve,
                           float* workspace, void* stream);
int blvm_wavenet_stack_bwd(const float* x, const float* const* params, const int* dilations, const int* groups, int n_blocks, int L,
                           int B, int C, int S, int T_skip, float inv_std, const float* acts, const float* reserve,
                           const float* const* d_skips, float* d_x, float* d_scratch, float* const* grads, float* workspace,
                           void* stream);

size_t blvm_wavenet_decode_pack_floats(int C, int S, int O, int n_blocks);
size_t blvm_wavenet_decode_scratch_floats(const int* dilations, int n_blocks, int B, int C, int S);
int blvm_wavenet_decode(const float* packed, const int* dilations, int n_blocks, int B, int C, int S, int O, int num_mix,
                        int n_frames, float inv_std, float skip_scale, float log_eps, const float* u, const float* v,
                        float* scratch, float* x_out, void* stream);

size_t blvm_wavenet_decode_ring_offset_floats(int n_blocks, int C, int S);
int blvm_wavenet_decode_ring_fill(const float* h, int L, int B, int C, int dilation, int t0, float* ring, void* stream);
int blvm_wavenet_decode_resume(const float* packed, const int* dilations, int n_blocks, int B, int C, int S, int O, int num_mix,
                               int n_frames, int t0, float inv_std, float skip_scale, float log_eps, const float* u,
                               const float* v, const float* x_in, float* scratch, float* x_out, float* x_state, void* stream);

size_t blvm_wavenet_cat_decode_pack_floats(int C, int S, int O, int n_blocks, int V);
int blvm_wavenet_cat_decode(const float* packed, const int* dilations, int n_blocks, int B, int C, int S, int O, int V, int n_frames,
                            float inv_std, float skip_scale, const float* levels, const float* u, float* scratch, float* x_out,
                            int32_t* k_out, void* stream);
int blvm_wavenet_cat_decode_resume(const float* packed, const int* dilations, int n_blocks, int B, int C, int S, int O, int V,
                                   int n_frames, int t0, float inv_std, float skip_scale, const float* levels, const float* u,
                                   const float* x_in, float* scratch, float* x_out, int32_t* k_out, float* x_state, void* stream);

int blvm_wavenet_embed_tables(const float* emb, const float* cw, int V, int C, int m, float* P, void* stream);
int blvm_wavenet_embed_fwd(const float* P, const float* bias, const int32_t* k, int L_in, int B, int V, int C, int pad_causal,
                           float* out, void* stream);
size_t blvm_wavenet_embed_bwd_workspace_floats(int n, int V, int C, int m);
int blvm_wavenet_embed_bwd(const float* d_out, const int32_t* sorted_keys, const int32_t* perm, const int32_t* starts, int L_out,
                           int B, int V, int C, int m, const float* emb, const float* cw, float* G, float* workspace, float* d_emb,
                           float* d_cw, float* d_bias, void* stream);

int blvm_wavenet_embed_cat_decode(const float* packed, const float* tables, const int* dilations, int n_blocks, int B, int C, int S,
                                  int O, int V, int n_frames, float inv_std, float skip_scale, const float* levels, const float* u,
                                  float* scratch, float* x_out, int32_t* k_out, void* stream);
int blvm_wavenet_embed_cat_decode_resume(const float* packed, const float* tables, const int* dilations, int n_blocks, int B, int C,
                                         int S, int O, int V, int n_frames, int t0, float inv_std, float skip_scale,
                                         const float* levels, const float* u, const int32_t* k_in, float* scratch, float* x_out,
                                         int32_t* k_out, int32_t* k_state, void* stream);

size_t blvm_stcn_generate_pack_floats(int C, int S, int n_blocks, int n_out, const int* latent, const int* order, int n_latents,
                                      int dense, int num_mix);
size_t blvm_stcn_generate_scratch_floats(const int* dilations, int C, int S, int n_blocks, int n_out, const int* latent,
                                         const int* order, int n_latents, int dense, int num_mix, int B);
int blvm_stcn_generate(const float* packed, const int* dilations, const int* groups, int n_blocks, int n_out, const int* latent,
// ... 79 lines not shown
```

Before: 96.05 million.

## Fold d_enc gradient GEMMs into persistent VRNN backward kernel as lagged followers

The two batched post-loop GEMMs that compute d_enc (from DGI through gru_wih and from DQ through post_w) move into the persistent backward program. They run as two lagged K_LIN follower links on the posterior workgroups, so the encoder gradient is produced while the recurrence is still running. A second kernel instantiation, extra workspace for transposed weights and a partial-product buffer, and validation checks are added. d_enc is also skipped entirely when the input does not need a gradient. The fold applies only to a narrow shape set (H=256, R=512, X=H, B<=64) and adds work to those workgroups, which can lengthen the critical path.

```diff
diff --git a/benchmarking-lvms_amd/blvm/ops.py b/benchmarking-lvms_amd/blvm/ops.py
--- a/benchmarking-lvms_amd/blvm/ops.py
+++ b/benchmarking-lvms_amd/blvm/ops.py
@@ -802,7 +802,7 @@
             dz3, M, DH, SF, slope = _f32c(d_dec), Tp * B, W2.shape[0], W3.shape[0], ctx.dec_slope
             dy2, dy1 = torch.empty(M, DH, **f32), torch.empty(M, DH, **f32)
             grads = _zeros_like_many(params)
-            d_enc = torch.empty_like(enc)
+            d_enc = torch.empty_like(enc) if ctx.needs_input_grad[0] else None
             d_h0 = torch.empty(B, R, **f32) if ctx.has_h0 else None
             w, g = _pack_weights(params), _pack_weights(grads, _hip.VrnnGrads)
             folded = ctypes.c_int(0)
@@ -849,7 +849,7 @@
         params = params[:28]
         d_decin = _f32c(d_decin) if d_decin is not None else torch.zeros_like(decin)
         grads = _zeros_like_many(params)
-        d_enc = torch.empty_like(enc)
+        d_enc = torch.empty_like(enc) if ctx.needs_input_grad[0] else None
         d_h0 = torch.empty(B, R, **f32) if ctx.has_h0 else None
         ws = torch.empty(lib.blvm_vrnn_bwd_workspace_floats(Tp, B, X, H, Z, R), **f32)
         w, g = _pack_weights(params), _pack_weights(grads, _hip.VrnnGrads)
diff --git a/benchmarking-lvms_amd/csrc/vrnn.hip b/benchmarking-lvms_amd/csrc/vrnn.hip
--- a/benchmarking-lvms_amd/csrc/vrnn.hip
+++ b/benchmarking-lvms_amd/csrc/vrnn.hip
@@ -181,10 +181,10 @@
   size_t x16_bytes;
   float *DPHI3b, *DPHI3c;
   float *DY216, *DY116, *DD, *dT[3];
+  float *wixT, *qxT, *EP;
 };
 
-size_t carve_ws(float* base, int Tp, int B, int X, int H, int Z, int R, BwdWs* w, int SF = 0) {
-  (void)X;
+size_t carve_ws(float* base, int Tp, int B, int X, int H, int Z, int R, BwdWs* w, int SF = 0, bool enc = false) {
   const size_t n = (size_t)Tp * B;
   Arena ar{base};
   BwdWs t;
@@ -217,6 +217,8 @@
     t.DPHI3b = ar.take(n * H); t.DPHI3c = ar.take(n * H);
     if (SF > 0) { t.dT[0] = ar.take((size_t)(H + R) * H); t.dT[1] = ar.take((size_t)H * H); t.dT[2] = ar.take((size_t)H * SF); }
   }
+  t.wixT = t.qxT = t.EP = nullptr;
+  if (enc) { t.wixT = ar.take((size_t)3 * R * X); t.qxT = ar.take((size_t)H * X); t.EP = ar.take(n * X); }
   if (w) *w = t;
   return ar.floats();
 }
@@ -271,6 +273,17 @@
   return dl.split3 && dl.bdec[0].nwg > 0;
 }
 
+int g_enc_bwd_fold = [] { const char* e = getenv("BLVM_VRNN_ENC_BWD_FOLD"); return e ? (atoi(e) != 0 ? 1 : 0) : 1; }();
+long g_enc_bwd_folded = 0;
+bool vrnn_enc_bwd_folds(int Tp, int B, int X, int H, int Z, int R) {
+  if (!g_enc_bwd_fold || !vrnn_persistent(B) || device_cus() < 32 || operand_16bit() || pchain_optype(B) != OP_F32) return false;
+  if (B > 64 || vrnn_row_groups(B) || Z != H || X != H || H != 256 || R != 512 || Tp <= pchain::kArmAhead) return false;
+  const int tl = (B + 15) / 16;
+  if (vrnn_shared_deal(false, tl)) return false;
+  const pchain::VrnnBwdDeal dl = pchain::vrnn_bwd_deal(H / 16, Z / 16, R / 16, tl, device_cus() & ~7, false, pchain_split3(), 0, X / 16);
+  return dl.split3 && dl.benc[0].nwg > 0;
+}
+
 enum { VRNN_FWD_PROGRAM = 0, VRNN_FWD_PER_LINK = 1, VRNN_BWD_PROGRAM = 2, VRNN_BWD_PER_LINK = 3, VRNN_ROW_GROUPS = 4, VRNN_LIN16 = 5, VRNN_LIN32 = 6 };
 std::atomic<unsigned long long> g_vrnn_counts[7];
 inline void count_vrnn(int k) { g_vrnn_counts[k].fetch_add(1, std::memory_order_relaxed); }
@@ -311,10 +324,17 @@
 }
 
 extern "C" size_t blvm_vrnn_bwd_workspace_floats(int Tp, int B, int X, int H, int Z, int R) {
-  return carve_ws(nullptr, Tp, B, X, H, Z, R, nullptr);
+  return carve_ws(nullptr, Tp, B, X, H, Z, R, nullptr, 0, vrnn_enc_bwd_folds(Tp, B, X, H, Z, R));
 }
 extern "C" size_t blvm_vrnn_bwd_dec_workspace_floats(int Tp, int B, int X, int H, int Z, int R, int DH, int SF) {
-  return carve_ws(nullptr, Tp, B, X, H, Z, R, nullptr, vrnn_dec_bwd_folds(Tp, B, H, Z, R, DH, SF) ? SF : 0);
+  return carve_ws(nullptr, Tp, B, X, H, Z, R, nullptr, vrnn_dec_bwd_folds(Tp, B, H, Z, R, DH, SF) ? SF : 0,
+                  vrnn_enc_bwd_folds(Tp, B, X, H, Z, R));
+}
+extern "C" int blvm_vrnn_enc_bwd_fold(int mode) {
+  if (mode == -2) return (int)std::min<long>(g_enc_bwd_folded, 0x7fffffffL);
+  const int was = g_enc_bwd_fold;
+  if (mode >= 0) g_enc_bwd_fold = mode != 0;
+  return was;
 }
 extern "C" int blvm_vrnn_dec_bwd_fold(int mode) {
   if (mode == -2) return (int)std::min<long>(g_dec_bwd_folded, 0x7fffffffL);
@@ -553,8 +573,10 @@
   BLVM_REQUIRE(aligned16(workspace) && aligned16(reserve) && aligned16(d_decin), "vrnn_bwd: buffers must be 16-byte aligned");
   Reserve rs;
   carve_reserve(const_cast<float*>(reserve), Tp, B, H, Z, R, &rs);
+  const bool encf = d_enc != nullptr && vrnn_enc_bwd_folds(Tp, B, X, H, Z, R);
+  BLVM_REQUIRE(!encf || aligned16(d_enc), "vrnn_bwd: d_enc must be 16-byte aligned");
   BwdWs ws;
-  carve_ws(workspace, Tp, B, X, H, Z, R, &ws, dec ? dec->SF : 0);
+  carve_ws(workspace, Tp, B, X, H, Z, R, &ws, dec ? dec->SF : 0, encf);
   const size_t n = (size_t)Tp * B;
   const int ldd = H + R;
   const float beta = softplus_beta_of(sd_eps);
@@ -577,6 +599,10 @@
     BLVM_TRY(t16_pack_transposed(dec->w[1], H, H, H, ws.dT[1], s));
     BLVM_TRY(t16_pack_transposed(dec->w[2], H, dec->SF, H, ws.dT[2], s));
   }
+  if (encf) {
+    BLVM_TRY(t16_pack_transposed(w->gru_wih, X + H, 3 * R, X, ws.wixT, s));
+    BLVM_TRY(t16_pack_transposed(w->post_w[0] + R, R + X, H, X, ws.qxT, s));
+  }
   BLVM_TRY(pack_scope.flush());
 
   BLVM_HIP(hipMemsetAsync(ws.G, 0, sizeof(float) * (size_t)B * R, s));
@@ -604,7 +630,7 @@
 
   const float* hprev_all = decin + H;
   auto batched = [&]() -> int {
-    if (d_enc) {
+    if (d_enc && !encf) {
       BLVM_TRY(gemm_f32(0, 1, (int)n, X, H, ws.DQ[0], H, w->post_w[0] + R, R + X, d_enc, X, nullptr, 0, 0.f, nullptr, 0, 0, 1, s));
       BLVM_TRY(gemm_f32(0, 1, (int)n, X, 3 * R, ws.DGI, 3 * R, w->gru_wih, X + H, d_enc, X, nullptr, 0, 0.f, nullptr, 0, 1, 1, s));
     }
@@ -642,8 +668,9 @@
     const int RTG = groups ? vrnn_rt(B) : 1;
     const int tl = (rt + RTG - 1) / RTG;
     const bool shared = vrnn_shared_deal(groups, tl);
-    const VrnnBwdDeal dl = vrnn_bwd_deal(ctH, ctZ, ctR, tl, cus, shared, pchain_split3(), dec ? (H + R) / 16 : 0);
+    const VrnnBwdDeal dl = vrnn_bwd_deal(ctH, ctZ, ctR, tl, cus, shared, pchain_split3(), dec ? (H + R) / 16 : 0, encf ? X / 16 : 0);
     BLVM_REQUIRE(!dec || (dl.split3 && dl.bdec[0].nwg > 0 && !groups), "vrnn_bwd: the deal has no decoder leader range");
+    BLVM_REQUIRE(!encf || (dl.split3 && dl.benc[0].nwg > 0 && !groups), "vrnn_bwd: the deal has no range for the d_enc follower");
     Builder bld;
     bld.begin(pchain_optype(B), T + 1, B, groups ? 8 : 2, true, dl.g);
     bld.p.rt_group = RTG;
@@ -722,8 +749,19 @@
       b2.p[LIN_A] = lead(ws.DY116, xH); b2.p[LIN_W] = ws.dT[0]; b2.p[LIN_ORM] = lead(ws.DD, sD); b2.ld[LD_OUT] = ldd;
       add_desc(bld, K_LIN, (H + R) / 16, dl.bdec[2].wg0, dl.bdec[2].nwg, H, DF_RM_SC1 | DF_GENTLE | DF_CANARY, 0, T - L, b2);
     }
+    if (encf) {
+      const long sX = (long)B * X;
+      auto lag = [&](const float* base, long step) { return rev(base, step, T - 1 + kBencLag); };
+      Operands e0, e1;
+      e0.p[LIN_A] = lag(ws.DGI16, x3R); e0.p[LIN_W] = ws.wixT; e0.p[LIN_ORM] = lag(ws.EP, sX); e0.ld[LD_OUT] = X;
+      add_desc(bld, K_LIN, X / 16, dl.benc[0].wg0, dl.benc[0].nwg, 3 * R, DF_RM_SC1 | DF_GENTLE | DF_CANARY, kBencLag, T + 1, e0);
+      e1.p[LIN_A] = lag(ws.DQ16[0], xH); e1.p[LIN_W] = ws.qxT; e1.p[LIN_ADD] = lag(ws.EP, sX); e1.ld[LIN_LD_ADD] = X;
+      e1.p[LIN_ORM] = lag(d_enc, sX); e1.ld[LD_OUT] = X;
+      add_desc(bld, K_LIN, X / 16, dl.benc[1].wg0, dl.benc[1].nwg, H, DF_ADD_POLLED | DF_GENTLE | DF_CANARY, kBencLag, T + 1, e1);
+    }
     ArmPlan plan;
     plan.fill(ws.GA, ws.x16_bytes);
+    if (encf) plan.fill(ws.EP, sizeof(float) * n * X);
     if (!groups) {
       plan.add(arm_rm(ws.GA, R, B, T, true)); plan.add(arm_rm(ws.GB, R, B, T, true));
       for (int i = 0; i < 3; ++i) { plan.add(arm_t16(ws.DP16[i], H, rt, T, true)); plan.add(arm_t16(ws.DQ16[i], H, rt, T, true)); }
@@ -732,6 +770,7 @@
       plan.add(arm_t16(ws.DPH16, 2 * Z, rt, T, true)); plan.add(arm_t16(ws.DQH16, 2 * Z, rt, T, true));
       plan.add(arm_t16(ws.DPHI16b, H, rt, T, true)); plan.add(arm_t16(ws.DPHI16c, H, rt, T, true));
       if (dec) { plan.add(arm_t16(ws.DY216, H, rt, T, true)); plan.add(arm_t16(ws.DY116, H, rt, T, true)); plan.add(arm_rm(ws.DD, ldd, B, T, true)); }
+      if (encf) plan.add(arm_rm(ws.EP, X, B, T, true));
     }
     auto lead_rows = [&]() -> int {
       if (!dec) return BLVM_OK;
@@ -743,6 +782,7 @@
     };
     BLVM_TRY(vrnn_launch(bld, false, "vrnn_bwd", s, plan, lead_rows));
     if (dec) ++g_dec_bwd_folded;
+    if (encf) ++g_enc_bwd_folded;
     if (split3) {
       const size_t n4 = n * H / 4;
       hipLaunchKernelGGL(add3_kernel, dim3((unsigned)std::min<size_t>((n4 + 255) / 256, 2048)), dim3(256), 0, s, reinterpret_cast<float4*>(ws.DPHI[3]),
diff --git a/benchmarking-lvms_amd/csrc/vrnn_static.h b/benchmarking-lvms_amd/csrc/vrnn_static.h
--- a/benchmarking-lvms_amd/csrc/vrnn_static.h
+++ b/benchmarking-lvms_amd/csrc/vrnn_static.h
@@ -42,12 +42,13 @@
   return d;
 }
 constexpr int kBdecAhead = 2;
+constexpr int kBencLag = 1;
 struct VrnnBwdDeal {
   int def_n, half, g, spare;
   bool split3;
-  LinkRange grub, part[3], dphi, gb, wide_h, dz, prior, post, bdec[3];
-};
-inline VrnnBwdDeal vrnn_bwd_deal(int ctH, int ctZ, int ctR, int tl, int cus, bool shared, bool allow_split3, int ctD = 0) {
+  LinkRange grub, part[3], dphi, gb, wide_h, dz, prior, post, bdec[3], benc[2];
+};
+inline VrnnBwdDeal vrnn_bwd_deal(int ctH, int ctZ, int ctR, int tl, int cus, bool shared, bool allow_split3, int ctD = 0, int ctX = 0) {
   VrnnBwdDeal d;
   d.def_n = shared ? 0 : range_for(ctR * tl, std::min(cus / 4, 64));
   d.half = range_for(ctH * tl, (cus - d.def_n) / 2);
@@ -76,6 +77,12 @@
       d.bdec[2] = LinkRange{ctD, w0, n};
     }
   }
+  for (LinkRange& r : d.benc) r = LinkRange{0, 0, 0};
+  if (ctX > 0 && d.split3) {
+    bool fits = ctX * tl == d.post.nwg && d.wide_h.wg0 + d.wide_h.nwg <= d.post.wg0 && d.dz.wg0 + d.dz.nwg <= d.post.wg0;
+    for (bool xcd : {false, true}) fits = fits && tiles_per_workgroup(tl, ctX, d.post.nwg, xcd) <= 1;
+    if (fits) d.benc[0] = d.benc[1] = LinkRange{ctX, d.post.wg0, d.post.nwg};
+  }
   return d;
 }
 
@@ -85,6 +92,7 @@
 constexpr std::initializer_list<int> kFwdDecResident = {6, 7, 8};
 constexpr int kBwdDesc = 10, kBwdDecDesc = 13;
 constexpr std::initializer_list<int> kBwdDecResident = {11};
+constexpr int kBwdEncLinks = 2, kBwdEncDesc = kBwdDesc + kBwdEncLinks, kBwdDecEncDesc = kBwdDecDesc + kBwdEncLinks;
 inline bool one_tile_each(const Program& p, std::initializer_list<int> links, bool xcd) {
   for (int i : links)
     if (tiles_per_workgroup((p.B + 15) / 16, p.d[i].ct, p.d[i].nwg, xcd) > 1) return false;
diff --git a/benchmarking-lvms_amd/csrc/vrnn_static.hip b/benchmarking-lvms_amd/csrc/vrnn_static.hip
--- a/benchmarking-lvms_amd/csrc/vrnn_static.hip
+++ b/benchmarking-lvms_amd/csrc/vrnn_static.hip
@@ -24,7 +24,7 @@
 }
 __device__ __forceinline__ int tile_count(int lanes) { return __popcll(__ballot(lanes >= 0)); }
 
-constexpr int kAnatBase = 128, kAnatRole = 512, kAnatSlots = 56;
+constexpr int kAnatBase = 128, kAnatRole = 512, kAnatSlots = 64;
 #ifdef PCHAIN_TPROF
 __device__ __forceinline__ void anat_begin(unsigned* tab) {
   for (int i = threadIdx.x; i < kAnatSlots * 8; i += blockDim.x) tab[i] = 0u;
@@ -458,6 +458,12 @@
   else fwd_half<NW, 1>(a, w, rt, xcd, wk);
 }
 
+struct EncArgs {
+  float *ep, *out;
+  const float *W0, *W1;
+  int stride;
+};
+
 struct BwdArgs {
   GrubArgs grub;
   LinArgs part[3], gb, sum;
@@ -466,6 +472,8 @@
   SeqArgs run[2];
   LinArgs bdec[3];
   Deal deal[kBwdDecDesc];
+  EncArgs enc;
+  int nenc;
   int nbdec;
   int bdec_k, gb_ldadd2;
   SPtr gb_add2;
@@ -476,6 +484,19 @@
 };
 
 static_assert(sizeof(BwdArgs) <= 4096 && sizeof(FwdArgs) <= 4096, "kernel argument size");
+__device__ __forceinline__ SPtr lagged(const SPtr& p) { return SPtr{p.base - (long)kBencLag * p.stride, p.stride}; }
+__device__ __forceinline__ LinArgs enc_lin(const BwdArgs& a, int k) {
+  LinArgs q{};
+  q.a = lagged(k == 0 ? a.grub.dgi16 : a.run[1].o16[2]);
+  q.orm = SPtr{k == 0 ? a.enc.ep : a.enc.out, a.enc.stride};
+  if (k == 1) { q.add = SPtr{a.enc.ep, a.enc.stride}; q.ld1 = kH; }
+  q.W = k == 0 ? a.enc.W0 : a.enc.W1;
+  q.ld3 = kH;
+  return q;
+}
+__device__ __forceinline__ Deal enc_deal(const BwdArgs& a, int k) {
+  return Deal{a.deal[9].wg0, a.deal[9].nwg, kH / 16, kBencLag, a.S, (a.nbdec != 0 ? kBwdDecDesc : kBwdDesc) + k};
+}
 
 template <int NW, int HALF>
 __device__ __forceinline__ void bwd_half(const BwdArgs& a, int w, int rt, bool xcd, Walk& wk) {
@@ -548,7 +569,47 @@
 #endif
 }
 
+constexpr int kBenc0Flags = DF_RM_SC1 | DF_GENTLE | DF_CANARY, kBenc1Flags = DF_ADD_POLLED | DF_GENTLE | DF_CANARY;
 template <int NW>
+__device__ __forceinline__ void bwd_post_follower(const BwdArgs& a, int w, int rt, bool xcd, Walk& wk) {
+  const int t0 = tile_lanes(w, a.deal[0].wg0, a.deal[0].nwg, rt, a.deal[0].ct, xcd), n0 = tile_count(t0);
+  const int t1 = tile_lanes(w, a.deal[2].wg0, a.deal[2].nwg, rt, a.deal[2].ct, xcd), n1 = tile_count(t1);
+  const int t8 = tile_lanes(w, a.deal[9].wg0, a.deal[9].nwg, rt, a.deal[9].ct, xcd), n8 = tile_count(t8);
+  const int te = tile_lanes(w, a.deal[9].wg0, a.deal[9].nwg, rt, kH / 16, xcd), ne = tile_count(te);
+  Res<kH, 2> grub;
+  Res<kR> part;
+  RunRes<3, 2 * kH, kH> run;
+  Res<kH> wq;
+  load_grub<NW>(grub, kargs<BwdArgs>().grub, t0, n0);
+  load_lin<NW, kR>(part, kargs<BwdArgs>().part[1].W, kargs<BwdArgs>().part[1].w_width, t1, n1);
+  load_run<NW>(run, kargs<BwdArgs>().run[1], t8, n8);
+  load_lin<NW, kH>(wq, kargs<BwdArgs>().enc.W1, kH, te, ne);
+#ifdef PCHAIN_TPROF
+  unsigned long long follow = 0;
+  const unsigned long long tb = wall_clock64();
+#endif
+  for (int s = a.s0; s < a.S; ++s) {
+    visit_grub<NW, Paced>(kargs<BwdArgs>().grub, kargs<BwdArgs>().deal[0], s, t0, n0, wk, grub);
+    visit_lin<NW, kR, 0, Paced>(kargs<BwdArgs>().part[1], kargs<BwdArgs>().deal[2], s, t1, n1, wk, part);
+    ANAT(const unsigned long long f0 = wall_clock64();)
+    visit_lin<NW, 3 * kR, kBenc0Flags>(enc_lin(kargs<BwdArgs>(), 0), enc_deal(kargs<BwdArgs>(), 0), s, te, ne, wk, WMem());
+    visit_lin<NW, kH, kBenc1Flags>(enc_lin(kargs<BwdArgs>(), 1), enc_deal(kargs<BwdArgs>(), 1), s, te, ne, wk, wq);
+    ANAT(follow += wall_clock64() - f0;)
+    visit_run<NW, 3, 2 * kH, kH, true>(kargs<BwdArgs>().run[1], kargs<BwdArgs>().deal[9], s, t8, n8, wk, run);
+  }
+#ifdef PCHAIN_TPROF
+  const unsigned long long whole = wall_clock64() - tb;
+  __syncthreads();
+  if (threadIdx.x == 0) {
+    unsigned* q = wk.anat + 13 * 2 * 4;
+    q[0] = (unsigned)(a.S - a.s0); q[2] = (unsigned)follow;
+    q[8] = 1u; q[10] = (unsigned)whole;
+  }
+  anat_end(wk.anat, kargs<BwdArgs>().prof, 3, w == kargs<BwdArgs>().deal[2].wg0);
+#endif
+}
+
+template <int NW, bool ENC = false>
 __global__ __launch_bounds__(NW * 64, 1) void vrnn_static_bwd_kernel(BwdArgs a) {
   extern __shared__ __attribute__((aligned(16))) float lds_red[];
   const int w = placed_wg(a.place), rt = (a.B + 15) / 16;
@@ -586,6 +647,7 @@
     return;
   }
   if (w < a.deal[2].wg0) bwd_half<NW, 0>(a, w, rt, xcd, wk);
+  else if constexpr (ENC) bwd_post_follower<NW>(a, w, rt, xcd, wk);
   else bwd_half<NW, 1>(a, w, rt, xcd, wk);
 }
 
@@ -602,7 +664,7 @@
 template <class Kern>
 int static_go(Kern kernel, int slot, int grid, size_t lds, const char* what) {
   static std::mutex mu;
-  static int attr_dev[3] = {-1, -1, -1}, occ[3] = {0, 0, 0};
+  static int attr_dev[4] = {-1, -1, -1, -1}, occ[4] = {0, 0, 0, 0};
   int dev = 0, cus = 0;
   BLVM_HIP(hipGetDevice(&dev));
   BLVM_HIP(hipDeviceGetAttribute(&cus, hipDeviceAttributeMultiprocessorCount, dev));
@@ -768,8 +830,10 @@
 
 int vrnn_static_bwd(const Program& p, hipStream_t stream, const ArmPlan& plan, const std::function<int()>& pre) {
   int place = kPlaceProgram;
-  const bool lead = p.ndesc == kBwdDecDesc;
-  if (vrnn_static_check(p, lead ? kBwdDecDesc : kBwdDesc, kBwdProducts, 8, 9, &place)) return 1;
+  const bool enc = p.ndesc == kBwdEncDesc || p.ndesc == kBwdDecEncDesc;
+  const bool lead = p.ndesc - (enc ? kBwdEncLinks : 0) == kBwdDecDesc;
+  const int nbase = lead ? kBwdDecDesc : kBwdDesc;
+  if (vrnn_static_check(p, nbase + (enc ? kBwdEncLinks : 0), kBwdProducts, 8, 9, &place)) return 1;
   const Desc* d = p.d;
   const int S = p.S;
   for (int i = 0; i < kBwdDesc; ++i)
@@ -797,6 +861,22 @@
     if (!one_tile_each(p, kBwdDecResident, place_xcd(place, p))) return 1;
     if (d[3].p[LIN_ADD] == nullptr || d[4].p[LIN_ADD2] == nullptr || d[1].p[LIN_ADD] != nullptr || d[0].p[GRUB_DD] != nullptr) return 1;
   }
+  if (enc) {
+    const Desc &e0 = d[nbase], &e1 = d[nbase + 1];
+    const long st_dgi = p.stride[d[0].sidx[GRUB_DGI16]], st_dq = p.stride[d[9].sidx[LINSEQ_O16 + 2]], st_ep = p.stride[e0.sidx[LIN_ORM]];
+    if (e0.p[LIN_A] != d[0].p[GRUB_DGI16] - kBencLag * st_dgi || p.stride[e0.sidx[LIN_A]] != st_dgi) return 1;
+    if (e1.p[LIN_A] != d[9].p[LINSEQ_O16 + 2] - kBencLag * st_dq || p.stride[e1.sidx[LIN_A]] != st_dq || p.stride[e1.sidx[LIN_ORM]] != st_ep) return 1;
+    for (const Desc* e : {&e0, &e1}) {
+      if (e->s_begin != kBencLag || e->s_end != S || e->wg0 != d[9].wg0 || e->nwg != d[9].nwg || e->wg0 != half || e->nwg != gentle - half || e->ct != kH / 16 || e->ct * ((p.B + 15) / 16) != e->nwg) return 1;
+      if (e->p[LIN_A2] || e->p[LIN_A3] || e->p[LIN_O16] || e->p[LIN_O16B] || e->p[LIN_GATE] || e->p[LIN_BIAS] || e->p[LIN_ADD2] || !e->p[LIN_ORM]) return 1;
+      if (e->i[LIN_I_W_WIDTH] != 0 || e->ld[LIN_LD_A] != 0 || e->ld[LD_OUT] != kH) return 1;
+    }
+    if (!shaped(e0, K_LIN, kBenc0Flags, 3 * kR) || !shaped(e1, K_LIN, kBenc1Flags, kH) || e0.p[LIN_ADD] != nullptr) return 1;
+    if (e1.p[LIN_ADD] != e0.p[LIN_ORM] || p.stride[e1.sidx[LIN_ADD]] != st_ep || e1.ld[LIN_LD_ADD] != kH) return 1;
+    if (!one_tile_each(p, {nbase, nbase + 1}, place_xcd(place, p))) return 1;
+    for (int i : {5, 6, 7})
+      if (!within(d[i], 0, half)) return 1;
+  }
   BwdArgs a{};
   const Desc& g = d[0];
   a.grub = GrubArgs{sp(p, g, GRUB_D0_16), sp(p, g, GRUB_D1_16), sp(p, g, GRUB_G_IN), sp(p, g, GRUB_RG), sp(p, g, GRUB_UG), sp(p, g, GRUB_NG), sp(p, g, GRUB_GH),
@@ -815,15 +895,28 @@
   a.nbdec = lead ? 3 : 0;
   if (lead) { a.bdec_k = d[kBwdDesc].K; a.gb_add2 = sp(p, d[4], LIN_ADD2); a.gb_ldadd2 = d[4].i[LIN_I_LD_ADD2]; }
   for (int k = 0; k < a.nbdec; ++k) a.bdec[k] = lin_args(p, d[kBwdDesc + k]);
+  a.nenc = enc ? kBwdEncLinks : 0;
+  if (enc) {
+    const Desc &e0 = d[nbase], &e1 = d[nbase + 1];
+    a.enc = EncArgs{const_cast<float*>(e0.p[LIN_ORM]), const_cast<float*>(e1.p[LIN_ORM]), e0.p[LIN_W], e1.p[LIN_W], (int)p.stride[e0.sidx[LIN_ORM]]};
+  }
   int grid = 0;
-  for (int i = 0; i < p.ndesc; ++i) { a.deal[i] = deal_of(d[i], i); grid = std::max(grid, d[i].wg0 + d[i].nwg); }
+  for (int i = 0; i < p.ndesc; ++i) {
+    if (i < nbase) a.deal[i] = deal_of(d[i], i);
+    grid = std::max(grid, d[i].wg0 + d[i].nwg);
+  }
   a.B = p.B; a.s0 = p.s_first; a.S = S; a.xcd = p.xcd; a.place = place; a.ctl = p.ctl;
   ANAT(a.prof = pchain_profile_buffer();)
   BLVM_TRY(arm_or_fill(p, plan, 3, {}, spare, d[3].nwg, place_xcd(place, p), stream, &a.arm));
   BLVM_TRY(pre());
   const size_t lds = sizeof(float) * 2 * kBwdProducts * 16 * 256;
-  BLVM_TRY(static_go(&vrnn_static_bwd_kernel<16>, 1, grid, lds, "vrnn_static_bwd"));
-  hipLaunchKernelGGL(vrnn_static_bwd_kernel<16>, dim3(grid), dim3(1024), lds, stream, a);
+  if (enc) {
+    BLVM_TRY(static_go(&vrnn_static_bwd_kernel<16, true>, 3, grid, lds, "vrnn_static_bwd"));
+    hipLaunchKernelGGL((vrnn_static_bwd_kernel<16, true>), dim3(grid), dim3(1024), lds, stream, a);
+  } else {
+    BLVM_TRY(static_go(&vrnn_static_bwd_kernel<16, false>, 1, grid, lds, "vrnn_static_bwd"));
+    hipLaunchKernelGGL((vrnn_static_bwd_kernel<16, false>), dim3(grid), dim3(1024), lds, stream, a);
+  }
   BLVM_CHECK_LAUNCH("vrnn_static_bwd");
   ++g_static_launches;
   if (a.arm.n != 0) ++g_armed_launches;
diff --git a/include/blvm_hip.h b/include/blvm_hip.h
--- a/include/blvm_hip.h
+++ b/include/blvm_hip.h
@@ -208,6 +208,8 @@
                           int SF, float slope, int* folded, void* stream);
 int blvm_vrnn_dec_bwd_fold(int mode);
 
+int blvm_vrnn_enc_bwd_fold(int mode);
+
 size_t blvm_lstm_reserve_floats(int T, int B, int H);
 size_t blvm_lstm_bwd_workspace_floats(int T, int B, int H);
 int blvm_lstm_seq_fwd(const float* Wih, const float* Whh, const float* bih, const float* bhh, const float* in,
```

After: 98.21 million, median of 6. 2.3% higher.
